# luoao-kddi/SCP

Hardware: AMD Instinct MI355X
Metric: KITTI frames/sec encode (SCP-EHEM, level 16) + bpp match vs ref (higher is better)
Workload: dtype f32 (dense layers and attention as bf16x3 split on bf16 MFMA, feature kNN as f16x3 split on f16 MFMA, fp32 accumulate; position kNN / CDF in fp32); 1 GPU; SCP-EHEM KITTI-like synthetic 120k-pt frames, --spher --mullevel lidar_level=16 (BASELINE.json configs[2]), seeded random weights; nodes_per_frame=577403, windows_per_frame=100, frames_per_gpu=46, frames_in_flight=4, frames_per_launch_sequence=1, transform=host-numpy on a prefetch thread (strict identity: the reference's integers), parallelism=frame-sharded x1, rank_cores=256, rank_cores_pinned=False

## Files before the change

include/scp.h:

```cpp
#ifndef SCP_H
#define SCP_H
#include <stddef.h>
#include <stdint.h>

#ifdef __cplusplus
extern "C" {
#endif

#define SCP_API __attribute__((visibility("default")))

#define SCP_OK 0
#define SCP_EINVAL (-1)
#define SCP_ENOMEM (-2)
#define SCP_ESMALL (-3)
#define SCP_EHIP (-4)
#define SCP_ESTATE (-5)

#define SCP_MAX_DEPTH 21
#define SCP_MAX_SEGMENTS 62

#define SCP_ABI_VERSION 220
SCP_API int scp_version(void);
SCP_API int scp_last_hip_error(void);
SCP_API int scp_device_count(void);
SCP_API int scp_device_name(char *buf, int cap);

typedef struct scp_ctx scp_ctx;
enum { SCP_CTX_KNN_F16X3 = 1, SCP_CTX_ATTENTION_BF16X3 = 2 };
SCP_API int scp_ctx_create(scp_ctx **out);
SCP_API int scp_ctx_destroy(scp_ctx *c);
SCP_API int scp_ctx_set(scp_ctx *c, int32_t key, int32_t value);
SCP_API int scp_ctx_get(const scp_ctx *c, int32_t key);
SCP_API int scp_ctx_make_current(const scp_ctx *c);

enum { SCP_CART = 0, SCP_SPHER = 1, SCP_CYLIN = 2 };

typedef struct scp_quant_info {
    double bin_num;
    double qs[3];
    double offset[3];
    int32_t max_coord;
    int32_t min_coord;
} scp_quant_info;

SCP_API int scp_quantize(const float *xyz, int64_t n, int32_t mode, double qs, double cart_offset,
                 int32_t *q_out, float *tr_out, scp_quant_info *info, void *stream);

typedef struct scp_geom scp_geom;

typedef struct scp_segment {
    int64_t point_begin;
    int64_t point_count;
    int32_t path_len;
    int32_t path_bits;
    int32_t drop_last;
    int32_t reserved;
} scp_segment;

typedef struct scp_segment_info {
    int32_t depth;
    int32_t max_coord;
    int64_t n_leaves;
    int64_t n_nodes;
    int64_t node_base;
    int64_t level_count[SCP_MAX_DEPTH + 1];
} scp_segment_info;

SCP_API int scp_geom_create(scp_geom **out);
SCP_API int scp_geom_destroy(scp_geom *g);

SCP_API int scp_geom_build(scp_geom *g, const int32_t *q, int64_t n, const scp_segment *segs, int32_t nseg,
                   scp_segment_info *info, void *stream);

SCP_API int scp_geom_build_xyz(scp_geom *g, const float *const *frames, const int64_t *n_points, int32_t nframes, int32_t mode,
                               const double *qs, int32_t nshell, double cart_offset, const scp_segment *shells, int32_t *q_out,
                               scp_quant_info *qinfo, scp_segment_info *info, void *stream);

SCP_API int scp_geom_emit_nodes(scp_geom *g, uint8_t *occ, uint8_t *level, uint8_t *octant, int32_t *parent,
                        int32_t *pos, void *stream);

SCP_API int scp_geom_emit_leaves(scp_geom *g, int32_t seg, int32_t *pts, void *stream);

SCP_API int scp_geom_krecords_i64(scp_geom *g, int32_t seg, int64_t *out, void *stream);

enum { SCP_POS_MINMAX = 0,
       SCP_POS_MINMAX_MUL = 1,
       SCP_POS_POW2 = 2 };

SCP_API int scp_geom_context_ehem(scp_geom *g, int32_t seg, int32_t pos_mode, int32_t lidar_level,
                          uint8_t *ctx, float *pos, uint8_t *sym, int64_t *pos_mm, void *stream);

SCP_API int scp_geom_context_ehem_all(scp_geom *g, int32_t pos_mode, int32_t lidar_level, int32_t context_size, uint8_t *ctx, float *pos,
                                      uint8_t *sym_coded, int64_t *pos_mm, void *stream);

SCP_API int scp_geom_context_octattn(scp_geom *g, int32_t seg, uint8_t *ctx, float *pos, uint8_t *sym, void *stream);

SCP_API int scp_knn_topk(const float *x, int32_t B, int32_t n, int32_t C, int32_t k, int32_t *idx, void *stream);

SCP_API int scp_knn_topk_packed(const float *x, const int32_t *ctab, int32_t total_rows, int32_t C, int32_t *idx, void *stream);
SCP_API int scp_knn_topk_packed_bounded(const float *x, const int32_t *ctab, int32_t total_rows, int32_t C, const float *thr0,
                                int32_t *idx, void *stream);

SCP_API int scp_edge_gather_max(const float *u, const float *v, const int32_t *idx, const float *scale, const float *shift,
                        int32_t B, int32_t n, int32_t Cout, int32_t k, float *out, int32_t out_stride, void *stream);
SCP_API int scp_edge_gather_max_ld(const float *u, int64_t ldu, const float *v, int64_t ldv, const int32_t *idx, const float *scale,
                           const float *shift, int32_t B, int32_t n, int32_t Cout, int32_t k, float *out, int32_t out_stride,
                           void *stream);

SCP_API int scp_swin_attention(const float *q, const float *k, const float *v, const float *bias_table,
                       int32_t B, int32_t Lp, int32_t shift, int32_t ldq, int32_t ldkv, float *out, void *stream);

SCP_API int scp_split_weight_bf16(const float *W, int32_t N, int32_t K, int32_t Npad, int32_t Kpad, void *hi, void *lo, void *stream);
SCP_API int scp_linear_bf16x3(const float *A, int64_t lda, const void *Whi, const void *Wlo, int32_t Kpad, const float *bias,
                      const float *residual, int64_t ldr, float *C, int64_t ldc, int32_t M, int32_t N, int32_t K, int32_t act,
                      void *stream);

SCP_API int scp_split_weight_f16(const float *W, int32_t N, int32_t K, int32_t Npad, int32_t Kpad, void *hi, void *lo,
                                 float *inv_scale, void *stream);
SCP_API int scp_linear_f16x3(const float *A, int64_t lda, const void *Whi, const void *Wlo, const float *w_inv_scale, int32_t Kpad,
                             const float *bias, const float *residual, int64_t ldr, float *C, int64_t ldc, int32_t M, int32_t N,
                             int32_t K, int32_t act, float *row_scale_ws, void *stream);
SCP_API int scp_row_scale_f16(const float *A, int64_t lda, int32_t M, int32_t K, float *scale, float *inv_scale, void *stream);
SCP_API int scp_linear_f16x3_scaled(const float *A, int64_t lda, const void *Whi, const void *Wlo, const float *w_inv_scale, int32_t Kpad,
                                    const float *bias, const float *residual, int64_t ldr, float *C, int64_t ldc, int32_t M, int32_t N,
                                    int32_t K, int32_t act, const float *scale, const float *inv_scale, void *stream);

SCP_API int scp_tile_weight_bf16(const void *plane, int32_t Npad, int32_t Kpad, void *tiled, void *stream);
SCP_API int scp_split_rows_f16(const float *A, int64_t lda, int32_t M, int32_t K, void *hi, void *lo, int64_t ldp, float *scale, float *inv_scale,
                               void *stream);
SCP_API int scp_layernorm_add_split_f16(const float *a, const float *b, int64_t rows, int32_t C, const float *gamma, const float *beta, float eps,
                                        float *out, void *hi, void *lo, int64_t ldp, float *scale, float *inv_scale, void *stream);
SCP_API int scp_linear_split_f16(const void *Ahi, const void *Alo, int64_t lda, const float *a_inv_scale, const void *Whi, const void *Wlo,
                                 const float *w_inv_scale, int32_t Npad, int32_t Kpad, const float *bias, const float *residual, int64_t ldr,
                                 float *C, int64_t ldc, int32_t M, int32_t N, int32_t K, int32_t act, int32_t cfg, void *stream);
SCP_API int scp_linear_split_f16_max(const void *Ahi, const void *Alo, int64_t lda, const float *a_inv_scale, const void *Whi, const void *Wlo,
                                     const float *w_inv_scale, int32_t Npad, int32_t Kpad, const float *bias, const float *residual, int64_t ldr,
                                     float *C, int64_t ldc, int32_t M, int32_t N, int32_t K, int32_t act, int32_t cfg, uint32_t *row_max,
                                     uint32_t *col_max, int32_t col_lo, int32_t col_hi, int32_t col_rows, void *stream);
SCP_API int scp_row_scale_from_max(const uint32_t *row_max, int32_t M, float *scale, float *inv_scale, void *stream);
SCP_API int scp_linear_split(const void *Ahi, const void *Alo, int64_t lda, const void *Whi, const void *Wlo, int32_t Npad, int32_t Kpad,
                     const float *bias, const float *residual, int64_t ldr, float *C, int64_t ldc, void *Ohi, void *Olo, int64_t ldo,
                     int32_t M, int32_t N, int32_t K, int32_t act, int32_t cfg, void *stream);

SCP_API int scp_linear_split_gather(const void *Ahi, const void *Alo, int64_t lda, const void *Whi, const void *Wlo, int32_t Npad, int32_t Kpad,
                            const float *bias, const float *residual, int64_t ldr, const int64_t *res_map, float *C, int64_t ldc, void *Ohi,
                            void *Olo, int64_t ldo, int32_t M, int32_t N, int32_t K, int32_t act, int32_t cfg, void *stream);
SCP_API int scp_linear_split_hier2(const void *A0hi, const void *A0lo, int64_t lda0, int32_t K0pad, const void *A1hi, const void *A1lo, int64_t lda1,
                                   int64_t M1, const void *W0hi, const void *W0lo, const void *W1hi, const void *W1lo, int32_t Npad,
                                   const int64_t *parent, const float *bias, const float *res, int64_t ldr, const int64_t *res_map, void *Ohi,
                                   void *Olo, int64_t ldo, int32_t M, int32_t N, int32_t act, void *stream);
SCP_API int scp_linear_split_scatter(const void *Ahi, const void *Alo, int64_t lda, const void *Whi, const void *Wlo, int32_t Npad, int32_t Kpad,
                             const float *bias, const int64_t *out_map, float *C, int64_t ldc, int32_t M, int32_t N, int32_t K, int32_t act,
                             int32_t cfg, void *stream);
SCP_API int scp_split_rows(const float *src, int64_t ld_src, int64_t n_src, const int64_t *idx, int32_t C, void *hi, void *lo, int64_t ldo,
                   int64_t rows, void *stream);
SCP_API int scp_layernorm_rows_split(const float *x, int64_t ldx, int64_t n_src_rows, const int64_t *ia, const int64_t *ib, int32_t C,
                             const float *gamma, const float *beta, const float *valid, float eps, void *ohi, void *olo, int64_t ldo,
                             int64_t rows, void *stream);
SCP_API int scp_layernorm_add(const float *a, const float *b, int64_t rows, int32_t C, const float *gamma, const float *beta, float eps,
                              float *out, void *stream);
SCP_API int scp_swin_attention_packed_split(const float *q, const float *k, const float *v, const float *bias_table, const int32_t *wtab,
                                    int32_t total_windows, int32_t shift, int32_t ldq, int32_t ldkv, void *ohi, void *olo, int64_t ldo,
                                    void *stream);


SCP_API int scp_swin_attention_packed(const float *q, const float *k, const float *v, const float *bias_table, const int32_t *wtab,
                              int32_t total_windows, int32_t shift, int32_t ldq, int32_t ldkv, float *out, void *stream);

SCP_API int scp_layernorm_rows(const float *x, int64_t ldx, int64_t n_src_rows, const int64_t *ia, const int64_t *ib, int32_t C,
                       const float *gamma, const float *beta, const float *valid, float eps, float *out, int64_t ldo, int64_t rows,
                       void *stream);
SCP_API int scp_gather_rows(const float *src, int64_t lds, const int64_t *idx, int32_t C, float *out, int64_t ldo, int64_t rows, void *stream);

SCP_API int scp_linear_f32(const float *A, int64_t lda, const float *W, const float *bias, float *C, int64_t ldc, int32_t M, int32_t N, int32_t K,
                   int32_t act, void *stream);

SCP_API int scp_octattn_attention(const float *q_u, const float *k, const float *k_u, const float *v, const float *v_u,
                          int32_t B, int32_t c, int32_t H, int32_t hd, float *out, float *out_u, void *stream);

SCP_API int64_t scp_octattn_f16x3_ws_bytes(int32_t B, int32_t c, int32_t H);
SCP_API int scp_octattn_attention_f16x3(const float *q_u, const float *k, const float *k_u, const float *v, const float *v_u,
                                        int64_t ldkv, int32_t B, int32_t c, int32_t H, int32_t hd, float *out, float *out_u, void *workspace,
                                        int64_t ws_bytes, void *stream);
SCP_API int scp_octattn_attention_f16x3_vmax(const float *q_u, const float *k, const float *k_u, const float *v, const float *v_u,
                                             int64_t ldkv, int32_t B, int32_t c, int32_t H, int32_t hd, float *out, float *out_u, void *workspace,
                                             int64_t ws_bytes, const uint32_t *vmax_bits, void *stream);
SCP_API int scp_octattn_attention_rowinv(const float *q_u, int64_t qw, int64_t qr, const float *k, const float *v, int64_t kw, int64_t kr,
                                         const float *k_u, const float *v_u, int64_t uw, int64_t ur, float *out, float *out_u, int64_t ow,
                                         int64_t orr, int32_t B, int32_t q0, int32_t q1, int32_t qoff, int32_t H, int32_t hd, void *stream);
SCP_API int scp_decode_expand_octattn(const int64_t *sym, const int64_t *cum, const uint8_t *ctx, const int32_t *apos, int64_t n, int32_t L,
                                      int32_t shift, int32_t depth, uint8_t *cctx, int32_t *capos, float *cpos, uint8_t *occ8, void *stream);
SCP_API int scp_octattn_embed(const uint8_t *ctx, const float *pos, int64_t n, int32_t c, const float *occ_enc, int32_t d_occ,
                              const float *level_enc, int32_t d_lvl, int32_t max_level, const float *octant_enc, int32_t d_oct,
                              const float *pos_w, const float *pos_b, int32_t d_pos, const float *pe, int32_t level_cap, float *E,
                              void *hi, void *lo, int64_t ldp, float *scale, float *inv_scale, void *stream);

SCP_API int scp_softmax_cdf(const float *logits, int64_t ld, int64_t n, int32_t nsym, const uint8_t *sym,
                    float *pmf, uint32_t *lohi, uint16_t *cdf_full, void *stream);
SCP_API int scp_pmf_cdf(const float *pmf, int64_t n, int32_t nsym, const uint8_t *sym, uint32_t *lohi,
                uint16_t *cdf_full, void *stream);

SCP_API int scp_ac_encode_cdf(const uint16_t *cdf, const int16_t *sym, int64_t n, int32_t Lp, uint8_t *out, size_t cap,
                      size_t *out_len);
SCP_API int scp_ac_encode_lohi(const uint32_t *lohi, int64_t n, uint8_t *out, size_t cap, size_t *out_len);
typedef struct scp_ac_dec scp_ac_dec;
SCP_API int scp_ac_dec_new(scp_ac_dec **d, const uint8_t *stream, size_t len, int32_t Lp);
SCP_API int scp_ac_dec_next(scp_ac_dec *d, const uint16_t *cdf_row);
SCP_API int scp_ac_dec_run(scp_ac_dec *d, const uint16_t *cdf, int64_t n, int16_t *out);
SCP_API int scp_ac_dec_free(scp_ac_dec *d);

typedef struct scp_legacy_node { uint32_t nodeid, octant, parent; uint8_t oct; uint32_t pos[3]; } scp_legacy_node;
SCP_API void *new_vector(void);
SCP_API void delete_vector(void *v);
SCP_API int vector_size(void *v);
SCP_API void *vector_get(void *v, int level);
SCP_API void vector_push_back(void *v, int i);
SCP_API void *genOctreeInterface(void *v, const double *xyz, int n);
SCP_API int Nodes_size(void *level);
SCP_API scp_legacy_node *Nodes_get(void *level, int i);
SCP_API int int_size(void *codes);
SCP_API int int_get(void *codes, int i);

SCP_API int scp_nn_sqdist_f64(const double *a, int64_t na, const double *b, int64_t nb, double *d2, void *stream);

SCP_API int scp_embed_gather(const uint8_t *ctx, const float *pos, const int64_t *inmap, int64_t n_tokens, const float *occ_enc,
                     const float *level_enc, const float *octant_enc, float *x, float *pos_out, int64_t *occ_self, int64_t rows,
                     void *stream);

SCP_API int scp_packed_plan_sizes(const int64_t *lengths, int32_t W, int64_t *rows_out);
SCP_API int scp_packed_plan(const int64_t *lengths, int32_t W, int64_t *tables_dev, void *const *outs, int32_t n_outs, void *stream);

SCP_API int scp_decode_expand(const int64_t *sym, const int64_t *cum, const int32_t *pos, const uint8_t *anc, const uint8_t *octant, int64_t n,
                              int32_t L, int32_t shift, int32_t lv_next, int32_t lv_clamp, int32_t polar, double mn, double den, int32_t *cpos,
                              uint8_t *canc, uint8_t *coct, uint8_t *cctx, float *cposn, uint8_t *occ8, void *stream);

SCP_API int scp_swin_ln_linear(const float *x, int64_t ldx, const float *valid, const void *Whi, const void *Wlo, const float *bias,
                               const float *wbeta, float eps, float *out, int64_t ldo, int32_t M, int32_t N, void *stream);
SCP_API int scp_swin_post_attn(const void *Ohi, const void *Olo, int64_t ldo_in, const float *x, int64_t ldx, const void *W, const float *bp,
                               const float *b1, const float *b2, float eps, float *out, int64_t ldc, int32_t M, const int32_t *tile_list,
                               int32_t n_tiles, void *stream);
SCP_API int64_t scp_swin_post_attn_weight_bytes(void);
SCP_API double scp_gelu_prescale(void);

SCP_API int scp_swin_merge(const float *x, int64_t ldx, int64_t n_src, const int64_t *ia, const int64_t *ib, const void *W, const float *wbeta,
                           float eps, float *out, int64_t ldo, int32_t M, void *stream);

SCP_API int scp_geo_edge_mlps(const float *pos1, int64_t ld1, const float *pos2, int64_t ld2, const float *pos3, int64_t ld3, const void *W,
                              const float *bias, float *out, int64_t ldo, int32_t M, void *stream);
SCP_API int scp_mlp3_rows(const float *x, int64_t ldx, int64_t n_src, const int64_t *in_map, const void *W, const float *bias, float *out, int64_t ldo,
                          const int64_t *out_map, int32_t M, int32_t N, void *stream);

SCP_API int scp_swin_kv_planes(const float *k, const float *v, int64_t ldkv, int64_t rows, void *khi, void *klo, void *vthi, void *vtlo, void *stream);
SCP_API int scp_swin_ln_qkv(const float *x, int64_t ldx, const float *valid, const void *Whi, const void *Wlo, const float *bias, const float *wbeta,
                            float eps, float *q, int64_t ldq, void *planes, int64_t Tp, int32_t M, int32_t N, void *stream);
SCP_API int scp_swin_attention_packed_planes(const float *q, const void *khi, const void *klo, const void *vthi, const void *vtlo,
                                             const float *bias_table, const int32_t *wtab, int32_t total_windows, int32_t shift, int32_t ldq,
                                             float *out, void *ohi, void *olo, int64_t ldo, const float *valid, void *stream);

#ifdef __cplusplus
}
#endif
#endif
```

scp_amd/csrc/rowchain.hip:

```cpp
#include <stdlib.h>
#include "scp_internal.h"

typedef __bf16 rbf16x8 __attribute__((ext_vector_type(8)));
typedef float rf32x16 __attribute__((ext_vector_type(16)));
typedef float rf32x4 __attribute__((ext_vector_type(4)));
typedef int ri32x4 __attribute__((ext_vector_type(4)));
typedef __attribute__((address_space(3))) void *rc_lds_ptr_t;
typedef const __attribute__((address_space(1))) void *rc_glb_ptr_t;

#define RC_ROWS 128
#define RC_SLOT 32768
#define RC_RING (4 * RC_SLOT)
#define RC_BOUNCE 4096
#define RC_OFF_BOUNCE RC_RING
#define RC_OFF_BIAS (RC_RING + 4 * RC_BOUNCE)
#define RC_LDS (RC_OFF_BIAS + 16384)

__device__ __forceinline__ void rc_dma16(const void *g, char *l) {
    __builtin_amdgcn_global_load_lds((rc_glb_ptr_t)g, (rc_lds_ptr_t)l, 16, 0, 0);
}

typedef float rf32x2 __attribute__((ext_vector_type(2)));
typedef __bf16 rbf16x2 __attribute__((ext_vector_type(2)));
typedef unsigned ru32x4 __attribute__((ext_vector_type(4)));
typedef unsigned ru32x2 __attribute__((ext_vector_type(2)));
__device__ __forceinline__ unsigned rc_pack2(float a, float b) {
    const rf32x2 v = {a, b};
    return __builtin_bit_cast(unsigned, __builtin_convertvector(v, rbf16x2));
}
__device__ __forceinline__ void rc_split2(float a, float b, unsigned &hi, unsigned &lo) {
    asm volatile("" : "+v"(a), "+v"(b));
    hi = rc_pack2(a, b);
    lo = rc_pack2(a - __builtin_bit_cast(float, hi << 16), b - __builtin_bit_cast(float, hi & 0xffff0000u));
}
__device__ __forceinline__ void rc_split8(const float *f, rbf16x8 &hi, rbf16x8 &lo) {
    ru32x4 h, l;
#pragma unroll
    for (int i = 0; i < 4; ++i) { unsigned a, b; rc_split2(f[2 * i], f[2 * i + 1], a, b); h[i] = a; l[i] = b; }
    hi = __builtin_bit_cast(rbf16x8, h);
    lo = __builtin_bit_cast(rbf16x8, l);
}

struct RcLane {
    int lane, col, h, w;
    int frag;
    int rg;
};

__device__ __forceinline__ RcLane rc_lane() {
    RcLane L;
    const int tid = threadIdx.x;
    L.lane = tid & 63; L.col = L.lane & 31; L.h = L.lane >> 5;
    L.w = __builtin_amdgcn_readfirstlane(tid >> 6);
    L.frag = (L.col & 15) * 64 + ((L.h ^ ((L.col >> 2) & 3)) << 4);
    L.rg = L.col >> 4;
    return L;
}

__device__ __forceinline__ void rc_issue_rowchunk(const RcLane &L, const __bf16 *Whi, const __bf16 *Wlo, int g, char *slot) {
#pragma unroll
    for (int j = 0; j < 4; ++j) {
        const int p = L.w + 4 * j;
        const int64_t off = ((int64_t)g * 16 + p) * 512 + L.lane * 8;
        rc_dma16(Whi + off, slot + p * 1024);
        rc_dma16(Wlo + off, slot + 16384 + p * 1024);
    }
}

__device__ __forceinline__ void rc_issue_kchunk(const RcLane &L, const __bf16 *Whi, const __bf16 *Wlo, int c, int nks, char *slot) {
#pragma unroll
    for (int j = 0; j < 4; ++j) {
        const int p = L.w + 4 * j;
        const int64_t off = ((int64_t)p * nks + c) * 512 + L.lane * 8;
        rc_dma16(Whi + off, slot + p * 1024);
        rc_dma16(Wlo + off, slot + 16384 + p * 1024);
    }
}

__device__ __forceinline__ rbf16x8 rc_frag_rowchunk(const RcLane &L, const char *slot, int plane, int s) {
    return *(const rbf16x8 *)(slot + plane * 16384 + (L.rg * 8 + (s >> 1)) * 1024 + (L.frag ^ ((s & 1) << 5)));
}

__device__ __forceinline__ rbf16x8 rc_frag_kchunk(const RcLane &L, const char *slot, int plane, int b, int t) {
    return *(const rbf16x8 *)(slot + plane * 16384 + (2 * b + L.rg) * 1024 + (L.frag ^ (t << 5)));
}

#define RC_DS_READ4_WAIT(d0, a0, o0, d1, a1, o1, d2, a2, o2, d3, a3, o3)                                                              \
    asm volatile("ds_read_b128 %0, %4 offset:%8\n\tds_read_b128 %1, %5 offset:%9\n\tds_read_b128 %2, %6 offset:%10\n\t"                   \
                 "ds_read_b128 %3, %7 offset:%11\n\ts_waitcnt lgkmcnt(0)"                                                              \
                 : "=&v"(d0), "=&v"(d1), "=&v"(d2), "=&v"(d3) : "v"(a0), "v"(a1), "v"(a2), "v"(a3), "n"(o0), "n"(o1), "n"(o2), "n"(o3) : "memory")
#define RC_DS_READ(dst, addr, off) asm volatile("ds_read_b128 %0, %1 offset:%2" : "=v"(dst) : "v"(addr), "n"(off) : "memory")

__device__ __forceinline__ void rc_mfma3x2(rf32x16 &c0, rf32x16 &c1, const rbf16x8 &a0h, const rbf16x8 &a0l, const rbf16x8 &a1h,
                                           const rbf16x8 &a1l, const rbf16x8 &bh, const rbf16x8 &bl) {
    c0 = __builtin_amdgcn_mfma_f32_32x32x16_bf16(a0l, bh, c0, 0, 0, 0);
    c1 = __builtin_amdgcn_mfma_f32_32x32x16_bf16(a1l, bh, c1, 0, 0, 0);
    c0 = __builtin_amdgcn_mfma_f32_32x32x16_bf16(a0h, bl, c0, 0, 0, 0);
    c1 = __builtin_amdgcn_mfma_f32_32x32x16_bf16(a1h, bl, c1, 0, 0, 0);
    c0 = __builtin_amdgcn_mfma_f32_32x32x16_bf16(a0h, bh, c0, 0, 0, 0);
    c1 = __builtin_amdgcn_mfma_f32_32x32x16_bf16(a1h, bh, c1, 0, 0, 0);
}

__device__ __forceinline__ void rc_store_block(const RcLane &L, char *bounce, const rf32x4 v[4], __amdgpu_buffer_rsrc_t rs, int ldo_bytes, int voff,
                                               int ch0) {
#pragma unroll
    for (int q = 0; q < 4; ++q)
        *(rf32x4 *)(bounce + L.col * 128 + (((2 * q + L.h) ^ (L.col & 7)) << 4)) = v[q];
    asm volatile("s_waitcnt lgkmcnt(0)" ::: "memory");
    rf32x4 y[4];
#pragma unroll
    for (int it = 0; it < 4; ++it) {
        const int rho = 8 * it + (L.lane >> 3), kap = L.lane & 7;
        y[it] = *(const rf32x4 *)(bounce + rho * 128 + ((kap ^ (rho & 7)) << 4));
    }
#pragma unroll
    for (int it = 0; it < 4; ++it) __builtin_amdgcn_raw_buffer_store_b128(__builtin_bit_cast(ri32x4, y[it]), rs, voff, it * 8 * ldo_bytes + ch0 * 4, 0);
    asm volatile("s_waitcnt lgkmcnt(0)" ::: "memory");
}

__device__ __forceinline__ void rc_ln_stats(const float *v , float eps, float &mean, float &rstd) {
    float s = 0.f;
#pragma unroll
    for (int i = 0; i < 128; i += 4) s += (v[i] + v[i + 1]) + (v[i + 2] + v[i + 3]);
    s += __shfl_xor(s, 32);
    mean = s * (1.0f / 256.0f);
    float q = 0.f;
#pragma unroll
    for (int i = 0; i < 128; ++i) { const float d = v[i] - mean; q += d * d; }
    q += __shfl_xor(q, 32);
    rstd = rsqrtf(q * (1.0f / 256.0f) + eps);
}

struct RcLnLinArgs {
    const float *x; int64_t ldx;
    const float *valid;
    const __bf16 *Whi, *Wlo;
    const float *bias, *wbeta;
    float *out; int64_t ldo;
    int M, N;
    float eps;
    int probe;
    unsigned long long *dbg;
    __bf16 *planes; int64_t plane_bytes; int nq;
    int ngroups;
};

#define RC_DS_WRITE(addr, val, off) asm volatile("ds_write_b128 %0, %1 offset:%2" :: "v"(addr), "v"(val), "n"(off) : "memory")

#define RC_SB __builtin_amdgcn_sched_barrier(0)
#ifndef RC_SKEW
#define RC_SKEW 0
#endif
#if RC_SKEW > 0
#define RC_STEP_BARRIER(WAITS, w)                                                                                                          \
    do {                                                                                                                                   \
        int _rc_n;                                                                                                                         \
        asm volatile("s_waitcnt " WAITS "\n\ts_barrier\n\ts_mov_b32 %0, %1\n\ts_cmp_eq_u32 %0, 0\n\ts_cbranch_scc1 .Lrcskew_done%=\n"          \
                     ".Lrcskew_loop%=:\n\ts_nop 7\n\ts_sub_u32 %0, %0, 1\n\ts_cmp_lg_u32 %0, 0\n\ts_cbranch_scc1 .Lrcskew_loop%=\n"              \
                     ".Lrcskew_done%=:"                                                                                                   \
                     : "=&s"(_rc_n) : "s"((w) * RC_SKEW) : "memory", "scc");                                                                \
    } while (0)
#else
#ifdef RC_PROBE_NOBAR
#define RC_STEP_BARRIER(WAITS, w) asm volatile("s_waitcnt " WAITS ::: "memory")
#else
#define RC_STEP_BARRIER(WAITS, w) asm volatile("s_waitcnt " WAITS "\n\ts_barrier" ::: "memory")
#endif
#endif
#ifdef RC_PROBE_NODMA
#define RC_PROBE_DMA_ON 0
#else
#define RC_PROBE_DMA_ON 1
#endif
#ifdef RC_PROBE_NOFRAG
#define RC_PROBE_FRAG_ON 0
#else
#define RC_PROBE_FRAG_ON 1
#endif
#ifdef RC_DMA_SPREAD
#define RC_DMA_P(s, gap) ((s) < 4 ? 2 * (s) + ((gap) == 3) : (s) + 4)
#define RC_DMA_HERE(s, gap) (((s) < 4 && ((gap) == 1 || (gap) == 3)) || ((s) >= 4 && (s) < 12 && (gap) == 1))
#define RC_DMA_SLOT(s, gap) (RC_DMA_P(s, gap) >> 3)
#define RC_DMA_IDX(s, gap) ((RC_DMA_P(s, gap) >> 1) & 3)
#define RC_DMA_PLANE(s, gap) (RC_DMA_P(s, gap) & 1)
#else
#define RC_DMA_HERE(s, gap) ((s) < 8 && ((gap) == 1 || (gap) == 3))
#define RC_DMA_SLOT(s, gap) ((s) >> 2)
#define RC_DMA_IDX(s, gap) ((s) & 3)
#define RC_DMA_PLANE(s, gap) ((gap) >> 1)
#endif
#ifdef RC_WAIT0
#define RC_FRAG_WAIT() asm volatile("s_waitcnt lgkmcnt(0)" ::: "memory")
#else
#define RC_FRAG_WAIT() asm volatile("s_waitcnt lgkmcnt(3)" ::: "memory")
#endif
#ifndef RC_STORE_AUX
#define RC_STORE_AUX 0
#endif
template <bool LOADX, int PROBE, bool SWAP = false, bool NSWAP = false>
__device__ __forceinline__ void rc_ll_step(const RcLane &L, const RcLnLinArgs &a, char *smem, int half, rf32x16 &c0, rf32x16 &c1,
                                           rf32x16 &p0, rf32x16 &p1, const rbf16x8 (&Xh)[16], const rbf16x8 (&Xl)[16], int g_next,
                                           __amdgpu_buffer_rsrc_t rs_prev, int voff, int ldo_bytes, int ch0_prev, const unsigned (&bw)[4],
                                           unsigned br, const float *xsrc, float (&v)[128], rbf16x8 (&A)[2][4], const float *tb_next, unsigned long long *st,
                                           __amdgpu_buffer_rsrc_t wr_hi, __amdgpu_buffer_rsrc_t wr_lo, const float *sbn = nullptr, unsigned maskh = 0) {
    const unsigned ab = (unsigned)(uintptr_t)(rc_lds_ptr_t)(smem + half * (2 * RC_SLOT)) + L.rg * 8192;
    const unsigned ad0 = ab + L.frag, ad1 = ab + (L.frag ^ 32);
    const unsigned an0 = (unsigned)(uintptr_t)(rc_lds_ptr_t)(smem + (half ^ 1) * (2 * RC_SLOT)) + L.rg * 8192 + L.frag;
    char *nxt = smem + (half ^ 1) * (2 * RC_SLOT);
    rf32x4 rd[4];
    unsigned long long ts0 = 0;
    if (st) ts0 = __builtin_amdgcn_s_memtime();
#pragma unroll
    for (int s = 0; s < 16; ++s) {
        if (st && (s == 1 || s == 8 || s == 15)) { const unsigned long long t = __builtin_amdgcn_s_memtime(); st[s == 1 ? 0 : s == 8 ? 1 : 2] += t - ts0; ts0 = t; }
        if (s == 15) {
            asm volatile("s_waitcnt lgkmcnt(0)" ::: "memory");
            if (PROBE) RC_STEP_BARRIER("vmcnt(0)", L.w);
            else if (LOADX) RC_STEP_BARRIER("vmcnt(24)", L.w);
            else RC_STEP_BARRIER("vmcnt(8)", L.w);
            if (st) { const unsigned long long t = __builtin_amdgcn_s_memtime(); st[3] += t - ts0; ts0 = t; }
        }
        RC_SB;
        const int nb = (s + 1) & 1, ns = (s + 1) & 15;
        const unsigned ra = (ns & 1) ? ad1 : ad0;
#pragma unroll
        for (int gap = 0; gap < 6; ++gap) {
            if (gap < 4) { RC_FRAG_WAIT(); RC_SB; }
#define RC_LL_MFMA(c, wf, xf) c = SWAP ? __builtin_amdgcn_mfma_f32_32x32x16_bf16(xf, wf, c, 0, 0, 0) : __builtin_amdgcn_mfma_f32_32x32x16_bf16(wf, xf, c, 0, 0, 0)
            if (gap == 0) RC_LL_MFMA(c0, A[s & 1][1], Xh[s]);
            if (gap == 1) RC_LL_MFMA(c1, A[s & 1][3], Xh[s]);
            if (gap == 2) RC_LL_MFMA(c0, A[s & 1][0], Xl[s]);
            if (gap == 3) RC_LL_MFMA(c1, A[s & 1][2], Xl[s]);
            if (gap == 4) RC_LL_MFMA(c0, A[s & 1][0], Xh[s]);
            if (gap == 5) RC_LL_MFMA(c1, A[s & 1][2], Xh[s]);
#undef RC_LL_MFMA
            RC_SB;
            if (gap < 4 && s < 15) {
                if (gap == 0) RC_DS_READ(A[nb][1], ra, 16384 + (ns >> 1) * 1024);
                if (gap == 1) RC_DS_READ(A[nb][3], ra, RC_SLOT + 16384 + (ns >> 1) * 1024);
                if (gap == 2) RC_DS_READ(A[nb][0], ra, (ns >> 1) * 1024);
                if (gap == 3) RC_DS_READ(A[nb][2], ra, RC_SLOT + (ns >> 1) * 1024);
            }
            if (s < 8 && (gap == 1 || gap == 3) && !(PROBE & 2)) {
                const int slot = s >> 2, pb = L.w + 4 * (s & 3), plane = gap >> 1;
                const int soff = ((g_next + slot) * 16 + pb) * 1024;
                __builtin_amdgcn_raw_ptr_buffer_load_lds(plane ? wr_lo : wr_hi, (rc_lds_ptr_t)(nxt + slot * RC_SLOT + plane * 16384 + pb * 1024), 16,
                                                         L.lane * 16, soff, 0, 0);
            }
            if ((s == 8 || s == 11) && gap < 4 && !(PROBE & 8)) {
                const rf32x16 &pp = (s == 8) ? p0 : p1;
                const rf32x4 t = {pp[4 * gap], pp[4 * gap + 1], pp[4 * gap + 2], pp[4 * gap + 3]};
                RC_DS_WRITE(bw[gap], t, 0);
            }
            if ((s == 9 || s == 12) && gap < 4 && !(PROBE & 8))
                asm volatile("ds_read_b128 %0, %1 offset:%2" : "=v"(rd[gap]) : "v"(br), "n"(gap * 1024) : "memory");
            if ((s == 10 || s == 13) && gap < 4 && !(PROBE & 8))
                __builtin_amdgcn_raw_buffer_store_b128(__builtin_bit_cast(ri32x4, rd[gap]), rs_prev, voff,
                                                       gap * 8 * ldo_bytes + (ch0_prev + 32 * (s == 13 ? 1 : 0)) * 4, RC_STORE_AUX);
            if (LOADX && s >= 14 && gap < 4 && !(PROBE & 4)) {
#pragma unroll
                for (int t = 8 * (s - 14) + 2 * gap; t < 8 * (s - 14) + 2 * gap + 2; ++t) {
                    const rf32x4 q0 = *(const rf32x4 *)(xsrc + 16 * t), q1 = *(const rf32x4 *)(xsrc + 16 * t + 4);
#pragma unroll
                    for (int u = 0; u < 4; ++u) { v[8 * t + u] = q0[u]; v[8 * t + 4 + u] = q1[u]; }
                }
            }
            if (NSWAP && s == 14 && gap >= 4) {
                const float bb = sbn[32 * (gap - 4)], bwv = sbn[32 * (gap - 4) + 1024];
                rf32x16 &pp = (gap == 4) ? p0 : p1;
#pragma unroll
                for (int r = 0; r < 16; ++r) pp[r] = ((maskh >> (8 * (r >> 2) + (r & 3))) & 1u) ? bwv : bb;
            }
            if (!NSWAP && s == 14 && gap >= 4) {
#pragma unroll
                for (int q = 2 * (gap - 4); q < 2 * (gap - 4) + 2; ++q) {
                    const rf32x4 b0 = *(const rf32x4 *)(tb_next + 8 * q), b1 = *(const rf32x4 *)(tb_next + 32 + 8 * q);
#pragma unroll
                    for (int u = 0; u < 4; ++u) { p0[4 * q + u] = b0[u]; p1[4 * q + u] = b1[u]; }
                }
            }
            RC_SB;
        }
    }
    RC_DS_READ4_WAIT(A[0][1], an0, 16384, A[0][3], an0, RC_SLOT + 16384, A[0][0], an0, 0, A[0][2], an0, RC_SLOT);
    if (st) { const unsigned long long t = __builtin_amdgcn_s_memtime(); st[4] += t - ts0; }
}

template <int PROBE, bool KV = false>
__global__ __launch_bounds__(256, 1) void rc_ln_linear_kernel(const RcLnLinArgs a) {
    extern __shared__ __attribute__((aligned(1024))) char smem[];
    const RcLane L = rc_lane();
    const int ntiles = (a.M + RC_ROWS - 1) / RC_ROWS;
    const int nsteps = a.N >> 6;
    float *sb = (float *)(smem + RC_OFF_BIAS), *sbw = sb + 1024;
    for (int i = threadIdx.x; i < a.N; i += 256) {
        const float b = a.bias ? a.bias[i] : 0.f;
        sb[i] = b; sbw[i] = b + (a.wbeta ? a.wbeta[i] : 0.f);
    }
    __syncthreads();
    const int ngr = a.ngroups > 1 ? a.ngroups : 1;
    int tile = blockIdx.x / ngr;
    const int tstride = (int)gridDim.x / ngr;
    const int j0 = (int)(blockIdx.x % ngr) * (nsteps / ngr), j1 = j0 + nsteps / ngr;
    if (tile >= ntiles) return;
    char *bounce = smem + RC_OFF_BOUNCE + L.w * RC_BOUNCE;
    unsigned bw[4];
#pragma unroll
    for (int q = 0; q < 4; ++q) bw[q] = (unsigned)(uintptr_t)(rc_lds_ptr_t)(bounce + L.col * 128 + (((2 * q + L.h) ^ (L.col & 7)) << 4));
    const unsigned br0 = (unsigned)(uintptr_t)(rc_lds_ptr_t)(bounce + (L.lane >> 3) * 128 + (((L.lane & 7) ^ ((L.lane >> 3) & 7)) << 4));
    const int ldo_bytes = (int)(a.ldo * 4);
    const int voff = (32 * L.w + (L.lane >> 3)) * ldo_bytes + (L.lane & 7) * 16;
    const __amdgpu_buffer_rsrc_t rs_none = __builtin_amdgcn_make_buffer_rsrc(a.out, 0, 0, 0x00020000);
    const int pbytes = (int)a.plane_bytes;
    const __amdgpu_buffer_rsrc_t prs = __builtin_amdgcn_make_buffer_rsrc((void *)a.planes, 0, KV ? (int)(4 * a.plane_bytes) : 0, 0x00020000);

    const int wbytes = ((a.N + 255) & ~255) * 512;
    const __amdgpu_buffer_rsrc_t wr_hi = __builtin_amdgcn_make_buffer_rsrc((void *)a.Whi, 0, wbytes, 0x00020000);
    const __amdgpu_buffer_rsrc_t wr_lo = __builtin_amdgcn_make_buffer_rsrc((void *)a.Wlo, 0, wbytes, 0x00020000);
    unsigned long long t_step = 0, t_ln = 0, t_drain = 0, t_prev = 0, n_tiles = 0;
    unsigned long long tsl[5] = {0, 0, 0, 0, 0};
    const bool DBG = a.dbg != nullptr;
    if (DBG) t_prev = __builtin_amdgcn_s_memtime();
    auto stamp = [&](unsigned long long &acc_t) { if (DBG) { const unsigned long long t = __builtin_amdgcn_s_memtime(); acc_t += t - t_prev; t_prev = t; } };

    rc_issue_rowchunk(L, a.Whi, a.Wlo, 2 * j0, smem);
    rc_issue_rowchunk(L, a.Whi, a.Wlo, 2 * j0 + 1, smem + RC_SLOT);
    float v[128];
    auto xrow = [&](int t) {
        const int r = t * RC_ROWS + 32 * L.w + L.col;
        return a.x + (int64_t)(r < a.M ? r : a.M - 1) * a.ldx + 8 * L.h;
    };
    {
        const float *src = xrow(tile);
#pragma unroll
        for (int s = 0; s < 16; ++s) {
            const rf32x4 q0 = *(const rf32x4 *)(src + 16 * s), q1 = *(const rf32x4 *)(src + 16 * s + 4);
#pragma unroll
            for (int u = 0; u < 4; ++u) { v[8 * s + u] = q0[u]; v[8 * s + 4 + u] = q1[u]; }
        }
    }
    rbf16x8 A[2][4];
    {
        SCP_BARRIER_DMA(0);
        const unsigned ad0 = (unsigned)(uintptr_t)(rc_lds_ptr_t)(smem) + L.rg * 8192 + L.frag;
        RC_DS_READ4_WAIT(A[0][1], ad0, 16384, A[0][3], ad0, RC_SLOT + 16384, A[0][0], ad0, 0, A[0][2], ad0, RC_SLOT);
    }
    int gstep = 0;
    for (; tile < ntiles; tile += tstride) {
        const int m0 = tile * RC_ROWS;
        const int row = m0 + 32 * L.w + L.col;
        const int rowc = row < a.M ? row : a.M - 1;
        float keep = (row < a.M) ? 1.0f : 0.0f;
        if (a.valid) keep *= a.valid[rowc];
        float mean, rstd;
        rc_ln_stats(v, a.eps, mean, rstd);
        const float sc = rstd * keep;
        rbf16x8 Xh[16], Xl[16];
#pragma unroll
        for (int s = 0; s < 16; ++s) {
            float f[8];
#pragma unroll
            for (int i = 0; i < 8; ++i) f[i] = (v[8 * s + i] - mean) * sc;
            rc_split8(f, Xh[s], Xl[s]);
        }
        stamp(t_ln);
        const float *tb = (keep != 0.f ? sbw : sb) + 4 * L.h;
        const int64_t rows_left = (int64_t)a.M - m0;
        const int64_t span = (rows_left < RC_ROWS ? rows_left : RC_ROWS) * a.ldo * 4;
        const __amdgpu_buffer_rsrc_t rs = (a.probe & 1) ? rs_none : __builtin_amdgcn_make_buffer_rsrc(a.out + (int64_t)m0 * a.ldo, 0, (int)span, 0x00020000);
        const bool more = tile + tstride < ntiles;
        const float *xnext = xrow(more ? tile + tstride : tile);

        rf32x16 acc[2][2];
#pragma unroll
        for (int q = 0; q < 4; ++q) {
            const rf32x4 b0 = *(const rf32x4 *)(tb + 64 * j0 + 8 * q), b1 = *(const rf32x4 *)(tb + 64 * j0 + 32 + 8 * q);
#pragma unroll
            for (int u = 0; u < 4; ++u) { acc[0][0][4 * q + u] = b0[u]; acc[0][1][4 * q + u] = b1[u]; }
        }
        if (!KV) {
        for (int j = j0; j < j1; j += 2) {
            if (j + 2 == j1)
                rc_ll_step<true, PROBE>(L, a, smem, gstep & 1, acc[0][0], acc[0][1], acc[1][0], acc[1][1], Xh, Xl, 2 * (j + 1), j > j0 ? rs : rs_none, voff,
                                 ldo_bytes, 64 * (j - 1), bw, br0, xnext, v, A, tb + 64 * (j + 1), DBG ? tsl : nullptr, wr_hi, wr_lo);
            else
                rc_ll_step<false, PROBE>(L, a, smem, gstep & 1, acc[0][0], acc[0][1], acc[1][0], acc[1][1], Xh, Xl, 2 * (j + 1), j > j0 ? rs : rs_none, voff,
                                  ldo_bytes, 64 * (j - 1), bw, br0, xnext, v, A, tb + 64 * (j + 1), DBG ? tsl : nullptr, wr_hi, wr_lo);
            ++gstep;
            rc_ll_step<false, PROBE>(L, a, smem, gstep & 1, acc[1][0], acc[1][1], acc[0][0], acc[0][1], Xh, Xl, (j + 2 < j1) ? 2 * (j + 2) : 2 * j0, rs, voff,
                              ldo_bytes, 64 * j, bw, br0, xnext, v, A, tb + 64 * ((j + 2 < j1) ? j + 2 : j0), DBG ? tsl : nullptr, wr_hi, wr_lo);
            ++gstep;
        }
        stamp(t_step);
        asm volatile("s_waitcnt lgkmcnt(0)" ::: "memory");
#pragma unroll
        for (int blk = 0; blk < 2; ++blk) {
            rf32x4 o[4];
#pragma unroll
            for (int q = 0; q < 4; ++q)
#pragma unroll
                for (int u = 0; u < 4; ++u) o[q][u] = acc[1][blk][4 * q + u];
            rc_store_block(L, bounce, o, rs, ldo_bytes, voff, 64 * (j1 - 1) + 32 * blk);
        }
        } else {
        const int nq = a.nq;
        const unsigned kmask = (unsigned)__builtin_amdgcn_ballot_w64(keep != 0.f);
        const unsigned maskh = kmask >> (4 * L.h);
        const float *sbl = sb + L.col;
        const int kvoff = (m0 + 32 * L.w + (L.lane >> 3)) * 512 + (L.lane & 7) * 16;
        const int vblk = ((m0 >> 5) + L.w) * 4;
        auto split_pair = [&](float x0, float x1, int plane) {
            const unsigned hh = rc_pack2(x0, x1);
            return plane ? rc_pack2(x0 - __builtin_bit_cast(float, hh << 16), x1 - __builtin_bit_cast(float, hh & 0xffff0000u)) : hh;
        };
        auto store_k = [&](const rf32x16 &c0, const rf32x16 &c1, int head) {
            ri32x4 y[2][4];
#pragma unroll
            for (int plane = 0; plane < 2; ++plane) {
#pragma unroll
                for (int b = 0; b < 2; ++b)
#pragma unroll
                    for (int q = 0; q < 4; ++q) {
                        const rf32x16 &c = b ? c1 : c0;
                        *(ru32x2 *)(bounce + L.col * 128 + (((4 * b + q) ^ (L.col & 7)) << 4) + 8 * L.h) =
                            (ru32x2){split_pair(c[4 * q], c[4 * q + 1], plane), split_pair(c[4 * q + 2], c[4 * q + 3], plane)};
                    }
#pragma unroll
                for (int it = 0; it < 4; ++it) y[plane][it] = *(const ri32x4 *)(bounce + it * 1024 + L.lane * 16);
            }
#pragma unroll
            for (int plane = 0; plane < 2; ++plane)
#pragma unroll
                for (int it = 0; it < 4; ++it)
                    __builtin_amdgcn_raw_buffer_store_b128(y[plane][it], prs, kvoff, it * 8 * 512 + head * 128 + plane * pbytes, 0);
            asm volatile("s_waitcnt lgkmcnt(0)" ::: "memory");
        };
        auto store_v = [&](const rf32x16 &c0, const rf32x16 &c1, int head) {
            ri32x4 y[2][4];
#pragma unroll
            for (int plane = 0; plane < 2; ++plane) {
#pragma unroll
                for (int b = 0; b < 2; ++b)
#pragma unroll
                    for (int cc = 0; cc < 2; ++cc) {
                        const rf32x16 &c = b ? c1 : c0;
                        const int d = L.col + 32 * b, R = d >> 1, sl = (d & 1) * 4 + 2 * cc + L.h;
                        *(ru32x4 *)(bounce + R * 128 + ((sl ^ (R & 7)) << 4)) =
                            (ru32x4){split_pair(c[8 * cc], c[8 * cc + 1], plane), split_pair(c[8 * cc + 2], c[8 * cc + 3], plane),
                                     split_pair(c[8 * cc + 4], c[8 * cc + 5], plane), split_pair(c[8 * cc + 6], c[8 * cc + 7], plane)};
                    }
#pragma unroll
                for (int it = 0; it < 4; ++it) y[plane][it] = *(const ri32x4 *)(bounce + it * 1024 + L.lane * 16);
            }
#pragma unroll
            for (int plane = 0; plane < 2; ++plane)
#pragma unroll
                for (int it = 0; it < 4; ++it)
                    __builtin_amdgcn_raw_buffer_store_b128(y[plane][it], prs, L.lane * 16, it * 1024 + (vblk + head) * 4096 + (2 + plane) * pbytes, 0);
            asm volatile("s_waitcnt lgkmcnt(0)" ::: "memory");
        };
        auto role = [&](int j) { return j < nq ? 0 : (j < nq + 4 ? 1 : 2); };
        if (role(j0) == 2) {
#pragma unroll
            for (int blk = 0; blk < 2; ++blk) {
                const float bb = sbl[64 * j0 + 32 * blk], bwv = sbl[64 * j0 + 32 * blk + 1024];
#pragma unroll
                for (int r = 0; r < 16; ++r) acc[0][blk][r] = ((maskh >> (8 * (r >> 2) + (r & 3))) & 1u) ? bwv : bb;
            }
        }
        auto post = [&](int j, const rf32x16 &c0, const rf32x16 &c1) {
            const int r = role(j);
            if (r == 1) store_k(c0, c1, j - nq);
            else if (r == 2) store_v(c0, c1, j - nq - 4);
        };
        for (int j = j0; j < j1; j += 2) {
            const int jn = j + 2 < j1 ? j + 2 : j0;
            const bool val = role(j) == 2, nval = role(jn) == 2;
            const __amdgpu_buffer_rsrc_t rsa = (j > j0 && role(j - 1) == 0) ? rs : rs_none, rsb = role(j) == 0 ? rs : rs_none;
            const int gn = 2 * jn;
            const float *tbn = tb + 64 * jn, *sbn1 = sbl + 64 * (j + 1), *sbn2 = sbl + 64 * jn;
#define RC_STEP_A(LX, SW) rc_ll_step<LX, PROBE, SW, SW>(L, a, smem, gstep & 1, acc[0][0], acc[0][1], acc[1][0], acc[1][1], Xh, Xl, 2 * (j + 1), rsa, voff, ldo_bytes, \
                                                64 * (j - 1), bw, br0, xnext, v, A, tb + 64 * (j + 1), DBG ? tsl : nullptr, wr_hi, wr_lo, sbn1, maskh)
#define RC_STEP_B(SW, NSW) rc_ll_step<false, PROBE, SW, NSW>(L, a, smem, gstep & 1, acc[1][0], acc[1][1], acc[0][0], acc[0][1], Xh, Xl, gn, rsb, voff, ldo_bytes, 64 * j, bw, \
                                                     br0, xnext, v, A, tbn, DBG ? tsl : nullptr, wr_hi, wr_lo, sbn2, maskh)
            if (!val) RC_STEP_A(false, false);
            else if (j + 2 == j1) RC_STEP_A(true, true);
            else RC_STEP_A(false, true);
            ++gstep;
            post(j, acc[0][0], acc[0][1]);
            if (!val) { if (nval) RC_STEP_B(false, true); else RC_STEP_B(false, false); }
            else { if (nval) RC_STEP_B(true, true); else RC_STEP_B(true, false); }
            ++gstep;
            post(j + 1, acc[1][0], acc[1][1]);
#undef RC_STEP_A
#undef RC_STEP_B
        }
        stamp(t_step);
        if (role(j1 - 1) == 0) {
            asm volatile("s_waitcnt lgkmcnt(0)" ::: "memory");
#pragma unroll
            for (int blk = 0; blk < 2; ++blk) {
                rf32x4 o[4];
#pragma unroll
                for (int q = 0; q < 4; ++q)
#pragma unroll
                    for (int u = 0; u < 4; ++u) o[q][u] = acc[1][blk][4 * q + u];
                rc_store_block(L, bounce, o, rs, ldo_bytes, voff, 64 * (j1 - 1) + 32 * blk);
            }
        }
        }
        stamp(t_drain);
        ++n_tiles;
    }
    if (DBG && L.lane == 0) {
        unsigned long long *o = a.dbg + ((size_t)blockIdx.x * 4 + L.w) * 8;
        o[0] = tsl[3]; o[1] = t_step; o[2] = t_ln; o[3] = t_drain; o[4] = n_tiles; o[5] = tsl[0]; o[6] = tsl[1]; o[7] = tsl[2] + tsl[4];
    }
    SCP_WAIT_DMA(0);
}

struct RcPostArgs {
    const __bf16 *Ohi, *Olo; int64_t ldo_in;
    const float *x; int64_t ldx;
    const void *W;
    const float *bp, *b1, *b2;
    float *out; int64_t ldc;
    int M;
    float eps;
    unsigned long long *dbg;
    int dbg_mode;
    const int32_t *tile_list; int n_list;
};

#define RC_W_PROJ 0
#define RC_W_FC1 (256 * 512)
#define RC_W_FC2 (RC_W_FC1 + 1024 * 512)
#define RC_W_PLANE (RC_W_FC2 + 256 * 2048)
struct RcSlotSrc { int base, stride; };

__device__ __forceinline__ void rc_dma_piece(const RcLane &L, __amdgpu_buffer_rsrc_t wr, const RcSlotSrc &src, char *slot_lds, int s, int plane) {
    const int pb = L.w + 4 * (s & 3);
    const int soff = src.base + pb * src.stride + plane * RC_W_PLANE;
    __builtin_amdgcn_raw_ptr_buffer_load_lds(wr, (rc_lds_ptr_t)(slot_lds + plane * 16384 + pb * 1024), 16, L.lane * 16, soff, 0, 0);
}

struct RcFragAddr { unsigned r0, r1, k0, k1; };
__device__ __forceinline__ RcFragAddr rc_frag_addr(const RcLane &L, char *half_base) {
    RcFragAddr f;
    const unsigned b = (unsigned)(uintptr_t)(rc_lds_ptr_t)half_base;
    f.r0 = b + L.rg * 8192 + L.frag; f.r1 = b + L.rg * 8192 + (L.frag ^ 32);
    f.k0 = b + L.rg * 1024 + L.frag; f.k1 = b + L.rg * 1024 + (L.frag ^ 32);
    return f;
}

#ifdef RC_PROBE_SHAPE16
__device__ __forceinline__ void rc_mfma_shape16(rf32x16 &acc, const rbf16x8 &a, const rbf16x8 &b) {
    rf32x4 q0 = {acc[0], acc[1], acc[2], acc[3]}, q1 = {acc[4], acc[5], acc[6], acc[7]};
    q0 = __builtin_amdgcn_mfma_f32_16x16x32_bf16(a, b, q0, 0, 0, 0);
    q1 = __builtin_amdgcn_mfma_f32_16x16x32_bf16(a, b, q1, 0, 0, 0);
    acc[0] = q0[0]; acc[1] = q0[1]; acc[2] = q0[2]; acc[3] = q0[3];
    acc[4] = q1[0]; acc[5] = q1[1]; acc[6] = q1[2]; acc[7] = q1[3];
}
#define RC_MFMA_AVA(acc, a, b) rc_mfma_shape16(acc, a, b)
#define RC_MFMA_AVV(acc, a, b) rc_mfma_shape16(acc, a, __builtin_bit_cast(rbf16x8, b))
#else
#define RC_MFMA_AVA(acc, a, b) acc = __builtin_amdgcn_mfma_f32_32x32x16_bf16(a, b, acc, 0, 0, 0)
#define RC_MFMA_AVV(acc, a, b) acc = __builtin_amdgcn_mfma_f32_32x32x16_bf16(a, __builtin_bit_cast(rbf16x8, b), acc, 0, 0, 0)
#endif
#define RC_MFMA_DRAIN() do { } while (0)

template <bool NEXT_BODY>
__device__ __forceinline__ void rc_gemm_step(const RcLane &L, char *smem, int half, rf32x16 &c0, rf32x16 &c1, const rbf16x8 (&Bh)[16],
                                             const rbf16x8 (&Bl)[16], rbf16x8 (&A)[2][4], __amdgpu_buffer_rsrc_t wr, const RcSlotSrc &n0,
                                             const RcSlotSrc &n1) {
    const RcFragAddr f = rc_frag_addr(L, smem + half * (2 * RC_SLOT)), fn = rc_frag_addr(L, smem + (half ^ 1) * (2 * RC_SLOT));
    char *nxt = smem + (half ^ 1) * (2 * RC_SLOT);
#pragma unroll
    for (int s = 0; s < 16; ++s) {
        if (s == 15) RC_STEP_BARRIER("vmcnt(0) lgkmcnt(0)", L.w);
        RC_SB;
        const int nb = (s + 1) & 1, ns = (s + 1) & 15;
#pragma unroll
        for (int gap = 0; gap < 6; ++gap) {
            if (gap < 4 && RC_PROBE_FRAG_ON) { RC_FRAG_WAIT(); RC_SB; }
            if (gap == 0) RC_MFMA_AVA(c0, A[s & 1][1], Bh[s]);
            if (gap == 1) RC_MFMA_AVA(c1, A[s & 1][3], Bh[s]);
            if (gap == 2) RC_MFMA_AVV(c0, A[s & 1][0], Bl[s]);
            if (gap == 3) RC_MFMA_AVV(c1, A[s & 1][2], Bl[s]);
            if (gap == 4) RC_MFMA_AVA(c0, A[s & 1][0], Bh[s]);
            if (gap == 5) RC_MFMA_AVA(c1, A[s & 1][2], Bh[s]);
            RC_SB;
            if (s < 15 && RC_PROBE_FRAG_ON) {
                const unsigned ra = (ns & 1) ? f.r1 : f.r0;
                if (gap == 0) RC_DS_READ(A[nb][1], ra, 16384 + (ns >> 1) * 1024);
                if (gap == 1) RC_DS_READ(A[nb][3], ra, RC_SLOT + 16384 + (ns >> 1) * 1024);
                if (gap == 2) RC_DS_READ(A[nb][0], ra, (ns >> 1) * 1024);
                if (gap == 3) RC_DS_READ(A[nb][2], ra, RC_SLOT + (ns >> 1) * 1024);
            }
            if (RC_DMA_HERE(s, gap) && RC_PROBE_DMA_ON) rc_dma_piece(L, wr, RC_DMA_SLOT(s, gap) ? n1 : n0, nxt + RC_DMA_SLOT(s, gap) * RC_SLOT, RC_DMA_IDX(s, gap), RC_DMA_PLANE(s, gap));
            RC_SB;
        }
    }
    if (NEXT_BODY) RC_DS_READ4_WAIT(A[0][1], fn.r0, 16384, A[0][3], fn.k0, RC_SLOT + 16384, A[0][0], fn.r0, 0, A[0][2], fn.k0, RC_SLOT);
    else RC_DS_READ4_WAIT(A[0][1], fn.r0, 16384, A[0][3], fn.r0, RC_SLOT + 16384, A[0][0], fn.r0, 0, A[0][2], fn.r0, RC_SLOT);
}

struct RcGelu { float ea, eb, pa, pb, wa, wb, xa, xb, ga, gb; unsigned hw; };
__device__ __forceinline__ void rc_gelu_stage(int st, RcGelu &g, float ya, float yb, unsigned &wh, unsigned &wl) {
#ifdef RC_NOGELU
    if (st == 0) { g.ga = ya; g.gb = yb; asm volatile("" : "+v"(g.ga), "+v"(g.gb)); }
    if (st == 10) { g.hw = rc_pack2(g.ga, g.gb); wh = g.hw; asm volatile("" : "+v"(g.hw)); }
    if (st == 11) wl = rc_pack2(g.ga - __builtin_bit_cast(float, g.hw << 16), g.gb - __builtin_bit_cast(float, g.hw & 0xffff0000u));
    return;
#endif
    switch (st) {
    case 0: g.ea = -ya * ya; g.eb = -yb * yb; break;
    case 1: g.ea = __builtin_amdgcn_exp2f(g.ea); g.eb = __builtin_amdgcn_exp2f(g.eb); break;
    case 2: g.pa = fmaf(SCP_GELU_C4, __builtin_fabsf(ya), SCP_GELU_C3); g.pb = fmaf(SCP_GELU_C4, __builtin_fabsf(yb), SCP_GELU_C3); break;
    case 3: g.pa = fmaf(g.pa, __builtin_fabsf(ya), SCP_GELU_C2); g.pb = fmaf(g.pb, __builtin_fabsf(yb), SCP_GELU_C2); break;
    case 4: g.pa = fmaf(g.pa, __builtin_fabsf(ya), SCP_GELU_C1); g.pb = fmaf(g.pb, __builtin_fabsf(yb), SCP_GELU_C1); break;
    case 5: g.pa = fmaf(g.pa, __builtin_fabsf(ya), SCP_GELU_C0); g.pb = fmaf(g.pb, __builtin_fabsf(yb), SCP_GELU_C0); break;
    case 6: g.pa = __builtin_amdgcn_rcpf(g.pa); g.pb = __builtin_amdgcn_rcpf(g.pb); break;
    case 7: g.wa = __builtin_fabsf(ya) * g.ea; g.wb = __builtin_fabsf(yb) * g.eb; break;
    case 8: asm("v_max_f32_e32 %0, 0, %1" : "=v"(g.xa) : "v"(ya)); asm("v_max_f32_e32 %0, 0, %1" : "=v"(g.xb) : "v"(yb)); break;
    case 9: g.ga = fmaf(-g.wa, g.pa, g.xa); g.gb = fmaf(-g.wb, g.pb, g.xb); break;
    case 10: g.hw = rc_pack2(g.ga, g.gb); wh = g.hw; break;
    default: wl = rc_pack2(g.ga - __builtin_bit_cast(float, g.hw << 16), g.gb - __builtin_bit_cast(float, g.hw & 0xffff0000u)); break;
    }
    switch (st) {
    case 0: case 1: asm volatile("" : "+v"(g.ea), "+v"(g.eb)); break;
    case 2: case 3: case 4: case 5: case 6: asm volatile("" : "+v"(g.pa), "+v"(g.pb)); break;
    case 7: asm volatile("" : "+v"(g.wa), "+v"(g.wb)); break;
    case 8: asm volatile("" : "+v"(g.xa), "+v"(g.xb)); break;
    case 9: asm volatile("" : "+v"(g.ga), "+v"(g.gb)); break;
    case 10: asm volatile("" : "+v"(g.ga), "+v"(g.gb), "+v"(g.hw)); break;
    default: break;
    }
}

template <bool HAS_P1, bool HAS_GELU, int NEXT>
__device__ __forceinline__ void rc_body_step(const RcLane &L, char *smem, int half, rf32x16 (&Y)[8], rf32x16 &a1n, const rf32x16 &a1g,
                                             const ru32x4 (&Hch)[2], const ru32x4 (&Hcl)[2], ru32x4 (&Hnh)[2],
                                             ru32x4 (&Hnl)[2], const rbf16x8 (&Xh)[16], const rbf16x8 (&Xl)[16], rbf16x8 (&A)[2][4],
                                             __amdgpu_buffer_rsrc_t wr, const RcSlotSrc &n0, const RcSlotSrc &n1) {
    const RcFragAddr f = rc_frag_addr(L, smem + half * (2 * RC_SLOT)), fn = rc_frag_addr(L, smem + (half ^ 1) * (2 * RC_SLOT));
    char *nxt = smem + (half ^ 1) * (2 * RC_SLOT);
    RcGelu g;
#pragma unroll
    for (int s = 0; s < 16; ++s) {
        if (s == 15) RC_STEP_BARRIER("vmcnt(0) lgkmcnt(0)", L.w);
        RC_SB;
        const int nb = (s + 1) & 1, ns = (s + 1) & 15;
        const int blk = s >> 1, t = s & 1;
#pragma unroll
        for (int gap = 0; gap < 6; ++gap) {
            if (HAS_P1 && gap < 4 && RC_PROBE_FRAG_ON) { RC_FRAG_WAIT(); RC_SB; }
            if (!HAS_P1 && (gap == 1 || gap == 3) && RC_PROBE_FRAG_ON) { asm volatile("s_waitcnt lgkmcnt(1)" ::: "memory"); RC_SB; }
            if (gap == 0 && HAS_P1) RC_MFMA_AVA(a1n, A[s & 1][1], Xh[s]);
            if (gap == 1) RC_MFMA_AVV(Y[blk], A[s & 1][3], Hch[t]);
            if (gap == 2 && HAS_P1) RC_MFMA_AVV(a1n, A[s & 1][0], Xl[s]);
            if (gap == 3) RC_MFMA_AVV(Y[blk], A[s & 1][2], Hcl[t]);
            if (gap == 4 && HAS_P1) RC_MFMA_AVA(a1n, A[s & 1][0], Xh[s]);
            if (gap == 5) RC_MFMA_AVV(Y[blk], A[s & 1][2], Hch[t]);
            RC_SB;
            if (s < 15 && RC_PROBE_FRAG_ON) {
                if (gap == 0 && HAS_P1) RC_DS_READ(A[nb][1], (ns & 1) ? f.r1 : f.r0, 16384 + (ns >> 1) * 1024);
                if (gap == 1) RC_DS_READ(A[nb][3], (ns & 1) ? f.k1 : f.k0, RC_SLOT + 16384 + (ns >> 1) * 2048);
                if (gap == 2 && HAS_P1) RC_DS_READ(A[nb][0], (ns & 1) ? f.r1 : f.r0, (ns >> 1) * 1024);
                if (gap == 3) RC_DS_READ(A[nb][2], (ns & 1) ? f.k1 : f.k0, RC_SLOT + (ns >> 1) * 2048);
            }
            if (RC_DMA_HERE(s, gap) && RC_PROBE_DMA_ON) rc_dma_piece(L, wr, RC_DMA_SLOT(s, gap) ? n1 : n0, nxt + RC_DMA_SLOT(s, gap) * RC_SLOT, RC_DMA_IDX(s, gap), RC_DMA_PLANE(s, gap));
            if (HAS_GELU) {
                const int k = s >> 1, st = (s & 1) * 6 + gap;
                unsigned wh = 0, wl = 0;
// ... 595 lines not shown
#pragma unroll
                for (int s = 0; s < 16; ++s) {
                    float f[8];
#pragma unroll
                    for (int i = 0; i < 8; ++i) f[i] = (vb[8 * s + i] - mean) * rstd;
                    rc_split8(f, Xh[s], Xl[s]);
                }
            }
        }
        asm volatile("s_waitcnt lgkmcnt(0)" ::: "memory");
        const int64_t rows_left = (int64_t)a.M - m0;
        const int64_t span = (rows_left < RC_ROWS ? rows_left : RC_ROWS) * a.ldo * 4;
        const __amdgpu_buffer_rsrc_t rs = __builtin_amdgcn_make_buffer_rsrc(a.out + (int64_t)m0 * a.ldo, 0, (int)span, 0x00020000);
#pragma unroll
        for (int b = 0; b < 8; ++b) {
            rf32x4 o[4];
#pragma unroll
            for (int q = 0; q < 4; ++q)
#pragma unroll
                for (int u = 0; u < 4; ++u) o[q][u] = Y[b][4 * q + u];
            rc_store_block(L, bounce, o, rs, ldo_bytes, voff, 32 * b);
        }
    }
    SCP_WAIT_DMA(0);
}

extern "C" SCP_API int scp_swin_merge(const float *x, int64_t ldx, int64_t n_src, const int64_t *ia, const int64_t *ib, const void *W, const float *wbeta,
                                      float eps, float *out, int64_t ldo, int32_t M, void *stream);

struct RcEdgeArgs {
    const float *p1, *p2, *p3; int64_t ld1, ld2, ld3;
    const void *W; const float *bias;
    float *out; int64_t ldo; int M;
};

__device__ __forceinline__ float rc_leaky(float y) { return y > 0.f ? y : 0.01f * y; }

__global__ __launch_bounds__(256, 1) void rc_edge_mlp_kernel(const RcEdgeArgs a) {
    extern __shared__ __attribute__((aligned(1024))) char smem[];
    const RcLane L = rc_lane();
    const int ntiles = (a.M + RC_ROWS - 1) / RC_ROWS;
    float *sb = (float *)(smem + RC_OFF_BIAS);
    for (int i = threadIdx.x; i < 5 * 256 + 128; i += 256) sb[i] = a.bias[i];
    __syncthreads();
    int tile = blockIdx.x;
    if (tile >= ntiles) return;
    char *bounce = smem + RC_OFF_BOUNCE + L.w * RC_BOUNCE;
    const int ldo_bytes = (int)(a.ldo * 4);
    const int voff = (32 * L.w + (L.lane >> 3)) * ldo_bytes + (L.lane & 7) * 16;
    const __amdgpu_buffer_rsrc_t wr = __builtin_amdgcn_make_buffer_rsrc((void *)a.W, 0, 2 * RC_W_PLANE, 0x00020000);
    auto src = [&](int t, int k) {
        int m, g;
        if (t < 8) { m = t & 1; g = t >> 1; }
        else if (t < 16) { m = t >> 2; g = t & 3; }
        else if (t < 24) { m = 4 + (t & 1); g = (t - 16) >> 1; }
        else if (t < 28) { m = 6; g = t & 3; }
        else { m = 7; g = t - 28; }
        RcSlotSrc r = {m * 131072 + (2 * g + k) * 16384, 1024};
        return r;
    };
    {
        const RcSlotSrc s0 = src(0, 0), s1 = src(0, 1);
#pragma unroll
        for (int q = 0; q < 4; ++q)
#pragma unroll
            for (int plane = 0; plane < 2; ++plane) { rc_dma_piece(L, wr, s0, smem, q, plane); rc_dma_piece(L, wr, s1, smem + RC_SLOT, q, plane); }
    }
    rbf16x8 A[2][4];
    {
        SCP_BARRIER_DMA(0);
        const RcFragAddr f = rc_frag_addr(L, smem);
        RC_DS_READ4_WAIT(A[0][1], f.r0, 16384, A[0][3], f.r0, RC_SLOT + 16384, A[0][0], f.r0, 0, A[0][2], f.r0, RC_SLOT);
    }
    int gstep = 0, t = 0;
    for (; tile < ntiles; tile += gridDim.x) {
        const int m0 = tile * RC_ROWS;
        const int row = m0 + 32 * L.w + L.col;
        const int64_t rowc = row < a.M ? row : a.M - 1;
        const float *q1 = a.p1 + rowc * a.ld1 + 8 * L.h, *q2 = a.p2 + rowc * a.ld2 + 8 * L.h, *q3 = a.p3 + rowc * a.ld3 + 8 * L.h;
        rbf16x8 Xh[16], Xl[16], Zh[16], Zl[16];
        rf32x16 Y[8];
        auto frag_of = [&](const float *p, rbf16x8 &hi, rbf16x8 &lo) {
            const rf32x4 v0 = *(const rf32x4 *)p, v1 = *(const rf32x4 *)(p + 4);
            const float f[8] = {v0[0], v0[1], v0[2], v0[3], v1[0], v1[1], v1[2], v1[3]};
            rc_split8(f, hi, lo);
        };
        auto to_frags = [&](rbf16x8 (&Fh)[16], rbf16x8 (&Fl)[16], bool act) {
#pragma unroll
            for (int b = 0; b < 8; ++b)
#pragma unroll
                for (int tt = 0; tt < 2; ++tt) {
                    float fr[8];
#pragma unroll
                    for (int i = 0; i < 8; ++i) fr[i] = act ? rc_leaky(Y[b][8 * tt + i]) : Y[b][8 * tt + i];
                    rc_split8(fr, Fh[2 * b + tt], Fl[2 * b + tt]);
                }
        };
#define RC_STEP(Fh, Fl) { const int tn = t + 1 < 30 ? t + 1 : 0; rc_gemm_step<false>(L, smem, gstep & 1, c0, c1, Fh, Fl, A, wr, src(tn, 0), src(tn, 1)); ++gstep; t = tn; }
#define RC_LAYER(LAYER, NG, STEPS)                                                                                                             \
        for (int g = 0; g < (NG); ++g) {                                                                                                       \
            rf32x16 c0, c1;                                                                                                                    \
            _Pragma("unroll") for (int q = 0; q < 4; ++q) {                                                                                    \
                const rf32x4 b0 = *(const rf32x4 *)(sb + 256 * (LAYER) + 64 * g + 8 * q + 4 * L.h), b1 = *(const rf32x4 *)(sb + 256 * (LAYER) + 64 * g + 32 + 8 * q + 4 * L.h); \
                _Pragma("unroll") for (int u = 0; u < 4; ++u) { c0[4 * q + u] = b0[u]; c1[4 * q + u] = b1[u]; }                                 \
            }                                                                                                                                  \
            asm volatile("s_waitcnt lgkmcnt(0)" ::: "memory");                                                                                 \
            STEPS                                                                                                                              \
            switch (g) { case 0: Y[0] = c0; Y[1] = c1; break; case 1: Y[2] = c0; Y[3] = c1; break; case 2: Y[4] = c0; Y[5] = c1; break; default: Y[6] = c0; Y[7] = c1; break; } \
        }
#pragma unroll
        for (int s = 0; s < 16; ++s) frag_of(s < 4 ? q1 + 16 * s : (s < 12 ? q2 + 16 * (s - 4) : q3 + 16 * (s - 12)), Xh[s], Xl[s]);
#pragma unroll
        for (int s = 0; s < 16; ++s) {
            if (s < 12) frag_of(q3 + 64 + 16 * s, Zh[s], Zl[s]);
            else { Zh[s] = __builtin_bit_cast(rbf16x8, (ru32x4){0u, 0u, 0u, 0u}); Zl[s] = Zh[s]; }
        }
        RC_LAYER(0, 4, RC_STEP(Xh, Xl) RC_STEP(Zh, Zl))
        to_frags(Xh, Xl, true);
        RC_LAYER(1, 4, RC_STEP(Xh, Xl))
        to_frags(Xh, Xl, true);
        RC_LAYER(2, 4, RC_STEP(Xh, Xl))
        to_frags(Xh, Xl, false);
#pragma unroll
        for (int s = 0; s < 16; ++s) frag_of(q3 + 16 * s, Zh[s], Zl[s]);
        RC_LAYER(3, 4, RC_STEP(Xh, Xl) RC_STEP(Zh, Zl))
        to_frags(Xh, Xl, true);
        RC_LAYER(4, 4, RC_STEP(Xh, Xl))
        to_frags(Xh, Xl, true);
        RC_LAYER(5, 2, RC_STEP(Xh, Xl))
#undef RC_LAYER
#undef RC_STEP
        asm volatile("s_waitcnt lgkmcnt(0)" ::: "memory");
        const int64_t rows_left = (int64_t)a.M - m0;
        const int64_t span = (rows_left < RC_ROWS ? rows_left : RC_ROWS) * a.ldo * 4;
        const __amdgpu_buffer_rsrc_t rs = __builtin_amdgcn_make_buffer_rsrc(a.out + (int64_t)m0 * a.ldo, 0, (int)span, 0x00020000);
#pragma unroll
        for (int b = 0; b < 4; ++b) {
            rf32x4 o[4];
#pragma unroll
            for (int q = 0; q < 4; ++q)
#pragma unroll
                for (int u = 0; u < 4; ++u) o[q][u] = Y[b][4 * q + u];
            rc_store_block(L, bounce, o, rs, ldo_bytes, voff, 32 * b);
        }
    }
    SCP_WAIT_DMA(0);
}

struct RcMlp3Args {
    const float *x; int64_t ldx; const int64_t *in_map; int64_t n_src;
    const void *W; const float *bias;
    float *out; int64_t ldo; const int64_t *out_map;
    int M, N;
};

__global__ __launch_bounds__(256, 1) void rc_mlp3_kernel(const RcMlp3Args a) {
    extern __shared__ __attribute__((aligned(1024))) char smem[];
    const RcLane L = rc_lane();
    const int ntiles = (a.M + RC_ROWS - 1) / RC_ROWS;
    float *sb = (float *)(smem + RC_OFF_BIAS);
    for (int i = threadIdx.x; i < 3 * 256; i += 256) sb[i] = a.bias[i];
    __syncthreads();
    int tile = blockIdx.x;
    if (tile >= ntiles) return;
    char *bounce = smem + RC_OFF_BOUNCE + L.w * RC_BOUNCE;
    const __amdgpu_buffer_rsrc_t wr = __builtin_amdgcn_make_buffer_rsrc((void *)a.W, 0, 2 * RC_W_PLANE, 0x00020000);
    auto src = [&](int t, int k) {
        RcSlotSrc r = {(t >> 2) * 131072 + (2 * (t & 3) + k) * 16384, 1024};
        return r;
    };
    {
        const RcSlotSrc s0 = src(0, 0), s1 = src(0, 1);
#pragma unroll
        for (int q = 0; q < 4; ++q)
#pragma unroll
            for (int plane = 0; plane < 2; ++plane) { rc_dma_piece(L, wr, s0, smem, q, plane); rc_dma_piece(L, wr, s1, smem + RC_SLOT, q, plane); }
    }
    rbf16x8 A[2][4];
    {
        SCP_BARRIER_DMA(0);
        const RcFragAddr f = rc_frag_addr(L, smem);
        RC_DS_READ4_WAIT(A[0][1], f.r0, 16384, A[0][3], f.r0, RC_SLOT + 16384, A[0][0], f.r0, 0, A[0][2], f.r0, RC_SLOT);
    }
    int gstep = 0, t = 0;
    for (; tile < ntiles; tile += gridDim.x) {
        const int m0 = tile * RC_ROWS;
        const int row = m0 + 32 * L.w + L.col;
        int64_t srow = row < a.M ? row : a.M - 1;
        if (a.in_map) srow = a.in_map[srow];
        srow = srow < a.n_src ? (srow < 0 ? 0 : srow) : a.n_src - 1;
        const float *q0 = a.x + srow * a.ldx + 8 * L.h;
        rbf16x8 Xh[16], Xl[16];
        rf32x16 Y[8];
        auto to_frags = [&]() {
#pragma unroll
            for (int b = 0; b < 8; ++b)
#pragma unroll
                for (int tt = 0; tt < 2; ++tt) {
                    float fr[8];
#pragma unroll
                    for (int i = 0; i < 8; ++i) fr[i] = rc_leaky(Y[b][8 * tt + i]);
                    rc_split8(fr, Xh[2 * b + tt], Xl[2 * b + tt]);
                }
        };
#define RC_STEP3() { const int tn = t + 1 < 12 ? t + 1 : 0; rc_gemm_step<false>(L, smem, gstep & 1, c0, c1, Xh, Xl, A, wr, src(tn, 0), src(tn, 1)); ++gstep; t = tn; }
#define RC_BIAS3(LAYER)                                                                                                                        \
            rf32x16 c0, c1;                                                                                                                    \
            _Pragma("unroll") for (int q = 0; q < 4; ++q) {                                                                                    \
                const rf32x4 b0 = *(const rf32x4 *)(sb + 256 * (LAYER) + 64 * g + 8 * q + 4 * L.h), b1 = *(const rf32x4 *)(sb + 256 * (LAYER) + 64 * g + 32 + 8 * q + 4 * L.h); \
                _Pragma("unroll") for (int u = 0; u < 4; ++u) { c0[4 * q + u] = b0[u]; c1[4 * q + u] = b1[u]; }                                 \
            }                                                                                                                                  \
            asm volatile("s_waitcnt lgkmcnt(0)" ::: "memory");
#define RC_LAYER3(LAYER)                                                                                                                       \
        for (int g = 0; g < 4; ++g) {                                                                                                          \
            RC_BIAS3(LAYER)                                                                                                                    \
            RC_STEP3()                                                                                                                         \
            switch (g) { case 0: Y[0] = c0; Y[1] = c1; break; case 1: Y[2] = c0; Y[3] = c1; break; case 2: Y[4] = c0; Y[5] = c1; break; default: Y[6] = c0; Y[7] = c1; break; } \
        }
#pragma unroll
        for (int s = 0; s < 16; ++s) {
            const rf32x4 v0 = *(const rf32x4 *)(q0 + 16 * s), v1 = *(const rf32x4 *)(q0 + 16 * s + 4);
            const float f[8] = {v0[0], v0[1], v0[2], v0[3], v1[0], v1[1], v1[2], v1[3]};
            rc_split8(f, Xh[s], Xl[s]);
        }
        RC_LAYER3(0)
        to_frags();
        RC_LAYER3(1)
        to_frags();
        const int kap = L.lane & 7;
        float *orow[4];
#pragma unroll
        for (int it = 0; it < 4; ++it) {
            const int r = m0 + 32 * L.w + 8 * it + (L.lane >> 3);
            const int64_t o = r < a.M ? (a.out_map ? a.out_map[r] : (int64_t)r) : -1;
            orow[it] = o >= 0 ? a.out + o * a.ldo + 4 * kap : nullptr;
        }
        auto store_block = [&](const rf32x16 &c, int ch0) {
#pragma unroll
            for (int q = 0; q < 4; ++q) {
                rf32x4 v;
#pragma unroll
                for (int u = 0; u < 4; ++u) v[u] = c[4 * q + u];
                *(rf32x4 *)(bounce + L.col * 128 + (((2 * q + L.h) ^ (L.col & 7)) << 4)) = v;
            }
            asm volatile("s_waitcnt lgkmcnt(0)" ::: "memory");
            rf32x4 y[4];
#pragma unroll
            for (int it = 0; it < 4; ++it) {
                const int rho = 8 * it + (L.lane >> 3);
                y[it] = *(const rf32x4 *)(bounce + rho * 128 + ((kap ^ (rho & 7)) << 4));
            }
            asm volatile("s_waitcnt lgkmcnt(0)" ::: "memory");
#pragma unroll
            for (int it = 0; it < 4; ++it)
                if (orow[it] && ch0 + 4 * kap < a.N) *(rf32x4 *)(orow[it] + ch0) = y[it];
        };
        for (int g = 0; g < 4; ++g) {
            RC_BIAS3(2)
            RC_STEP3()
            store_block(c0, 64 * g);
            store_block(c1, 64 * g + 32);
        }
#undef RC_LAYER3
#undef RC_BIAS3
#undef RC_STEP3
    }
    SCP_WAIT_DMA(0);
}

extern "C" SCP_API double scp_gelu_prescale(void) { return (double)SCP_GELU_S; }

static int rc_ll_groups(int ntiles, int nsteps, int ncu) {
    static int on = -1;
    if (on < 0) { const char *e = getenv("SCP_RC_GROUPS"); on = (e && e[0] == '0') ? 0 : 1; }
    int best = 1;
    if (on)
        for (int g = 2; g <= nsteps / 2; ++g)
            if ((nsteps / 2) % g == 0 && (int64_t)ntiles * g <= ncu) best = g;
    return best;
}

static unsigned long long *g_rc_dbg = nullptr;
extern "C" SCP_API int scp_rc_debug_buffer(unsigned long long *dev_buf) { g_rc_dbg = dev_buf; return SCP_OK; }

static int g_rc_num_cu = 0, g_rc_grid = 0;
static int g_rc_wide = -2;
static int rc_wide_mode() {
    if (g_rc_wide == -2) { const char *e = getenv("SCP_RC_WIDE"); g_rc_wide = e ? atoi(e) : -1; if (g_rc_wide < -1 || g_rc_wide > 1) g_rc_wide = -1; }
    return g_rc_wide;
}
extern "C" SCP_API int scp_rc_set_wide(int32_t mode) { g_rc_wide = (mode < -1 || mode > 1) ? -1 : mode; return SCP_OK; }
extern "C" SCP_API int scp_rc_set_grid(int32_t workgroups) { g_rc_grid = workgroups > 0 ? workgroups : 0; return SCP_OK; }
static int rc_num_cu() {
    if (g_rc_grid) return g_rc_grid;
    if (!g_rc_num_cu) {
        int dev = 0;
        hipDeviceProp_t p;
        if (hipGetDevice(&dev) != hipSuccess || hipGetDeviceProperties(&p, dev) != hipSuccess) return 256;
        g_rc_num_cu = p.multiProcessorCount > 0 ? p.multiProcessorCount : 256;
    }
    return g_rc_num_cu;
}

extern "C" SCP_API int scp_swin_ln_linear(const float *x, int64_t ldx, const float *valid, const void *Whi, const void *Wlo, const float *bias,
                                          const float *wbeta, float eps, float *out, int64_t ldo, int32_t M, int32_t N, void *stream) {
    if (!x || !Whi || !Wlo || !out || M <= 0 || N <= 0 || (N & 127) || N > 1024 || ldx < 256 || (ldx & 3) || ldo < N || (ldo & 3) ||
        (((uintptr_t)x | (uintptr_t)out | (uintptr_t)Whi | (uintptr_t)Wlo) & 15) || (int64_t)RC_ROWS * ldo * 4 > 0x7fffffffLL)
        return SCP_EINVAL;
    static bool configured = false;
    if (!configured) {
        HIP_TRY(hipFuncSetAttribute((const void *)rc_ln_linear_kernel<0>, hipFuncAttributeMaxDynamicSharedMemorySize, RC_LDS));
        configured = true;
    }
    RcLnLinArgs a;
    a.x = x; a.ldx = ldx; a.valid = valid; a.Whi = (const __bf16 *)Whi; a.Wlo = (const __bf16 *)Wlo; a.bias = bias; a.wbeta = wbeta;
    a.out = out; a.ldo = ldo; a.M = M; a.N = N; a.eps = eps;
    a.planes = nullptr; a.plane_bytes = 0; a.nq = 0;
    { static int pr = -1; if (pr < 0) { const char *e = getenv("SCP_RC_PROBE"); pr = e ? atoi(e) : 0; } a.probe = pr; }
    if (a.probe) { const char *e = getenv("SCP_RC_PROBE"); a.probe = e ? atoi(e) : 0; }
    a.dbg = g_rc_dbg;
    const int ntiles = (M + RC_ROWS - 1) / RC_ROWS;
    const int ncu = rc_num_cu();
    SCP_PROF(SCP_PROF_LN_LINEAR, stream, 2.0 * M * 256.0 * N);
    a.ngroups = rc_ll_groups(ntiles, N / 64, ncu);
    hipLaunchKernelGGL(rc_ln_linear_kernel<0>, dim3((unsigned)(a.ngroups > 1 ? ntiles * a.ngroups : (ntiles < ncu ? ntiles : ncu))), dim3(256), RC_LDS, (hipStream_t)stream, a);
    LAUNCH_CHECK();
    return SCP_OK;
}

extern "C" SCP_API int scp_swin_ln_qkv(const float *x, int64_t ldx, const float *valid, const void *Whi, const void *Wlo, const float *bias,
                                       const float *wbeta, float eps, float *q, int64_t ldq, void *planes, int64_t Tp, int32_t M, int32_t N, void *stream) {
    if (!x || !Whi || !Wlo || !planes || M <= 0 || (M & 127) || (N != 768 && N != 512) || (N == 768 && (!q || ldq < 256 || (ldq & 3))) || ldx < 256 ||
        (ldx & 3) || Tp < M || (Tp & 31) || (((uintptr_t)x | (uintptr_t)q | (uintptr_t)Whi | (uintptr_t)Wlo | (uintptr_t)planes) & 15) ||
        (q && (int64_t)RC_ROWS * ldq * 4 > 0x7fffffffLL) || 4 * Tp * 512 > 0x7fffffffLL)
        return SCP_EINVAL;
    static bool configured = false;
    if (!configured) {
        HIP_TRY(hipFuncSetAttribute((const void *)rc_ln_linear_kernel<0, true>, hipFuncAttributeMaxDynamicSharedMemorySize, RC_LDS));
        configured = true;
    }
    RcLnLinArgs a;
    a.x = x; a.ldx = ldx; a.valid = valid; a.Whi = (const __bf16 *)Whi; a.Wlo = (const __bf16 *)Wlo; a.bias = bias; a.wbeta = wbeta;
    a.out = q; a.ldo = q ? ldq : 256; a.M = M; a.N = N; a.eps = eps; a.probe = 0; a.dbg = nullptr;
    a.planes = (__bf16 *)planes; a.plane_bytes = Tp * 512; a.nq = N / 64 - 8;
    const int ntiles = M / RC_ROWS, ncu = rc_num_cu();
    SCP_PROF(SCP_PROF_LN_LINEAR, stream, 2.0 * M * 256.0 * N);
    a.ngroups = rc_ll_groups(ntiles, N / 64, ncu);
    hipLaunchKernelGGL((rc_ln_linear_kernel<0, true>), dim3((unsigned)(a.ngroups > 1 ? ntiles * a.ngroups : (ntiles < ncu ? ntiles : ncu))), dim3(256), RC_LDS, (hipStream_t)stream, a);
    LAUNCH_CHECK();
    return SCP_OK;
}

extern "C" SCP_API int scp_swin_post_attn(const void *Ohi, const void *Olo, int64_t ldo_in, const float *x, int64_t ldx, const void *W, const float *bp,
                                          const float *b1, const float *b2, float eps, float *out, int64_t ldc, int32_t M, const int32_t *tile_list,
                                          int32_t n_tiles, void *stream) {
    if (!Ohi || !Olo || !x || !W || !bp || !b1 || !b2 || !out || M <= 0 || (tile_list && (n_tiles <= 0 || n_tiles > (M + RC_ROWS - 1) / RC_ROWS)) || ldo_in < 256 || (ldo_in & 7) || ldx < 256 || (ldx & 3) || ldc < 256 ||
        (ldc & 3) || (((uintptr_t)Ohi | (uintptr_t)Olo | (uintptr_t)x | (uintptr_t)out | (uintptr_t)W) & 15) ||
        (int64_t)RC_ROWS * ldc * 4 > 0x7fffffffLL)
        return SCP_EINVAL;
    static bool configured = false;
    if (!configured) {
        HIP_TRY(hipFuncSetAttribute((const void *)rc_post_attn_kernel, hipFuncAttributeMaxDynamicSharedMemorySize, RC_LDS));
        HIP_TRY(hipFuncSetAttribute((const void *)rc_post_attn_wide_kernel, hipFuncAttributeMaxDynamicSharedMemorySize, RC_LDS));
        configured = true;
    }
    RcPostArgs a;
    a.Ohi = (const __bf16 *)Ohi; a.Olo = (const __bf16 *)Olo; a.ldo_in = ldo_in; a.x = x; a.ldx = ldx; a.W = W;
    a.bp = bp; a.b1 = b1; a.b2 = b2; a.out = out; a.ldc = ldc; a.M = M; a.eps = eps;
    a.dbg = g_rc_dbg;
    { const char *e = getenv("SCP_RC_DUMP"); a.dbg_mode = e ? atoi(e) : 0; }
    a.tile_list = tile_list; a.n_list = tile_list ? n_tiles : 0;
    const int ntiles = tile_list ? n_tiles : (M + RC_ROWS - 1) / RC_ROWS;
    const int ncu = rc_num_cu();
    SCP_PROF(SCP_PROF_POST_ATTN, stream, 2.0 * (tile_list ? (double)n_tiles * RC_ROWS : (double)M) * (256.0 * 256.0 + 2.0 * 256.0 * 1024.0));
    if (rc_wide_mode() == 1 || (rc_wide_mode() < 0 && !g_rc_dbg && !a.dbg_mode && 4 * (int64_t)ntiles <= (int64_t)ncu)) {
        const int items = 4 * ntiles;
        hipLaunchKernelGGL(rc_post_attn_wide_kernel, dim3((unsigned)(items < 2 * ncu ? items : 2 * ncu)), dim3(256), RC_LDS, (hipStream_t)stream, a);
        LAUNCH_CHECK();
        return SCP_OK;
    }
    hipLaunchKernelGGL(rc_post_attn_kernel, dim3((unsigned)(ntiles < ncu ? ntiles : ncu)), dim3(256), RC_LDS, (hipStream_t)stream, a);
    LAUNCH_CHECK();
    return SCP_OK;
}

extern "C" SCP_API int64_t scp_swin_post_attn_weight_bytes(void) { return 2 * (int64_t)RC_W_PLANE; }

extern "C" SCP_API int scp_geo_edge_mlps(const float *pos1, int64_t ld1, const float *pos2, int64_t ld2, const float *pos3, int64_t ld3, const void *W,
                                         const float *bias, float *out, int64_t ldo, int32_t M, void *stream) {
    if (!pos1 || !pos2 || !pos3 || !W || !bias || !out || M <= 0 || ld1 < 64 || ld2 < 128 || ld3 < 256 || ((ld1 | ld2 | ld3) & 3) || ldo < 128 || (ldo & 3) ||
        (((uintptr_t)pos1 | (uintptr_t)pos2 | (uintptr_t)pos3 | (uintptr_t)out | (uintptr_t)W) & 15) || (int64_t)RC_ROWS * ldo * 4 > 0x7fffffffLL)
        return SCP_EINVAL;
    static bool configured = false;
    if (!configured) {
        HIP_TRY(hipFuncSetAttribute((const void *)rc_edge_mlp_kernel, hipFuncAttributeMaxDynamicSharedMemorySize, RC_LDS));
        configured = true;
    }
    RcEdgeArgs a;
    a.p1 = pos1; a.p2 = pos2; a.p3 = pos3; a.ld1 = ld1; a.ld2 = ld2; a.ld3 = ld3; a.W = W; a.bias = bias; a.out = out; a.ldo = ldo; a.M = M;
    const int ntiles = (M + RC_ROWS - 1) / RC_ROWS, ncu = rc_num_cu();
    SCP_PROF(SCP_PROF_EDGE_MLP, stream, 2.0 * M * (448.0 * 256 + 2.0 * 256 * 256 + 512.0 * 256 + 256.0 * 256 + 256.0 * 128));
    hipLaunchKernelGGL(rc_edge_mlp_kernel, dim3((unsigned)(ntiles < ncu ? ntiles : ncu)), dim3(256), RC_LDS, (hipStream_t)stream, a);
    LAUNCH_CHECK();
    return SCP_OK;
}

extern "C" SCP_API int scp_mlp3_rows(const float *x, int64_t ldx, int64_t n_src, const int64_t *in_map, const void *W, const float *bias, float *out, int64_t ldo,
                                     const int64_t *out_map, int32_t M, int32_t N, void *stream) {
    if (!x || !W || !bias || !out || M <= 0 || n_src <= 0 || N <= 0 || N > 256 || (N & 3) || ldx < 256 || (ldx & 3) || ldo < N || (ldo & 3) ||
        (((uintptr_t)x | (uintptr_t)out | (uintptr_t)W) & 15))
        return SCP_EINVAL;
    static bool configured = false;
    if (!configured) {
        HIP_TRY(hipFuncSetAttribute((const void *)rc_mlp3_kernel, hipFuncAttributeMaxDynamicSharedMemorySize, RC_LDS));
        configured = true;
    }
    RcMlp3Args a;
    a.x = x; a.ldx = ldx; a.in_map = in_map; a.n_src = n_src; a.W = W; a.bias = bias; a.out = out; a.ldo = ldo; a.out_map = out_map; a.M = M; a.N = N;
    const int ntiles = (M + RC_ROWS - 1) / RC_ROWS, ncu = rc_num_cu();
    SCP_PROF(SCP_PROF_MLP3, stream, 2.0 * M * 3.0 * 256.0 * 256.0);
    hipLaunchKernelGGL(rc_mlp3_kernel, dim3((unsigned)(ntiles < ncu ? ntiles : ncu)), dim3(256), RC_LDS, (hipStream_t)stream, a);
    LAUNCH_CHECK();
    return SCP_OK;
}

extern "C" SCP_API int scp_swin_merge(const float *x, int64_t ldx, int64_t n_src, const int64_t *ia, const int64_t *ib, const void *W, const float *wbeta,
                                      float eps, float *out, int64_t ldo, int32_t M, void *stream) {
    if (!x || !ia || !ib || !W || !out || M <= 0 || n_src <= 0 || ldx < 256 || (ldx & 3) || ldo < 256 || (ldo & 3) ||
        (((uintptr_t)x | (uintptr_t)out | (uintptr_t)W) & 15) || (int64_t)RC_ROWS * ldo * 4 > 0x7fffffffLL)
        return SCP_EINVAL;
    static bool configured = false;
    if (!configured) {
        HIP_TRY(hipFuncSetAttribute((const void *)rc_merge_kernel, hipFuncAttributeMaxDynamicSharedMemorySize, RC_LDS));
        configured = true;
    }
    RcMergeArgs a;
    a.x = x; a.ldx = ldx; a.n_src = n_src; a.ia = ia; a.ib = ib; a.W = W; a.wbeta = wbeta; a.out = out; a.ldo = ldo; a.M = M; a.eps = eps;
    const int ntiles = (M + RC_ROWS - 1) / RC_ROWS, ncu = rc_num_cu();
    SCP_PROF(SCP_PROF_MERGE, stream, 2.0 * M * 512.0 * 256.0);
    hipLaunchKernelGGL(rc_merge_kernel, dim3((unsigned)(ntiles < ncu ? ntiles : ncu)), dim3(256), RC_LDS, (hipStream_t)stream, a);
    LAUNCH_CHECK();
    return SCP_OK;
}
```

scp_amd/models/packed.py:

```python
import numpy as np
import torch
import torch.nn.functional as F

from .. import native
from ..ops import linear_s, leaky_mlp3_s, split_cat, linear, layer_norm, leaky_mlp3, _split, derived, frozen_epoch
from .ehem import SHIFT, WINDOW, _edge_conv_packed, qkv_fused


def _ceil512(a):
    return (a + WINDOW - 1) // WINDOW * WINDOW


def _tokens(L):
    wid = torch.repeat_interleave(torch.arange(L.numel(), device=L.device), L)
    first = torch.cumsum(L, 0) - L
    return wid, torch.arange(int(L.sum()), device=L.device) - first[wid]


class StageLayout:

    def __init__(self, L):
        self.L = L
        self.Lp = _ceil512(L)
        self.base = torch.cumsum(self.Lp, 0) - self.Lp
        self.rows = int(self.Lp.sum())
        self.wid, self.t = _tokens(L)
        self.real_rows = self.base[self.wid] + self.t

    def table(self, real=False):
        reps = self.Lp // WINDOW
        return torch.stack([torch.repeat_interleave(self.base, reps), torch.repeat_interleave(self.L if real else self.Lp, reps)],
                           1).to(torch.int32).contiguous()

    def valid(self):
        v = torch.zeros(self.rows, dtype=torch.float32, device=self.L.device)
        v[self.real_rows] = 1.0
        return v[:, None]

    def row_index(self, counts):
        wid, t = _tokens(counts)
        return self.base[wid] + t


def _merge_maps(cur, nxt):
    dev = cur.L.device
    even = torch.full((nxt.rows,), cur.rows, dtype=torch.int64, device=dev)
    odd = torch.full((nxt.rows,), cur.rows, dtype=torch.int64, device=dev)
    even[nxt.real_rows] = cur.base[nxt.wid] + 2 * nxt.t
    o = 2 * nxt.t + 1
    odd[nxt.real_rows] = torch.where(o < cur.L[nxt.wid], cur.base[nxt.wid] + o, torch.full_like(o, cur.rows))
    return even, odd


def _out_map(q0, counts, first):
    m = torch.full((q0.rows,), -1, dtype=torch.int64, device=q0.L.device)
    wid, t = _tokens(counts)
    m[q0.base[wid] + t] = first[wid] + t
    return m


def _concat_map(l0, ls, s):
    m = torch.zeros(l0.rows, dtype=torch.int64, device=l0.L.device)
    m[l0.real_rows] = ls.base[l0.wid] + (l0.t >> s)
    return m


class PackedPlan:

    def __init__(self, lengths, n_self=5, n_cross=4, device=None, use_native=True):
        dev = device if device is not None else torch.device("cuda", torch.cuda.current_device())
        dev = torch.device(dev)
        if use_native and dev.type == "cuda" and n_self == 5 and n_cross == 4:
            self.c = torch.as_tensor(np.asarray(lengths, np.int64))
            self.n_tokens = int(np.asarray(lengths, np.int64).sum())
            self.rows, self.d = native.packed_plan(lengths, dev)
            return
        c = torch.as_tensor(np.asarray(lengths, np.int64), device=dev)
        self.c = c
        e = c + (c & 1)
        self.self_layouts = [StageLayout(e)]
        for _ in range(n_self - 1):
            self.self_layouts.append(StageLayout((self.self_layouts[-1].L + 1) // 2))
        self.cross_layouts = [StageLayout(e // 2)]
        for _ in range(n_cross - 1):
            self.cross_layouts.append(StageLayout((self.cross_layouts[-1].L + 1) // 2))
        P0, Q0 = self.self_layouts[0], self.cross_layouts[0]
        self.n_tokens = int(c.sum())
        inmap = torch.full((P0.rows,), self.n_tokens, dtype=torch.int64, device=dev)
        inmap[P0.row_index(c)] = torch.arange(self.n_tokens, device=dev)
        a1 = torch.zeros(Q0.rows, dtype=torch.int64, device=dev)
        a2 = torch.zeros(Q0.rows, dtype=torch.int64, device=dev)
        a1[Q0.real_rows] = P0.base[Q0.wid] + 2 * Q0.t
        a2[Q0.real_rows] = P0.base[Q0.wid] + 2 * Q0.t + 1
        ne, no = (c + 1) // 2, c // 2
        coded = torch.cumsum(c, 0) - c
        we, te = _tokens(ne)
        wo, to = _tokens(no)
        self.d = dict(
            inmap=inmap, a1map=a1, a2map=a2, even_rows=Q0.row_index(ne), odd_rows=Q0.row_index(no),
            even_dst=coded[we] + te, odd_dst=coded[wo] + ne[wo] + to,
            self_merge=[_merge_maps(self.self_layouts[s], self.self_layouts[s + 1]) for s in range(n_self - 1)],
            cross_merge=[_merge_maps(self.cross_layouts[s], self.cross_layouts[s + 1]) for s in range(n_cross - 1)],
            self_concat=[_concat_map(P0, self.self_layouts[s], s) for s in range(1, n_self)],
            cross_concat=[_concat_map(Q0, self.cross_layouts[s], s) for s in range(1, n_cross)],
            self_tab=[l.table() for l in self.self_layouts], cross_tab=[l.table() for l in self.cross_layouts],
            knn_tab=P0.table(real=True),
            self_valid=[l.valid().contiguous() for l in self.self_layouts], cross_valid=[l.valid().contiguous() for l in self.cross_layouts],
            self_parent=[_concat_map(self.self_layouts[s], self.self_layouts[s + 1], 1) for s in range(n_self - 1)],
            cross_parent=[_concat_map(self.cross_layouts[s], self.cross_layouts[s + 1], 1) for s in range(n_cross - 1)],
            even_out=_out_map(Q0, ne, coded), odd_out=_out_map(Q0, no, coded + ne))


def _rowchain_weights(layer, cross):
    att = layer.attention.self
    lnb, lna = layer.layernorm_before, layer.layernorm_after
    W, b = qkv_fused(layer, cross)
    fc1, fc2, proj = layer.intermediate.dense, layer.output.dense, layer.attention.output.dense
    srcs = [W, b, lnb.weight, lnb.bias, lna.weight, lna.bias, fc1.weight, fc1.bias, fc2.weight, fc2.bias, proj.weight, proj.bias]
    if cross:
        srcs += [att.query.weight, att.query.bias]

    def build():
        out = dict(kv=native.LnFoldedWeight(W, lnb.weight, lnb.bias), b=b,
                   post=native.PostAttnWeights(proj.weight, proj.bias, lna.weight, lna.bias, fc1.weight, fc1.bias, fc2.weight, fc2.bias))
        if cross:
            out["q"] = native.LnFoldedWeight(att.query.weight, lnb.weight, lnb.bias)
        return out
    return derived(layer, "rowchain+" if cross else "rowchain", srcs, build)


def _block_consts(layer, cross):
    ep = frozen_epoch()
    key = "_scp_fast_x" if cross else "_scp_fast"
    fast = layer.__dict__.get(key) if ep else None
    if fast is not None and fast[0] == ep:
        return fast[1:]
    att = layer.attention.self
    out = (_rowchain_weights(layer, cross), att.relative_position_bias_table, (att.query.bias if cross else None), layer.layernorm_before.eps, layer.layernorm_after.eps)
    if ep:
        layer.__dict__[key] = (ep,) + out
    return out


def _swin_layer_rowchain(layer, x, valid, wtab, shift, query=None, tiles=None, q_pre=None):
    cross = query is not None
    w, table, qbias, eps_b, eps_a = _block_consts(layer, cross)
    v1 = None if valid is None else valid.reshape(-1)
    if native.attention_bf16x3():
        if not cross:
            q, kvp = native.swin_ln_qkv(x, w["kv"], w["b"], eps_b, v1)
        else:
            q = q_pre if q_pre is not None else native.swin_ln_linear(query, w["q"], qbias, eps_b, v1)
            _, kvp = native.swin_ln_qkv(x, w["kv"], w["b"], eps_b, v1)
        o = native.swin_attention_packed_planes(q, kvp, table, wtab, shift, split=True, valid=v1 if tiles is not None else None)
        if tiles is not None and tiles.shape[0] > 0:
            return native.swin_post_attn(o, x, w["post"], eps_a, out=x, tiles=tiles)
        return native.swin_post_attn(o, x, w["post"], eps_a)
    att, lnb = layer.attention.self, layer.layernorm_before
    if not cross:
        qkv = native.swin_ln_linear(x, w["kv"], w["b"], lnb.eps, v1)
        q, k, v = qkv[:, :256], qkv[:, 256:512], qkv[:, 512:]
    else:
        q = q_pre if q_pre is not None else native.swin_ln_linear(query, w["q"], att.query.bias, lnb.eps, v1)
        kv = native.swin_ln_linear(x, w["kv"], w["b"], lnb.eps, v1)
        k, v = kv[:, :256], kv[:, 256:]
    o = native.swin_attention_packed(q, k, v, att.relative_position_bias_table, wtab, shift, split=True)
    return native.swin_post_attn(o, x, w["post"], layer.layernorm_after.eps)


def _swin_layer(layer, x, valid, wtab, shift, query=None, tiles=None, q_pre=None):
    fc1, fc2 = layer.intermediate.dense, layer.output.dense
    if x.shape[1] != 256 or fc1.weight.shape != (1024, 256) or fc2.weight.shape != (256, 1024):
        raise native.ScpError("EHEM's Swin blocks are 256 wide with a 1024-wide MLP (configs/model/ehem.yaml); other widths are not built")
    return _swin_layer_rowchain(layer, x, valid, wtab, shift, query, tiles, q_pre)


def _merge(m, x, maps):
    ev, od = maps
    if x.shape[1] != 256 or m.reduction.weight.shape != (256, 512) or m.reduction.bias is not None:
        raise native.ScpError("SwinPatchMerging: 2 x 256 -> 256 without bias expected")
    mw = derived(m, "rowchain_merge", [m.reduction.weight, m.norm.weight, m.norm.bias],
                 lambda: native.MergeWeights(m.reduction.weight, m.norm.weight, m.norm.bias))
    return native.swin_merge(x, ev, od, mw, m.norm.eps)


def _encoder(enc, x, valids, tabs, merges, query=None, tiles=None, q_pre=None):
    hs = [x]
    for s, stage in enumerate(enc.layers):
        for b, blk in enumerate(stage.blocks):
            x = _swin_layer(blk, x, valids[s], tabs[s], SHIFT if b % 2 else 0, query, None if tiles is None else tiles[s],
                            None if q_pre is None else q_pre[s][b])
        hs.append(x)
        if s < len(enc.layers) - 1:
            x = _merge(stage.downsample, x, merges[s])
            if query is not None and q_pre is None:
                query = _merge(stage.downsample, query, merges[s])
    return hs


def _concat(hs, cmaps, extra=None):
    n = len(hs) - 1 + (1 if extra is not None else 0)
    out = native.SplitAct.empty(hs[1].shape[0], 256 * n, hs[1].device)
    native.split_rows(hs[1], out=out.cols(0, 256))
    for s in range(1, len(hs) - 1):
        native.split_rows(hs[s + 1], idx=cmaps[s - 1], out=out.cols(256 * s, 256 * (s + 1)))
    if extra is not None:
        k = len(hs) - 1
        native.split_rows(extra[0], idx=extra[1], out=out.cols(256 * k, 256 * (k + 1)))
    return out


HIER = True


FUSE2 = __import__("os").environ.get("SCP_CONCAT_FUSE2", "1")[:1] != "0"


def _concat_layer(lin, hs, parents, extra=None, grand=None, a0_pre=None):
    n = len(hs) - 1
    def build():
        W = lin.weight.detach()
        slabs = [W[:, 256 * s:256 * (s + 1)].contiguous() for s in range(n)]
        if extra is not None:
            slabs[0] = torch.cat((slabs[0], W[:, 256 * n:256 * (n + 1)]), 1).contiguous()
        return slabs
    cache = derived(lin, "slabs+" if extra is not None else "slabs", (lin.weight,), build)
    fused = FUSE2 and n >= 3 and grand is not None and native.WTILE and hs[1].shape[0] % 256 == 0
    z = None
    for s in range(n - 1, 1 if fused else 0, -1):
        z = linear_s(native.split_rows(hs[s + 1]), cache[s], None, residual=z, res_map=None if z is None else parents[s], res_first=z is not None)
    if a0_pre is not None:
        native.split_rows(hs[1], out=a0_pre.cols(0, 256))
        a0 = a0_pre
    else:
        a0 = native.split_rows(hs[1]) if extra is None else split_cat((hs[1], extra))
    if fused:
        return native.linear_split_hier2(a0, _split(cache[0]), native.split_rows(hs[2]), _split(cache[1]), parents[0], lin.bias, native.ACT_LEAKY,
                                         residual=z, res_map=grand)
    return linear_s(a0, cache[0], lin.bias, act="leaky", residual=z, res_map=None if z is None else parents[0], res_first=z is not None,
                    want="split")


def _mlp_over_concat(seq, hs, parents, extra=None, grand=None, a0_pre=None):
    a = _concat_layer(seq[0], hs, parents, extra, grand, a0_pre)
    a = linear_s(a, seq[2].weight, seq[2].bias, act="leaky", want="split")
    return linear_s(a, seq[4].weight, seq[4].bias)


CHAIN_HEADS = __import__("os").environ.get("SCP_HEADS", "chain") != "split"


def _mlp3_weights(owner, name, seq):
    return derived(owner, "mlp3_" + name, [seq[i].weight for i in (0, 2, 4)] + [seq[i].bias for i in (0, 2, 4)], lambda: native.Mlp3Weights(seq))


def _head3(model, name, a, out=None, out_map=None, ncols=None):
    seq = getattr(model, name)
    N = seq[4].weight.shape[0]
    if CHAIN_HEADS:
        if out is None:
            out = torch.empty((a.shape[0], -(-N // 4) * 4), dtype=torch.float32, device=a.device)
        native.mlp3_rows(a, _mlp3_weights(model, name, seq), out, out_map=out_map, ncols=ncols)
        return out[:, :N] if out_map is None else None
    sa = native.split_rows(a)
    if out_map is not None:
        sa = linear_s(sa, seq[0].weight, seq[0].bias, act="leaky", want="split")
        sa = linear_s(sa, seq[2].weight, seq[2].bias, act="leaky", want="split")
        native.linear_split_scatter(sa, _split(seq[4].weight), seq[4].bias, out_map, out)
        return None
    return leaky_mlp3_s(seq, sa, out=out)


def _head_to_table(model, a, out_map, table):
    if CHAIN_HEADS and table.stride(0) < 256:
        raise native.ScpError("the coding-order table must have rows of at least 256 floats")
    _head3(model, "prob_pred_mlp1", a, out=table, out_map=out_map)


@torch.no_grad()
def ehem_phase1_packed(model, ctx, pos, plan, table=None):
    d = plan.d
    g = model.geo_feat_generator
    dev = ctx.device
    fused_in = (ctx.dtype == torch.uint8 and g.occ_enc.weight.shape[1] == 16 and g.level_enc.weight.shape[1] == 4
                and g.octant_enc.weight.shape[1] == 4)
    if fused_in:
        x, pos0, occ_self = native.embed_gather(ctx, pos, d["inmap"], g.occ_enc.weight, g.level_enc.weight, g.octant_enc.weight)
        P0 = x.shape[0]
    else:
        pad_ctx = torch.tensor([[0, 0, 255] * 4], dtype=ctx.dtype, device=dev)
        ctx0 = torch.cat((ctx, pad_ctx))[d["inmap"]].long()
        pos0 = torch.cat((pos, torch.zeros((1, 3), dtype=pos.dtype, device=dev)))[d["inmap"]].contiguous()
        P0 = ctx0.shape[0]
        x = torch.cat((F.embedding(ctx0[:, 2:11:3], g.occ_enc.weight).reshape(P0, -1),
                       F.embedding(ctx0[:, 0::3], g.level_enc.weight).reshape(P0, -1),
                       F.embedding(ctx0[:, 1::3], g.octant_enc.weight).reshape(P0, -1)), 1)
        occ_self = ctx0[:, 11]
    ktab = d["knn_tab"]
    c1, c2 = g.conv1[0].weight.shape[0], g.conv2[0].weight.shape[0]
    f2 = torch.empty((P0, c1 + x.shape[1]), dtype=torch.float32, device=dev)
    f2[:, c1:] = x
    pos1 = _edge_conv_packed(g.conv1, pos0, ktab, out=f2[:, :c1])
    x = leaky_mlp3(g.mlp2, x, exact=True)
    f3 = torch.empty((P0, c2 + x.shape[1]), dtype=torch.float32, device=dev)
    f3[:, c2:] = x
    pos2 = _edge_conv_packed(g.conv2, f2, ktab, out=f3[:, :c2])
    pos3 = _edge_conv_packed(g.conv3, f3, ktab, feeds_knn=False)
    nx = g.mlp3[4].weight.shape[0]
    feat = torch.empty((P0, nx + g.edge_mlp2[4].weight.shape[0]), dtype=torch.float32, device=dev)
    leaky_mlp3_s(g.mlp3, native.split_rows(x), out=feat[:, :nx])
    if (pos1.shape[1], pos2.shape[1], pos3.shape[1]) != (64, 128, 256) or feat.shape[1] - nx != 128:
        raise native.ScpError("GeoFeatGenerator: edge features of 64 / 128 / 256 channels expected (models/dgcnn.py:74-119)")
    ew = derived(g, "rowchain_edge", [l.weight for l in (g.edge_mlp1[0], g.edge_mlp1[2], g.edge_mlp1[4], g.edge_mlp2[0], g.edge_mlp2[2], g.edge_mlp2[4])] +
                 [l.bias for l in (g.edge_mlp1[0], g.edge_mlp1[2], g.edge_mlp1[4], g.edge_mlp2[0], g.edge_mlp2[2], g.edge_mlp2[4])],
                 lambda: native.EdgeMlpWeights(g.edge_mlp1, g.edge_mlp2))
    native.geo_edge_mlps(pos1, pos2, pos3, ew, feat[:, nx:])
    hs = _encoder(model.swin_self_transformer, feat, d["self_valid"], d["self_tab"], d["self_merge"], tiles=d.get("self_tiles"))
    feat_a = _mlp_over_concat(model.ancient_mlp, hs, d["self_parent"], grand=d["self_concat"][1]) if HIER else leaky_mlp3_s(model.ancient_mlp, _concat(hs, d["self_concat"]))
    Q0 = d["a1map"].shape[0]
    a1 = native.gather_rows(feat_a, d["a1map"], torch.empty((Q0, 256), dtype=torch.float32, device=dev))
    a2 = native.gather_rows(feat_a, d["a2map"], torch.empty((Q0, 256), dtype=torch.float32, device=dev))
    st = dict(a1=a1, a2=a2, pre_occ=occ_self[d["a1map"]])
    if table is not None:
        _head_to_table(model, a1, d["even_out"], table)
        return None, st
    prob1 = _head3(model, "prob_pred_mlp1", a1)
    return prob1[d["even_rows"]], st


@torch.no_grad()
def ehem_phase2_prepare(model, st, plan):
    d = plan.d
    a1, a2 = st["a1"], st["a2"]
    no = model.pre_occ_mlp[4].weight.shape[0]
    pre = torch.empty((a2.shape[0], no + model.pre_attn_mlp[4].weight.shape[0]), dtype=torch.float32, device=a2.device)
    _head3(model, "pre_attn_mlp", a1, out=pre[:, no:])
    enc = model.swin_cross_transformer
    qs, query = [], a2
    for s, stage in enumerate(enc.layers):
        v1 = d["cross_valid"][s].reshape(-1)
        row = []
        for blk in stage.blocks:
            w, _, qbias, eps_b, _ = _block_consts(blk, True)
            row.append(native.swin_ln_linear(query, w["q"], qbias, eps_b, v1))
        qs.append(row)
        if s < len(enc.layers) - 1:
            query = _merge(stage.downsample, query, d["cross_merge"][s])
    a0 = native.SplitAct.empty(a2.shape[0], 512, a2.device)
    native.split_rows(a2, out=a0.cols(256, 512))
    return dict(pre=pre, q=qs, a0=a0)


def phase2_prep_window(prep, bases, rows):
    return dict(pre=prep["pre"][bases[0]:bases[0] + rows[0]], q=[[q[bases[s]:bases[s] + rows[s]] for q in qs] for s, qs in enumerate(prep["q"])],
                a0=native.SplitAct(prep["a0"].t[:, bases[0]:bases[0] + rows[0]], prep["a0"].K))


@torch.no_grad()
def ehem_phase2_packed(model, st, plan, pre_occ=None, table=None, prep=None):
    d = plan.d
    g = model.geo_feat_generator
    a1, a2 = st["a1"], st["a2"]
    po = st["pre_occ"] if pre_occ is None else pre_occ
    lut = derived(model, "pre_occ_lut", [g.occ_enc.weight] + [model.pre_occ_mlp[i].weight for i in (0, 2, 4)] + [model.pre_occ_mlp[i].bias for i in (0, 2, 4)],
                  lambda: leaky_mlp3(model.pre_occ_mlp, g.occ_enc.weight.detach()).contiguous())
    no = lut.shape[1]
    if prep is not None:
        pre = prep["pre"]
    else:
        pre = torch.empty((a2.shape[0], no + model.pre_attn_mlp[4].weight.shape[0]), dtype=torch.float32, device=a2.device)
        _head3(model, "pre_attn_mlp", a1, out=pre[:, no:])
    native.gather_rows(lut, po, pre[:, :no])
    hc = _encoder(model.swin_cross_transformer, pre, d["cross_valid"], d["cross_tab"], d["cross_merge"], query=a2, tiles=d.get("cross_tiles"),
                  q_pre=None if prep is None else prep["q"])
    if table is not None:
        a = _concat_layer(model.prob_pred_mlp2[0], hc, d["cross_parent"], a2, d["cross_concat"][1], None if prep is None else prep.get("a0")) if HIER else linear_s(_concat(hc, d["cross_concat"], extra=(a2, None)), model.prob_pred_mlp2[0].weight, model.prob_pred_mlp2[0].bias, act="leaky", want="split")
        from ..ops import _split
        a = linear_s(a, model.prob_pred_mlp2[2].weight, model.prob_pred_mlp2[2].bias, act="leaky", want="split")
        native.linear_split_scatter(a, _split(model.prob_pred_mlp2[4].weight), model.prob_pred_mlp2[4].bias, d["odd_out"], table)
        return None
    prob2 = (_mlp_over_concat(model.prob_pred_mlp2, hc, d["cross_parent"], extra=a2, grand=d["cross_concat"][1], a0_pre=None if prep is None else prep.get("a0")) if HIER
             else leaky_mlp3_s(model.prob_pred_mlp2, _concat(hc, d["cross_concat"], extra=(a2, None))))
    return prob2[d["odd_rows"]]


@torch.no_grad()
def ehem_forward_packed(model, ctx, pos, plan, table=None):
    ev, st = ehem_phase1_packed(model, ctx, pos, plan, table=table)
    return ev, ehem_phase2_packed(model, st, plan, table=table)
```

scp_amd/native.py:

```python
import ctypes as C
import os

import numpy as np
import torch

HERE = os.path.dirname(os.path.abspath(__file__))
LIB_PATH = os.path.join(HERE, "libscp_hip.so")
MAX_DEPTH = 21

CART, SPHER, CYLIN = 0, 1, 2
POS_MINMAX, POS_MINMAX_MUL, POS_POW2 = 0, 1, 2
_ERR = {-1: "SCP_EINVAL", -2: "SCP_ENOMEM", -3: "SCP_ESMALL", -4: "SCP_EHIP", -5: "SCP_ESTATE"}


class ScpError(RuntimeError):
    pass


class QuantInfo(C.Structure):
    _fields_ = [("bin_num", C.c_double), ("qs", C.c_double * 3), ("offset", C.c_double * 3),
                ("max_coord", C.c_int32), ("min_coord", C.c_int32)]


class Segment(C.Structure):
    _fields_ = [("point_begin", C.c_int64), ("point_count", C.c_int64), ("path_len", C.c_int32),
                ("path_bits", C.c_int32), ("drop_last", C.c_int32), ("reserved", C.c_int32)]


class SegmentInfo(C.Structure):
    _fields_ = [("depth", C.c_int32), ("max_coord", C.c_int32), ("n_leaves", C.c_int64), ("n_nodes", C.c_int64),
                ("node_base", C.c_int64), ("level_count", C.c_int64 * (MAX_DEPTH + 1))]


_lib = None
_vp = C.c_void_p


ABI_VERSION = 220


def lib():
    global _lib
    if _lib is not None:
        return _lib
    if not os.path.exists(LIB_PATH):
        raise ScpError(f"{LIB_PATH} is missing: run `python scp_amd/build.py` (hipcc, gfx950). "
                       "The SCP hot path has no CPU fallback.")
    L = C.CDLL(LIB_PATH)
    i32, i64 = C.c_int32, C.c_int64
    sig = {
        "scp_version": (C.c_int, []),
        "scp_geo_edge_mlps": (C.c_int, [_vp, i64, _vp, i64, _vp, i64, _vp, _vp, _vp, i64, i32, _vp]),
        "scp_mlp3_rows": (C.c_int, [_vp, i64, i64, _vp, _vp, _vp, _vp, i64, _vp, i32, i32, _vp]),
        "scp_swin_merge": (C.c_int, [_vp, i64, i64, _vp, _vp, _vp, _vp, C.c_float, _vp, i64, i32, _vp]),
        "scp_swin_ln_qkv": (C.c_int, [_vp, i64, _vp, _vp, _vp, _vp, _vp, C.c_float, _vp, i64, _vp, i64, i32, i32, _vp]),
        "scp_swin_kv_planes": (C.c_int, [_vp, _vp, i64, i64, _vp, _vp, _vp, _vp, _vp]),
        "scp_swin_attention_packed_planes": (C.c_int, [_vp, _vp, _vp, _vp, _vp, _vp, _vp, i32, i32, i32, _vp, _vp, _vp, i64, _vp, _vp]),
        "scp_split_rows_f16": (C.c_int, [_vp, i64, i32, i32, _vp, _vp, i64, _vp, _vp, _vp]),
        "scp_linear_split_f16": (C.c_int, [_vp, _vp, i64, _vp, _vp, _vp, _vp, i32, i32, _vp, _vp, i64, _vp, i64, i32, i32, i32, i32, i32, _vp]),
        "scp_last_hip_error": (C.c_int, []),
        "scp_device_count": (C.c_int, []),
        "scp_device_name": (C.c_int, [C.c_char_p, C.c_int]),
        "scp_quantize": (C.c_int, [_vp, i64, i32, C.c_double, C.c_double, _vp, _vp, C.POINTER(QuantInfo), _vp]),
        "scp_geom_create": (C.c_int, [C.POINTER(_vp)]),
        "scp_geom_destroy": (C.c_int, [_vp]),
        "scp_geom_build": (C.c_int, [_vp, _vp, i64, C.POINTER(Segment), i32, C.POINTER(SegmentInfo), _vp]),
        "scp_geom_build_xyz": (C.c_int, [_vp, _vp, _vp, i32, i32, _vp, i32, C.c_double, C.POINTER(Segment), _vp, C.POINTER(QuantInfo),
                                         C.POINTER(SegmentInfo), _vp]),
        "scp_geom_context_ehem_all": (C.c_int, [_vp, i32, i32, i32, _vp, _vp, _vp, _vp, _vp]),
        "scp_geom_emit_nodes": (C.c_int, [_vp, _vp, _vp, _vp, _vp, _vp, _vp]),
        "scp_geom_emit_leaves": (C.c_int, [_vp, i32, _vp, _vp]),
        "scp_geom_krecords_i64": (C.c_int, [_vp, i32, _vp, _vp]),
        "scp_geom_context_ehem": (C.c_int, [_vp, i32, i32, i32, _vp, _vp, _vp, _vp, _vp]),
        "scp_geom_context_octattn": (C.c_int, [_vp, i32, _vp, _vp, _vp, _vp]),
        "scp_knn_topk": (C.c_int, [_vp, i32, i32, i32, i32, _vp, _vp]),
        "scp_knn_topk_packed": (C.c_int, [_vp, _vp, i32, i32, _vp, _vp]),
        "scp_knn_topk_packed_bounded": (C.c_int, [_vp, _vp, i32, i32, _vp, _vp, _vp]),
        "scp_swin_attention_packed": (C.c_int, [_vp, _vp, _vp, _vp, _vp, i32, i32, i32, i32, _vp, _vp]),
        "scp_swin_attention_packed_split": (C.c_int, [_vp, _vp, _vp, _vp, _vp, i32, i32, i32, i32, _vp, _vp, i64, _vp]),
        "scp_set_attention_mode": (C.c_int, [i32]),
        "scp_set_attention_variant": (C.c_int, [i32]),
        "scp_get_attention_variant": (C.c_int, []),
        "scp_ctx_create": (C.c_int, [C.POINTER(_vp)]),
        "scp_ctx_destroy": (C.c_int, [_vp]),
        "scp_ctx_set": (C.c_int, [_vp, i32, i32]),
        "scp_ctx_get": (C.c_int, [_vp, i32]),
        "scp_ctx_make_current": (C.c_int, [_vp]),
        "scp_rc_debug_buffer": (C.c_int, [_vp]),
        "scp_rc_set_wide": (C.c_int, [i32]),
        "scp_prof_enable": (C.c_int, [i32]),
        "scp_prof_count": (C.c_int, []),
        "scp_prof_read": (C.c_int, [i32, _vp, _vp, _vp]),
        "scp_set_knn_mode": (C.c_int, [i32]),
        "scp_row_scale_f16": (C.c_int, [_vp, i64, i32, i32, _vp, _vp, _vp]),
        "scp_row_scale_from_max": (C.c_int, [_vp, i32, _vp, _vp, _vp]),
        "scp_linear_split_f16_max": (C.c_int, [_vp, _vp, i64, _vp, _vp, _vp, _vp, i32, i32, _vp, _vp, i64, _vp, i64, i32, i32, i32, i32, i32, _vp, _vp, i32, i32, i32, _vp]),
        "scp_octattn_attention_f16x3_vmax": (C.c_int, [_vp, _vp, _vp, _vp, _vp, i64, i32, i32, i32, i32, _vp, _vp, _vp, i64, _vp, _vp]),
        "scp_linear_f16x3_scaled": (C.c_int, [_vp, i64, _vp, _vp, _vp, i32, _vp, _vp, i64, _vp, i64, i32, i32, i32, i32, _vp, _vp, _vp]),
        "scp_layernorm_add": (C.c_int, [_vp, _vp, i64, i32, _vp, _vp, C.c_float, _vp, _vp]),
        "scp_layernorm_add_split_f16": (C.c_int, [_vp, _vp, i64, i32, _vp, _vp, C.c_float, _vp, _vp, _vp, i64, _vp, _vp, _vp]),
        "scp_set_knn_workgroup": (C.c_int, [i32]),
        "scp_knn_debug_buffer": (C.c_int, [_vp]),
        "scp_nn_sqdist_f64": (C.c_int, [_vp, i64, _vp, i64, _vp, _vp]),
        "scp_edge_gather_max_ld": (C.c_int, [_vp, i64, _vp, i64, _vp, _vp, _vp, i32, i32, i32, i32, _vp, i32, _vp]),
        "scp_embed_gather": (C.c_int, [_vp, _vp, _vp, i64, _vp, _vp, _vp, _vp, _vp, _vp, i64, _vp]),
        "scp_packed_plan_sizes": (C.c_int, [_vp, i32, _vp]),
        "scp_packed_plan": (C.c_int, [_vp, i32, _vp, _vp, i32, _vp]),
        "scp_decode_expand": (C.c_int, [_vp, _vp, _vp, _vp, _vp, i64, i32, i32, i32, i32, i32, C.c_double, C.c_double, _vp, _vp, _vp, _vp, _vp, _vp, _vp]),
        "scp_edge_gather_max": (C.c_int, [_vp, _vp, _vp, _vp, _vp, i32, i32, i32, i32, _vp, i32, _vp]),
        "scp_swin_attention": (C.c_int, [_vp, _vp, _vp, _vp, i32, i32, i32, i32, i32, _vp, _vp]),
        "scp_octattn_attention": (C.c_int, [_vp, _vp, _vp, _vp, _vp, i32, i32, i32, i32, _vp, _vp, _vp]),
        "scp_octattn_f16x3_ws_bytes": (C.c_int64, [i32, i32, i32]),
        "scp_octattn_embed": (C.c_int, [_vp, _vp, i64, i32, _vp, i32, _vp, i32, i32, _vp, i32, _vp, _vp, i32, _vp, i32, _vp, _vp, _vp, i64, _vp, _vp, _vp]),
        "scp_octattn_attention_f16x3": (C.c_int, [_vp, _vp, _vp, _vp, _vp, i64, i32, i32, i32, i32, _vp, _vp, _vp, i64, _vp]),
        "scp_octattn_attention_rowinv": (C.c_int, [_vp, i64, i64, _vp, _vp, i64, i64, _vp, _vp, i64, i64, _vp, _vp, i64, i64, i32, i32, i32, i32, i32,
                                                   i32, _vp]),
        "scp_decode_expand_octattn": (C.c_int, [_vp, _vp, _vp, _vp, i64, i32, i32, i32, _vp, _vp, _vp, _vp, _vp]),
        "scp_split_weight_bf16": (C.c_int, [_vp, i32, i32, i32, i32, _vp, _vp, _vp]),
        "scp_linear_bf16x3": (C.c_int, [_vp, i64, _vp, _vp, i32, _vp, _vp, i64, _vp, i64, i32, i32, i32, i32, _vp]),
        "scp_split_weight_f16": (C.c_int, [_vp, i32, i32, i32, i32, _vp, _vp, _vp, _vp]),
        "scp_linear_f16x3": (C.c_int, [_vp, i64, _vp, _vp, _vp, i32, _vp, _vp, i64, _vp, i64, i32, i32, i32, i32, _vp, _vp]),
        "scp_linear_split": (C.c_int, [_vp, _vp, i64, _vp, _vp, i32, i32, _vp, _vp, i64, _vp, i64, _vp, _vp, i64, i32, i32, i32, i32, i32, _vp]),
        "scp_tile_weight_bf16": (C.c_int, [_vp, i32, i32, _vp, _vp]),
        "scp_swin_ln_linear": (C.c_int, [_vp, i64, _vp, _vp, _vp, _vp, _vp, C.c_float, _vp, i64, i32, i32, _vp]),
        "scp_swin_post_attn": (C.c_int, [_vp, _vp, i64, _vp, i64, _vp, _vp, _vp, _vp, C.c_float, _vp, i64, i32, _vp, i32, _vp]),
        "scp_swin_post_attn_weight_bytes": (C.c_int64, []),
        "scp_gelu_prescale": (C.c_double, []),
        "scp_split_rows": (C.c_int, [_vp, i64, i64, _vp, i32, _vp, _vp, i64, i64, _vp]),
        "scp_linear_split_scatter": (C.c_int, [_vp, _vp, i64, _vp, _vp, i32, i32, _vp, _vp, _vp, i64, i32, i32, i32, i32, i32, _vp]),
        "scp_linear_split_gather": (C.c_int, [_vp, _vp, i64, _vp, _vp, i32, i32, _vp, _vp, i64, _vp, _vp, i64, _vp, _vp, i64, i32, i32, i32, i32, i32, _vp]),
        "scp_linear_split_hier2": (C.c_int, [_vp, _vp, i64, i32, _vp, _vp, i64, i64, _vp, _vp, _vp, _vp, i32, _vp, _vp, _vp, i64, _vp, _vp, _vp, i64, i32, i32, i32, _vp]),
        "scp_layernorm_rows": (C.c_int, [_vp, i64, i64, _vp, _vp, i32, _vp, _vp, _vp, C.c_float, _vp, i64, i64, _vp]),
        "scp_layernorm_rows_split": (C.c_int, [_vp, i64, i64, _vp, _vp, i32, _vp, _vp, _vp, C.c_float, _vp, _vp, i64, i64, _vp]),
        "scp_gather_rows": (C.c_int, [_vp, i64, _vp, i32, _vp, i64, i64, _vp]),
        "scp_linear_f32": (C.c_int, [_vp, i64, _vp, _vp, _vp, i64, i32, i32, i32, i32, _vp]),
        "scp_softmax_cdf": (C.c_int, [_vp, i64, i64, i32, _vp, _vp, _vp, _vp, _vp]),
        "scp_pmf_cdf": (C.c_int, [_vp, i64, i32, _vp, _vp, _vp, _vp]),
        "scp_ac_encode_cdf": (C.c_int, [_vp, _vp, i64, i32, _vp, C.c_size_t, C.POINTER(C.c_size_t)]),
        "scp_ac_encode_lohi": (C.c_int, [_vp, i64, _vp, C.c_size_t, C.POINTER(C.c_size_t)]),
        "scp_ac_dec_new": (C.c_int, [C.POINTER(_vp), _vp, C.c_size_t, i32]),
        "scp_ac_dec_next": (C.c_int, [_vp, _vp]),
        "scp_ac_dec_run": (C.c_int, [_vp, _vp, i64, _vp]),
        "scp_ac_dec_free": (C.c_int, [_vp]),
    }
    for name, (res, args) in sig.items():
        if hasattr(L, name):
            f = getattr(L, name)
            f.restype = res
            f.argtypes = args
    if L.scp_version() != ABI_VERSION:
        raise ScpError(f"{LIB_PATH} implements ABI {L.scp_version()}, this binding is written for {ABI_VERSION} (include/scp.h: "
                       "SCP_ABI_VERSION; the weight-plane layout differs between versions): rebuild with `python scp_amd/build.py`")
    _lib = L
    return L


def _check(rc, what):
    if rc < 0:
        extra = f" (hipError {lib().scp_last_hip_error()})" if rc == -4 else ""
        raise ScpError(f"{what} failed: {_ERR.get(rc, rc)}{extra}")
    return rc


_RAW_STREAM = getattr(torch._C, "_cuda_getCurrentRawStream", None)
_RAW_DEVICE = getattr(torch._C, "_cuda_getDevice", None)


def _stream():
    if _RAW_STREAM is not None and _RAW_DEVICE is not None:
        return _RAW_STREAM(_RAW_DEVICE())
    return torch.cuda.current_stream().cuda_stream


def _dev(t, dtype=None):
    if not t.is_cuda:
        raise ScpError("device tensor expected (the SCP hot path has no CPU fallback)")
    if dtype is not None and t.dtype != dtype:
        raise ScpError(f"expected {dtype}, got {t.dtype}")
    if not t.is_contiguous():
        raise ScpError("contiguous tensor expected")
    return t.data_ptr()


def _opt(t):
    return None if t is None else _dev(t)


PROF_TAGS = {1: "post_attn", 2: "ln_linear", 3: "attention", 4: "knn_feat", 5: "knn_pos", 6: "gemm_split", 7: "edge_mlp", 8: "merge",
             9: "edge_gather", 10: "cdf", 11: "gemm_f32", 12: "gemm_rows", 13: "split_rows", 14: "layernorm", 15: "oa_attention", 16: "geom",
             17: "other", 18: "mlp3"}


class launch_profile:

    def __enter__(self):
        _check(lib().scp_prof_enable(1), "scp_prof_enable")
        return self

    def __exit__(self, *exc):
        lib().scp_prof_enable(0)
        return False

    def records(self):
        n = _check(lib().scp_prof_count(), "scp_prof_count")
        tags, ms, work = np.zeros(n, np.int32), np.zeros(n, np.float32), np.zeros(n, np.float64)
        if n:
            n = _check(lib().scp_prof_read(n, tags.ctypes.data, ms.ctypes.data, work.ctypes.data), "scp_prof_read")
        return [(PROF_TAGS.get(int(t), str(int(t))), float(m), float(w)) for t, m, w in zip(tags[:n], ms[:n], work[:n])]


def quantize(xyz, mode, qs, cart_offset=-200.0, want_transformed=False):
    n = xyz.shape[0]
    q = torch.empty((n, 3), dtype=torch.int32, device=xyz.device)
    tr = torch.empty((n, 3), dtype=torch.float32, device=xyz.device) if want_transformed else None
    info = QuantInfo()
    rc = lib().scp_quantize(_dev(xyz, torch.float32), n, mode, float(qs), float(cart_offset), _dev(q), _opt(tr),
                            C.byref(info), _stream())
    _check(rc, "scp_quantize")
    return q, info, tr


class Geom:

    def __init__(self):
        self._h = _vp()
        _check(lib().scp_geom_create(C.byref(self._h)), "scp_geom_create")
        self.info = []
        self.device = None

    def close(self):
        if self._h:
            lib().scp_geom_destroy(self._h)
            self._h = _vp()

    def __del__(self):
        try:
            self.close()
        except Exception:
            pass

    def build(self, q, segments):
        nseg = len(segments)
        segs = (Segment * nseg)()
        for i, (b, c, path, drop) in enumerate(segments):
            path = list(path or [])
            bits = 0
            for p in path:
                bits = (bits << 1) | int(p)
            segs[i] = Segment(int(b), int(c), len(path), bits, int(bool(drop)), 0)
        infos = (SegmentInfo * nseg)()
        rc = lib().scp_geom_build(self._h, _dev(q, torch.int32), q.shape[0], segs, nseg, infos, _stream())
        _check(rc, "scp_geom_build")
        self.info = list(infos)
        self.segments = segments
        self.device = q.device
        self.total_nodes = sum(i.n_nodes for i in self.info)
        return self.info

    def build_xyz(self, frames, mode, qs_list, cart_offset, shells, want_q=False):
        nf, ns = len(frames), len(shells)
        if len(qs_list) != ns or nf == 0:
            raise ScpError("build_xyz: one step per shell expected")
        ptrs = (C.c_void_p * nf)(*[_dev(f, torch.float32) for f in frames])
        cnt = (C.c_int64 * nf)(*[int(f.shape[0]) for f in frames])
        qs = (C.c_double * ns)(*[float(q) for q in qs_list])
        segs = (Segment * ns)()
        for i, (path, drop) in enumerate(shells):
            path = list(path or [])
            bits = 0
            for p in path:
                bits = (bits << 1) | int(p)
            segs[i] = Segment(0, 0, len(path), bits, int(bool(drop)), 0)
        nseg = nf * ns
        qinfo, infos = (QuantInfo * nseg)(), (SegmentInfo * nseg)()
        q = torch.empty((sum(int(f.shape[0]) for f in frames) * ns, 3), dtype=torch.int32, device=frames[0].device) if want_q else None
        rc = lib().scp_geom_build_xyz(self._h, ptrs, cnt, nf, mode, qs, ns, float(cart_offset), segs, _opt(q), qinfo, infos, _stream())
        _check(rc, "scp_geom_build_xyz")
        self.info = list(infos)
        self.segments = [(0, int(f.shape[0]), path, drop) for f in frames for (path, drop) in shells]
        self.device = frames[0].device
        self.total_nodes = sum(i.n_nodes for i in self.info)
        return (list(qinfo), q) if want_q else list(qinfo)

    def context_ehem_all(self, pos_mode, lidar_level, context_size):
        R = sum(self.rows(s) for s in range(len(self.info)))
        dev = self.device
        ctx = torch.empty((R, 12), dtype=torch.uint8, device=dev)
        pos = torch.empty((R, 3), dtype=torch.float32, device=dev)
        sym = torch.empty(R, dtype=torch.uint8, device=dev)
        mm = torch.empty((sum(i.depth for i in self.info), 2), dtype=torch.int64, device=dev)
        _check(lib().scp_geom_context_ehem_all(self._h, pos_mode, lidar_level, context_size, _dev(ctx), _dev(pos), _dev(sym), _dev(mm), _stream()),
               "scp_geom_context_ehem_all")
        return ctx, pos, sym, mm

    def level_counts(self, seg):
        i = self.info[seg]
        return [int(i.level_count[l]) for l in range(i.depth)]

    def nodes(self, want=("occ", "level", "octant", "parent", "pos")):
        N, dev = self.total_nodes, self.device
        out = {}
        if "occ" in want:
            out["occ"] = torch.empty(N, dtype=torch.uint8, device=dev)
        if "level" in want:
            out["level"] = torch.empty(N, dtype=torch.uint8, device=dev)
        if "octant" in want:
            out["octant"] = torch.empty(N, dtype=torch.uint8, device=dev)
        if "parent" in want:
            out["parent"] = torch.empty(N, dtype=torch.int32, device=dev)
        if "pos" in want:
            out["pos"] = torch.empty((N, 3), dtype=torch.int32, device=dev)
        rc = lib().scp_geom_emit_nodes(self._h, _opt(out.get("occ")), _opt(out.get("level")), _opt(out.get("octant")),
                                       _opt(out.get("parent")), _opt(out.get("pos")), _stream())
        _check(rc, "scp_geom_emit_nodes")
        return out

    def leaves(self, seg):
        pts = torch.empty((self.info[seg].n_leaves, 3), dtype=torch.int32, device=self.device)
        _check(lib().scp_geom_emit_leaves(self._h, seg, _dev(pts), _stream()), "scp_geom_emit_leaves")
        return pts

    def rows(self, seg):
        return int(self.info[seg].n_nodes) - int(bool(self.segments[seg][3]))

    def krecords(self, seg):
        out = torch.empty((self.rows(seg), 4, 6), dtype=torch.int64, device=self.device)
        _check(lib().scp_geom_krecords_i64(self._h, seg, _dev(out), _stream()), "scp_geom_krecords_i64")
        return out

    def context_ehem(self, seg, pos_mode, lidar_level):
        r, dev = self.rows(seg), self.device
        ctx = torch.empty((r, 12), dtype=torch.uint8, device=dev)
        pos = torch.empty((r, 3), dtype=torch.float32, device=dev)
        sym = torch.empty(r, dtype=torch.uint8, device=dev)
        mm = torch.empty((self.info[seg].depth, 2), dtype=torch.int64, device=dev)
        rc = lib().scp_geom_context_ehem(self._h, seg, pos_mode, lidar_level, _dev(ctx), _dev(pos), _dev(sym), _dev(mm),
                                         _stream())
        _check(rc, "scp_geom_context_ehem")
        return ctx, pos, sym, mm

    def context_octattn(self, seg):
        r, dev = self.rows(seg), self.device
        ctx = torch.empty((r, 12), dtype=torch.uint8, device=dev)
        pos = torch.empty((r, 4, 3), dtype=torch.float32, device=dev)
        sym = torch.empty(r, dtype=torch.uint8, device=dev)
        _check(lib().scp_geom_context_octattn(self._h, seg, _dev(ctx), _dev(pos), _dev(sym), _stream()),
               "scp_geom_context_octattn")
        return ctx, pos, sym


def knn_topk(x, k):
    B, n, Cc = x.shape
    idx = torch.empty((B, n, k), dtype=torch.int32, device=x.device)
    _check(lib().scp_knn_topk(_dev(x, torch.float32), B, n, Cc, k, _dev(idx), _stream()), "scp_knn_topk")
    return idx


def knn_topk_packed(x, ctab, thr0=None):
    T, Cc = x.shape
    idx = torch.zeros((T, 20), dtype=torch.int32, device=x.device)
    if thr0 is None:
        _check(lib().scp_knn_topk_packed(_dev(x, torch.float32), _dev(ctab, torch.int32), T, Cc, _dev(idx), _stream()), "scp_knn_topk_packed")
    else:
        _check(lib().scp_knn_topk_packed_bounded(_dev(x, torch.float32), _dev(ctab, torch.int32), T, Cc, _dev(thr0, torch.float32), _dev(idx),
                                                 _stream()), "scp_knn_topk_packed_bounded")
    return idx


def swin_attention_packed(q, k, v, bias_table, wtab, shift, split=False):
    T = q.shape[0]
    if split:
        o = SplitAct.empty(T, 256, q.device)
        rc = lib().scp_swin_attention_packed_split(q.data_ptr(), k.data_ptr(), v.data_ptr(), _dev(bias_table, torch.float32),
                                                   _dev(wtab, torch.int32), T // 512, shift, q.stride(0), k.stride(0), o.t[0].data_ptr(),
                                                   o.t[1].data_ptr(), o.t.stride(1), _stream())
        _check(rc, "scp_swin_attention_packed_split")
        return o
    out = torch.empty((T, 256), dtype=torch.float32, device=q.device)
    rc = lib().scp_swin_attention_packed(q.data_ptr(), k.data_ptr(), v.data_ptr(), _dev(bias_table, torch.float32),
                                         _dev(wtab, torch.int32), T // 512, shift, q.stride(0), k.stride(0), _dev(out), _stream())
    _check(rc, "scp_swin_attention_packed")
    return out


class KvPlanes:

    __slots__ = ("t",)

    def __init__(self, k=None, v=None, t=None):
        if t is None:
            T = k.shape[0]
            t = torch.empty((4, T, 256), dtype=torch.bfloat16, device=k.device)
            _check(lib().scp_swin_kv_planes(k.data_ptr(), v.data_ptr(), k.stride(0), T, t[0].data_ptr(), t[1].data_ptr(), t[2].data_ptr(),
                                            t[3].data_ptr(), _stream()), "scp_swin_kv_planes")
        self.t = t


def swin_attention_packed_planes(q, kv, bias_table, wtab, shift, split=False, valid=None):
    T = q.shape[0]
    p = kv.t
    vp = None if valid is None else _dev(valid, torch.float32)
    if split:
        o = SplitAct.empty(T, 256, q.device)
        rc = lib().scp_swin_attention_packed_planes(q.data_ptr(), p[0].data_ptr(), p[1].data_ptr(), p[2].data_ptr(), p[3].data_ptr(),
                                                    _dev(bias_table, torch.float32), _dev(wtab, torch.int32), T // 512, shift, q.stride(0), None,
                                                    o.t[0].data_ptr(), o.t[1].data_ptr(), o.t.stride(1), vp, _stream())
        _check(rc, "scp_swin_attention_packed_planes")
        return o
    out = torch.empty((T, 256), dtype=torch.float32, device=q.device)
    rc = lib().scp_swin_attention_packed_planes(q.data_ptr(), p[0].data_ptr(), p[1].data_ptr(), p[2].data_ptr(), p[3].data_ptr(),
                                                _dev(bias_table, torch.float32), _dev(wtab, torch.int32), T // 512, shift, q.stride(0), _dev(out), None,
                                                None, 0, vp, _stream())
    _check(rc, "scp_swin_attention_packed_planes")
    return out


def nn_sqdist(a, b):
    a = _dev_f64(a)
    b = _dev_f64(b)
    out = torch.empty((a.shape[0],), dtype=torch.float64, device=a.device)
    _check(lib().scp_nn_sqdist_f64(a.data_ptr(), a.shape[0], b.data_ptr(), b.shape[0], out.data_ptr(), _stream()), "scp_nn_sqdist_f64")
    return out


def _dev_f64(t):
    if not t.is_cuda:
        raise ScpError("device tensor required (there is no CPU path in the product)")
    return t.to(torch.float64).contiguous()


def embed_gather(ctx, pos, inmap, occ_enc, level_enc, octant_enc):
    rows = inmap.shape[0]
    dev = ctx.device
    x = torch.empty((rows, 80), dtype=torch.float32, device=dev)
    p = torch.empty((rows, 3), dtype=torch.float32, device=dev)
    o = torch.empty((rows,), dtype=torch.int64, device=dev)
    _check(lib().scp_embed_gather(_dev(ctx, torch.uint8), _dev(pos, torch.float32), _dev(inmap, torch.int64), ctx.shape[0], _dev(occ_enc),
                                  _dev(level_enc), _dev(octant_enc), x.data_ptr(), p.data_ptr(), o.data_ptr(), rows, _stream()),
           "scp_embed_gather")
    return x, p, o


_POPC = {}


def decode_expand(sym, pos, anc, octant, L, shift, lv_next, lv_clamp, polar, mn, den):
    dev, n = sym.device, sym.shape[0]
    tab = _POPC.get(dev)
    if tab is None:
        tab = _POPC[dev] = torch.tensor([bin(v).count("1") for v in range(256)], dtype=torch.int64, device=dev)
    cum = torch.cumsum(tab[sym + 1], 0)
    m = int(cum[-1])
    occ8 = torch.empty(n, dtype=torch.uint8, device=dev)
    cpos = torch.empty((m, 3), dtype=torch.int32, device=dev)
    canc = torch.empty((m, 9), dtype=torch.uint8, device=dev)
    coct = torch.empty(m, dtype=torch.uint8, device=dev)
    cctx = torch.empty((m, 12), dtype=torch.uint8, device=dev)
    cposn = torch.empty((m, 3), dtype=torch.float32, device=dev)
    if m == 0:
        return (sym + 1).clamp_(min=0).to(torch.uint8), cpos, canc, coct, cctx, cposn
    _check(lib().scp_decode_expand(_dev(sym, torch.int64), cum.data_ptr(), _dev(pos, torch.int32), _dev(anc, torch.uint8), _dev(octant, torch.uint8), n,
                                   int(L), int(shift), int(lv_next), int(lv_clamp), 1 if polar else 0, float(mn), float(den), cpos.data_ptr(), canc.data_ptr(),
                                   coct.data_ptr(), cctx.data_ptr(), cposn.data_ptr(), occ8.data_ptr(), _stream()), "scp_decode_expand")
    return occ8, cpos, canc, coct, cctx, cposn


def packed_plan(lengths, device):
    import numpy as np
    c = np.ascontiguousarray(np.asarray(lengths, np.int64))
    W = int(c.shape[0])
    rows = np.zeros(11, np.int64)
    _check(lib().scp_packed_plan_sizes(c.ctypes.data, W, rows.ctypes.data), "scp_packed_plan_sizes")
    r = [int(x) for x in rows]
    i64, i32, f32 = torch.int64, torch.int32, torch.float32
    spec = [("inmap", i64, (r[0],)), ("a1map", i64, (r[5],)), ("a2map", i64, (r[5],)), ("even_rows", i64, (r[9],)), ("odd_rows", i64, (r[10],)),
            ("even_dst", i64, (r[9],)), ("odd_dst", i64, (r[10],))]
    for s_ in range(4):
        spec += [(f"sme{s_}", i64, (r[s_ + 1],)), (f"smo{s_}", i64, (r[s_ + 1],))]
    for s_ in range(3):
        spec += [(f"cme{s_}", i64, (r[6 + s_],)), (f"cmo{s_}", i64, (r[6 + s_],))]
    spec += [(f"sc{s_}", i64, (r[0],)) for s_ in range(1, 5)] + [(f"cc{s_}", i64, (r[5],)) for s_ in range(1, 4)]
    spec += [(f"tab{l}", i32, (r[l] // 512, 2)) for l in range(9)] + [("knn_tab", i32, (r[0] // 512, 2))]
    spec += [(f"valid{l}", f32, (r[l], 1)) for l in range(9)]
    spec += [(f"sp{s_}", i64, (r[s_],)) for s_ in range(4)] + [(f"cp{s_}", i64, (r[5 + s_],)) for s_ in range(3)]
    spec += [("even_out", i64, (r[5],)), ("odd_out", i64, (r[5],))]
    t = {name: torch.empty(shape, dtype=dt, device=device) for name, dt, shape in spec}
    ptrs = (C.c_void_p * len(spec))(*[t[name].data_ptr() for name, _, _ in spec])
    scratch = torch.empty((36 * W,), dtype=torch.int64, device=device)
    _check(lib().scp_packed_plan(c.ctypes.data, W, scratch.data_ptr(), ptrs, len(spec), _stream()), "scp_packed_plan")
    d = dict(inmap=t["inmap"], a1map=t["a1map"], a2map=t["a2map"], even_rows=t["even_rows"], odd_rows=t["odd_rows"],
             even_dst=t["even_dst"], odd_dst=t["odd_dst"],
             self_merge=[(t[f"sme{s_}"], t[f"smo{s_}"]) for s_ in range(4)], cross_merge=[(t[f"cme{s_}"], t[f"cmo{s_}"]) for s_ in range(3)],
             self_concat=[t[f"sc{s_}"] for s_ in range(1, 5)], cross_concat=[t[f"cc{s_}"] for s_ in range(1, 4)],
             self_tab=[t[f"tab{l}"] for l in range(5)], cross_tab=[t[f"tab{l}"] for l in range(5, 9)], knn_tab=t["knn_tab"],
             self_valid=[t[f"valid{l}"] for l in range(5)], cross_valid=[t[f"valid{l}"] for l in range(5, 9)],
             self_parent=[t[f"sp{s_}"] for s_ in range(4)], cross_parent=[t[f"cp{s_}"] for s_ in range(3)],
             even_out=t["even_out"], odd_out=t["odd_out"])
    d["self_tiles"], d["cross_tiles"] = real_tiles(c, device)
    return r, d


def real_tiles(lengths, device, n_self=5, n_cross=4):
    import numpy as np
    c = np.asarray(lengths, np.int64)
    e = c + (c & 1)

    def lists(L, n):
        out = []
        for _ in range(n):
            Lp = -(-L // 512) * 512
            base = np.cumsum(Lp) - Lp
            nt = -(-L // 128)
            first = np.repeat(base // 128, nt)
            within = np.arange(int(nt.sum())) - np.repeat(np.cumsum(nt) - nt, nt)
            out.append((first + within).astype(np.int32))
            L = (L + 1) // 2
        return out
    parts = lists(e, n_self) + lists(e // 2, n_cross)
    flat = torch.from_numpy(np.concatenate(parts)).to(device, non_blocking=True)
    cuts = np.cumsum([0] + [len(p) for p in parts])
    views = [flat[cuts[i]:cuts[i + 1]] for i in range(len(parts))]
    return views[:n_self], views[n_self:]


def edge_gather_max_rows(u, v, idx, scale, shift, out=None):
    n, Co = u.shape
    if out is None:
        out = torch.empty((n, Co), dtype=torch.float32, device=u.device)
    elif out.shape != (n, Co) or out.stride(1) != 1 or out.dtype != torch.float32 or out.stride(0) % 4 or out.data_ptr() % 16:
        raise ScpError("edge_gather_max_rows: out must be a float32 [n, C'] view with unit channel stride and 16-byte aligned rows")
    _check(lib().scp_edge_gather_max_ld(u.data_ptr(), u.stride(0), v.data_ptr(), v.stride(0), _dev(idx, torch.int32), _dev(scale), _dev(shift),
                                        1, n, Co, idx.shape[1], out.data_ptr(), out.stride(0), _stream()), "scp_edge_gather_max_ld")
    return out


_MODES = {"knn": "f32" if os.environ.get("SCP_KNN", "")[:1] == "f" else "f16x3",
          "attn": "f32" if os.environ.get("SCP_ATTN", "")[:1] == "f" else "bf16x3"}


def set_knn_mode(f16x3):
    _check(lib().scp_set_knn_mode(1 if f16x3 else 0), "scp_set_knn_mode")
    _MODES["knn"] = "f16x3" if f16x3 else "f32"


def set_knn_workgroup(shape):
    _check(lib().scp_set_knn_workgroup(int(shape)), "scp_set_knn_workgroup")


class NumericProfile:

    def __init__(self, knn_f16x3=True, attention_bf16x3=True):
        self._h = _vp()
        _check(lib().scp_ctx_create(C.byref(self._h)), "scp_ctx_create")
        self.knn_f16x3, self.attention_bf16x3 = bool(knn_f16x3), bool(attention_bf16x3)
        _check(lib().scp_ctx_set(self._h, 1, int(self.knn_f16x3)), "scp_ctx_set")
        _check(lib().scp_ctx_set(self._h, 2, int(self.attention_bf16x3)), "scp_ctx_set")

    def describe(self, model_name):
        return numeric_profile(model_name, self)

    def __del__(self):
        try:
            if self._h:
                lib().scp_ctx_destroy(self._h)
        except Exception:
            pass


_TLS = __import__("threading").local()


def current_profile():
    return getattr(_TLS, "profile", None)


class use_profile:

    def __init__(self, profile):
        self.profile = profile

    def __enter__(self):
        self.prev = current_profile()
        _check(lib().scp_ctx_make_current(self.profile._h if self.profile is not None else None), "scp_ctx_make_current")
        _TLS.profile = self.profile
        return self.profile

    def __exit__(self, *exc):
        lib().scp_ctx_make_current(self.prev._h if self.prev is not None else None)
        _TLS.profile = self.prev
        return False


def attention_bf16x3():
    p = current_profile()
    return (_MODES["attn"] == "bf16x3") if p is None else p.attention_bf16x3


def numeric_profile(model_name, profile="current", decodable=False):
    from . import ops
    from .models import packed
    if model_name == "OctAttention":
        if decodable:
            return f"octattn/1d:gemm={ops.MODE},attn=rowinv32"
        return f"octattn/1:gemm={ops.MODE},attn={OCTATTN_MODE}"
    if profile == "current":
        profile = current_profile()
    knn = _MODES["knn"] if profile is None else ("f16x3" if profile.knn_f16x3 else "f32")
    attn = _MODES["attn"] if profile is None else ("bf16x3" if profile.attention_bf16x3 else "f32")
    L = lib()
    attnv = "" if L.scp_get_attention_variant() == 1 else f",attnv={L.scp_get_attention_variant()}"
    concat = ("hier2" if packed.FUSE2 else "hier") if packed.HIER else "direct"
    heads = "" if packed.CHAIN_HEADS else ",heads=split"
    return f"ehem/6:gemm={ops.MODE},knn={knn},attn={attn},concat={concat},swin=rowchain{heads}{attnv}"


def edge_gather_max(u, v, idx, scale, shift, out=None):
    B, n, Co = u.shape
    k = idx.shape[2]
    if out is None:
        out = torch.empty((B, n, Co), dtype=torch.float32, device=u.device)
    stride = out.stride(1)
    if out.stride(2) != 1 or out.stride(0) != n * stride:
        raise ScpError("edge_gather_max: out must be row-major with unit channel stride")
    rc = lib().scp_edge_gather_max(_dev(u, torch.float32), _dev(v, torch.float32), _dev(idx, torch.int32), _dev(scale),
                                   _dev(shift), B, n, Co, k, out.data_ptr(), stride, _stream())
    _check(rc, "scp_edge_gather_max")
    return out


def set_attention_mode(bf16x3=True):
    _check(lib().scp_set_attention_mode(1 if bf16x3 else 0), "scp_set_attention_mode")
    _MODES["attn"] = "bf16x3" if bf16x3 else "f32"


def swin_attention(q, k, v, bias_table, shift):
    B, Lp, _ = q.shape
    for t in (q, k, v):
        if t.stride(2) != 1 or t.stride(0) != Lp * t.stride(1) or not t.is_cuda or t.dtype != torch.float32:
            raise ScpError("swin_attention: operands must be [B,Lp,256] views with unit channel stride")
    if k.stride(1) != v.stride(1):
        raise ScpError("swin_attention: k and v must share a row stride")
    out = torch.empty((B, Lp, 256), dtype=torch.float32, device=q.device)
    rc = lib().scp_swin_attention(q.data_ptr(), k.data_ptr(), v.data_ptr(), _dev(bias_table, torch.float32), B, Lp, shift,
                                  q.stride(1), k.stride(1), _dev(out), _stream())
    _check(rc, "scp_swin_attention")
    return out


ACT_NONE, ACT_LEAKY, ACT_GELU, ACT_RELU = 0, 1, 2, 3

CACHE_FILLS = 0


def note_cache_fill():
    global CACHE_FILLS
    CACHE_FILLS += 1



WTILE = os.environ.get("SCP_WTILE", "1")[:1] != "0"


def _tile_in_place_of(hi, lo, Npad, Kpad):
    th, tl = torch.empty_like(hi), torch.empty_like(lo)
    for src, dst in ((hi, th), (lo, tl)):
        _check(lib().scp_tile_weight_bf16(src.data_ptr(), Npad, Kpad, dst.data_ptr(), _stream()), "scp_tile_weight_bf16")
    return th, tl


class SplitWeight:

    def __init__(self, w, tiled=None):
        N, K = w.shape
        self.N, self.K = N, K
        self.Npad, self.Kpad = -(-N // 256) * 256, -(-K // 32) * 32
        self.hi = torch.empty((self.Npad, self.Kpad), dtype=torch.bfloat16, device=w.device)
        self.lo = torch.empty_like(self.hi)
        wc = w.detach().contiguous().float()
        _check(lib().scp_split_weight_bf16(_dev(wc), N, K, self.Npad, self.Kpad, _dev(self.hi), _dev(self.lo), _stream()),
               "scp_split_weight_bf16")
        self.tiled_layout = WTILE if tiled is None else bool(tiled)
        if self.tiled_layout:
            self.hi, self.lo = _tile_in_place_of(self.hi, self.lo, self.Npad, self.Kpad)
        note_cache_fill()

    def tiled(self):
        if self.tiled_layout != WTILE:
            raise ScpError("SplitWeight: planes are %s but the library reads %s planes (SCP_WTILE)" % (
                "tiled" if self.tiled_layout else "row-major", "tiled" if WTILE else "row-major"))
        return (self.hi, self.lo)


def linear_bf16x3(x, sw, bias=None, act=ACT_NONE, residual=None, out=None):
    K, N = sw.K, sw.N
    lead = x.shape[:-1]
    x2 = x.reshape(-1, K) if x.is_contiguous() else x
    if x2.dim() != 2:
        x2 = x.contiguous().reshape(-1, K)
    if x2.stride(1) != 1:
        x2 = x2.contiguous()
    M = x2.shape[0]
    if out is None:
        out = torch.empty((M, N), dtype=torch.float32, device=x.device)
        o2 = out
    else:
        o2 = out.reshape(-1, N) if out.is_contiguous() else out
    r2 = None
    if residual is not None:
        r2 = residual.reshape(-1, N) if residual.is_contiguous() else residual.contiguous().reshape(-1, N)
    wt = _tiled_pair(sw)
    rc = lib().scp_linear_bf16x3(x2.data_ptr(), x2.stride(0), wt[0].data_ptr(), wt[1].data_ptr(), sw.Kpad, _opt(bias),
                                 None if r2 is None else r2.data_ptr(), 0 if r2 is None else r2.stride(0), o2.data_ptr(),
                                 o2.stride(0), M, N, K, act, _stream())
    _check(rc, "scp_linear_bf16x3")
    return out.reshape(*lead, N) if out.dim() == 2 and len(lead) != 1 else out


def _tiled_pair(sw):
    if sw.tiled_layout != WTILE:
        raise ScpError("weight planes are not in the layout the library reads (SCP_WTILE)")
    return (sw.hi, sw.lo)


def _tiled_planes_always(sw):
    if sw.tiled_layout:
        return sw.hi, sw.lo
    return _tile_in_place_of(sw.hi, sw.lo, sw.Npad, sw.Kpad)


def _tile_planes(t):
    N, K = t.shape
    v = t.view(N // 16, 16, K // 32, 4, 8).permute(0, 2, 1, 3, 4)
    r = torch.arange(16, device=t.device)
    q = (torch.arange(4, device=t.device)[None, :] ^ ((r[:, None] >> 2) & 3))
    idx = q[None, None, :, :, None].expand(N // 16, K // 32, 16, 4, 8)
    return torch.gather(v, 3, idx).contiguous()


class SplitWeightF16:

    def __init__(self, w):
        N, K = w.shape
        self.N, self.K = N, K
        self.Npad, self.Kpad = -(-N // 256) * 256, -(-K // 32) * 32
        self.hi = torch.empty((self.Npad, self.Kpad), dtype=torch.float16, device=w.device)
        self.lo = torch.empty_like(self.hi)
        self.inv_scale = torch.empty((self.Npad,), dtype=torch.float32, device=w.device)
        wc = w.detach().contiguous().float()
        _check(lib().scp_split_weight_f16(_dev(wc), N, K, self.Npad, self.Kpad, _dev(self.hi), _dev(self.lo), _dev(self.inv_scale),
                                          _stream()), "scp_split_weight_f16")
        self.tiled_layout = WTILE
        if self.tiled_layout:
            self.hi, self.lo = _tile_in_place_of(self.hi, self.lo, self.Npad, self.Kpad)
        note_cache_fill()


class RowScales:

    __slots__ = ("sc", "isc", "x")

    def __init__(self, x2=None, sc=None, isc=None):
        if x2 is not None:
            M, K = x2.shape
            ws = torch.empty((2, M), dtype=torch.float32, device=x2.device)
            _check(lib().scp_row_scale_f16(x2.data_ptr(), x2.stride(0), M, K, ws[0].data_ptr(), ws[1].data_ptr(), _stream()), "scp_row_scale_f16")
            sc, isc = ws[0], ws[1]
        self.sc, self.isc, self.x = sc, isc, x2

    def rows(self, a, b):
        return RowScales(None, self.sc[a:b], self.isc[a:b])

    @staticmethod
    def from_max(row_max):
        M = row_max.shape[0]
        ws = torch.empty((2, M), dtype=torch.float32, device=row_max.device)
        _check(lib().scp_row_scale_from_max(_dev(row_max, torch.int32), M, ws[0].data_ptr(), ws[1].data_ptr(), _stream()), "scp_row_scale_from_max")
        return RowScales(None, ws[0], ws[1])


class SplitActF16:

    __slots__ = ("hi", "lo", "sc", "isc", "K")

    def __init__(self, x2=None, parts=None):
        if x2 is not None:
            M, K = x2.shape
            ld = -(-K // 32) * 32
            pl = torch.empty((2, M, ld), dtype=torch.float16, device=x2.device)
            ws = torch.empty((2, M), dtype=torch.float32, device=x2.device)
            _check(lib().scp_split_rows_f16(x2.data_ptr(), x2.stride(0), M, K, pl[0].data_ptr(), pl[1].data_ptr(), ld, ws[0].data_ptr(), ws[1].data_ptr(),
                                            _stream()), "scp_split_rows_f16")
            parts = (pl[0], pl[1], ws[0], ws[1], K)
        self.hi, self.lo, self.sc, self.isc, self.K = parts

    @property
    def M(self):
        return self.hi.shape[0]

    def rows(self, a, b):
        return SplitActF16(parts=(self.hi[a:b], self.lo[a:b], self.sc[a:b], self.isc[a:b], self.K))


def linear_split_f16(a, sw, bias=None, act=ACT_NONE, residual=None, cfg=0, out=None, row_max=None, col_max=None):
    if not sw.tiled_layout and WTILE:
        raise ScpError("linear_split_f16: weight planes are not tiled")
    M, N = a.M, sw.N
    if a.K != sw.K:
        raise ScpError("linear_split_f16: K mismatch")
    if out is None:
        out = torch.empty((M, N), dtype=torch.float32, device=a.hi.device)
    r2 = None
    if residual is not None:
        r2 = residual.reshape(-1, N)
        if r2.stride(1) != 1:
            r2 = r2.contiguous()
    if row_max is not None or col_max is not None:
        if row_max is not None and (row_max.dtype != torch.int32 or row_max.shape[0] != M or not row_max.is_contiguous()):
            raise ScpError("linear_split_f16: row_max must be a contiguous int32 [M]")
        cm, lo, hi, rows = col_max if col_max is not None else (None, 0, 0, 0)
        rc = lib().scp_linear_split_f16_max(a.hi.data_ptr(), a.lo.data_ptr(), a.hi.stride(0), a.isc.data_ptr(), sw.hi.data_ptr(), sw.lo.data_ptr(),
                                            sw.inv_scale.data_ptr(), sw.Npad, sw.Kpad, _opt(bias), None if r2 is None else r2.data_ptr(),
                                            0 if r2 is None else r2.stride(0), out.data_ptr(), out.stride(0), M, N, sw.K, act, cfg,
                                            None if row_max is None else row_max.data_ptr(), None if cm is None else _dev(cm, torch.int32), int(lo), int(hi), int(rows),
                                            _stream())
        _check(rc, "scp_linear_split_f16_max")
        return out
    rc = lib().scp_linear_split_f16(a.hi.data_ptr(), a.lo.data_ptr(), a.hi.stride(0), a.isc.data_ptr(), sw.hi.data_ptr(), sw.lo.data_ptr(),
                                    sw.inv_scale.data_ptr(), sw.Npad, sw.Kpad, _opt(bias), None if r2 is None else r2.data_ptr(),
                                    0 if r2 is None else r2.stride(0), out.data_ptr(), out.stride(0), M, N, sw.K, act, cfg, _stream())
    _check(rc, "scp_linear_split_f16")
    return out


def _rows_f16x3(x, K):
    x2 = x.reshape(-1, K)
    if x2.stride(1) != 1 or (x2.stride(0) & 3) or (x2.data_ptr() & 15):
        x2 = x2.contiguous()
    return x2


def linear_f16x3(x, sw, bias=None, act=ACT_NONE, residual=None, scales=None):
    K, N = sw.K, sw.N
    lead = x.shape[:-1]
    x2 = _rows_f16x3(x, K)
    M = x2.shape[0]
    out = torch.empty((M, N), dtype=torch.float32, device=x.device)
    r2 = None
    if residual is not None:
        r2 = residual.reshape(-1, N)
        if r2.stride(1) != 1:
            r2 = r2.contiguous()
    if scales is not None:
        if scales.sc.shape[0] != M:
            raise ScpError("linear_f16x3: row scales of another row count")
        rc = lib().scp_linear_f16x3_scaled(x2.data_ptr(), x2.stride(0), _tiled_pair(sw)[0].data_ptr(), _tiled_pair(sw)[1].data_ptr(), sw.inv_scale.data_ptr(), sw.Kpad,
                                           _opt(bias), None if r2 is None else r2.data_ptr(), 0 if r2 is None else r2.stride(0), out.data_ptr(),
                                           out.stride(0), M, N, K, act, scales.sc.data_ptr(), scales.isc.data_ptr(), _stream())
        _check(rc, "scp_linear_f16x3_scaled")
        return out.reshape(*lead, N)
    ws = torch.empty((2 * M,), dtype=torch.float32, device=x.device)
    rc = lib().scp_linear_f16x3(x2.data_ptr(), x2.stride(0), _tiled_pair(sw)[0].data_ptr(), _tiled_pair(sw)[1].data_ptr(), sw.inv_scale.data_ptr(), sw.Kpad,
                                _opt(bias), None if r2 is None else r2.data_ptr(), 0 if r2 is None else r2.stride(0), out.data_ptr(),
                                out.stride(0), M, N, K, act, ws.data_ptr(), _stream())
    _check(rc, "scp_linear_f16x3")
    return out.reshape(*lead, N)


class SplitAct:

    __slots__ = ("t", "K")

    def __init__(self, t, K):
        self.t, self.K = t, K

    @staticmethod
    def empty(M, K, device):
        return SplitAct(torch.empty((2, M, -(-K // 32) * 32), dtype=torch.bfloat16, device=device), K)

    @property
    def M(self):
        return self.t.shape[1]

    def cols(self, c0, c1):
        return SplitAct(self.t[:, :, c0:c1], c1 - c0)

    def float(self):
        return self.t[0, :, :self.K].float() + self.t[1, :, :self.K].float()


def linear_split_scatter(a, sw, bias, out_map, table, act=ACT_NONE, cfg=0):
    t = a.t
    N = sw.N
    if N % 4 and table.stride(0) >= -(-N // 4) * 4 and act == ACT_NONE:
        Np = -(-N // 4) * 4
        if bias is not None:
            pb = getattr(sw, "_bias_pad", None)
            ver = (bias._version, bias.data_ptr())
            if pb is None or pb[0] is not bias or pb[2] != ver:
                pb = (bias, torch.cat((bias.detach().float(), torch.zeros(Np - N, dtype=torch.float32, device=bias.device))).contiguous(), ver)
                sw._bias_pad = pb
                note_cache_fill()
            bias = pb[1]
        N = Np
    _check(lib().scp_linear_split_scatter(t[0].data_ptr(), t[1].data_ptr(), t.stride(1), sw.tiled()[0].data_ptr(), sw.tiled()[1].data_ptr(), sw.Npad, sw.Kpad,
                                          _opt(bias), _dev(out_map, torch.int64), table.data_ptr(), table.stride(0), a.M, N, sw.K, act, cfg,
                                          _stream()), "scp_linear_split_scatter")


def split_rows(x, idx=None, out=None):
    Cc = x.shape[1]
    rows = x.shape[0] if idx is None else idx.shape[0]
    if out is None:
        out = SplitAct.empty(rows, Cc, x.device)
    if x.stride(1) != 1:
        x = x.contiguous()
    t = out.t
    _check(lib().scp_split_rows(x.data_ptr(), x.stride(0), x.shape[0], _opt(idx), Cc, t[0].data_ptr(), t[1].data_ptr(), t.stride(1), rows,
                                _stream()), "scp_split_rows")
    return out


def linear_split(a, sw, bias=None, act=ACT_NONE, residual=None, out=None, out_split=None, want="f32", cfg=0, res_map=None, res_first=False):
    M, N, K = a.M, sw.N, sw.K
    if a.K != K:
        raise ScpError("linear_split: K mismatch %d vs %d" % (a.K, K))
    t = a.t
    c = o = None
    if want in ("f32", "both"):
        c = out if out is not None else torch.empty((M, N), dtype=torch.float32, device=t.device)
    if want in ("split", "both"):
        o = out_split if out_split is not None else SplitAct.empty(M, N, t.device)
    r2 = residual
    if res_map is not None or res_first:
        rc = lib().scp_linear_split_gather(t[0].data_ptr(), t[1].data_ptr(), t.stride(1), sw.tiled()[0].data_ptr(), sw.tiled()[1].data_ptr(), sw.Npad, sw.Kpad,
                                           _opt(bias), None if r2 is None else r2.data_ptr(), 0 if r2 is None else r2.stride(0),
                                           None if res_map is None else _dev(res_map, torch.int64),
                                           None if c is None else c.data_ptr(), 0 if c is None else c.stride(0),
                                           None if o is None else o.t[0].data_ptr(), None if o is None else o.t[1].data_ptr(),
                                           0 if o is None else o.t.stride(1), M, N, K, act, cfg, _stream())
        _check(rc, "scp_linear_split_gather")
        return c if want == "f32" else (o if want == "split" else (c, o))
    rc = lib().scp_linear_split(t[0].data_ptr(), t[1].data_ptr(), t.stride(1), sw.tiled()[0].data_ptr(), sw.tiled()[1].data_ptr(), sw.Npad, sw.Kpad, _opt(bias),
                                None if r2 is None else r2.data_ptr(), 0 if r2 is None else r2.stride(0),
                                None if c is None else c.data_ptr(), 0 if c is None else c.stride(0),
                                None if o is None else o.t[0].data_ptr(), None if o is None else o.t[1].data_ptr(),
                                0 if o is None else o.t.stride(1), M, N, K, act, cfg, _stream())
    _check(rc, "scp_linear_split")
    return c if want == "f32" else (o if want == "split" else (c, o))


def linear_split_hier2(a0, sw0, a1, sw1, parent, bias=None, act=ACT_NONE, residual=None, res_map=None, out_split=None):
    if not WTILE:
        raise ScpError("linear_split_hier2 reads tiled weight planes (SCP_WTILE=0 is not supported by it)")
    M, N = a0.M, sw0.N
    if a0.K != sw0.K or a1.K != sw1.K or sw1.K != 256 or sw1.N != N or sw1.Npad != sw0.Npad or parent.shape[0] != M:
        raise ScpError("linear_split_hier2: operand shapes do not match")
    o = out_split if out_split is not None else SplitAct.empty(M, N, a0.t.device)
    t0, t1 = a0.t, a1.t
    rc = lib().scp_linear_split_hier2(t0[0].data_ptr(), t0[1].data_ptr(), t0.stride(1), sw0.Kpad, t1[0].data_ptr(), t1[1].data_ptr(), t1.stride(1), a1.M,
                                      sw0.tiled()[0].data_ptr(), sw0.tiled()[1].data_ptr(), sw1.tiled()[0].data_ptr(), sw1.tiled()[1].data_ptr(), sw0.Npad,
                                      _dev(parent, torch.int64), _opt(bias), None if residual is None else residual.data_ptr(),
                                      0 if residual is None else residual.stride(0), None if (residual is None or res_map is None) else _dev(res_map, torch.int64),
                                      o.t[0].data_ptr(), o.t[1].data_ptr(), o.t.stride(1), M, N, act, _stream())
    _check(rc, "scp_linear_split_hier2")
    return o


class LnFoldedWeight:

    def __init__(self, w, gamma, beta):
        w64 = w.detach().double()
        self.sw = SplitWeight((w64 * gamma.detach().double()[None, :]).float())
        self.planes = _tiled_planes_always(self.sw)
        self.wbeta = (w64 @ beta.detach().double()).float().contiguous()
        self.N, self.K = self.sw.N, self.sw.K
        note_cache_fill()


def swin_ln_linear(x, fw, bias, eps=1e-5, valid=None, out=None):
    M = x.shape[0]
    if x.shape[1] != 256 or fw.K != 256 or x.stride(1) != 1:
        raise ScpError("swin_ln_linear: 256-channel rows expected")
    if out is None:
        out = torch.empty((M, fw.N), dtype=torch.float32, device=x.device)
    t = fw.planes
    rc = lib().scp_swin_ln_linear(x.data_ptr(), x.stride(0), None if valid is None else _dev(valid, torch.float32), t[0].data_ptr(), t[1].data_ptr(),
                                  _opt(bias), _dev(fw.wbeta), float(eps), out.data_ptr(), out.stride(0), M, fw.N, _stream())
    _check(rc, "scp_swin_ln_linear")
    return out


def swin_ln_qkv(x, fw, bias, eps=1e-5, valid=None):
    M = x.shape[0]
    if x.shape[1] != 256 or fw.K != 256 or x.stride(1) != 1 or fw.N not in (512, 768) or (M & 127):
        raise ScpError("swin_ln_qkv: 256-channel rows in multiples of 128, N = 768 or 512 expected")
    q = torch.empty((M, 256), dtype=torch.float32, device=x.device) if fw.N == 768 else None
    pl = torch.empty((4, M, 256), dtype=torch.bfloat16, device=x.device)
    t = fw.planes
    rc = lib().scp_swin_ln_qkv(x.data_ptr(), x.stride(0), None if valid is None else _dev(valid, torch.float32), t[0].data_ptr(), t[1].data_ptr(),
                               _opt(bias), _dev(fw.wbeta), float(eps), None if q is None else q.data_ptr(), 256, pl.data_ptr(), M, M, fw.N, _stream())
    _check(rc, "scp_swin_ln_qkv")
    return q, KvPlanes(t=pl)


class EdgeMlpWeights:

    def __init__(self, mlp1, mlp2):
        w11, w12, w13 = (mlp1[i].weight.detach().float() for i in (0, 2, 4))
        w21, w22, w23 = (mlp2[i].weight.detach().float() for i in (0, 2, 4))
        if tuple(w11.shape) != (256, 448) or tuple(w12.shape) != (256, 256) or tuple(w13.shape) != (256, 256) or tuple(w21.shape) != (256, 512) or \
                tuple(w22.shape) != (256, 256) or tuple(w23.shape) != (128, 256):
            raise ScpError("EdgeMlpWeights: unexpected layer shapes")
        dev = w11.device
        P = rc_perm16(256, dev)
        z = torch.zeros((256, 64), dtype=torch.float32, device=dev)
        mats = [w11[:, :256], torch.cat((w11[:, 256:], z), 1), w12[:, P], w13[:, P], w21[:, 256:][:, P], w21[:, :256], w22[:, P],
                torch.cat((w23[:, P], torch.zeros((128, 256), dtype=torch.float32, device=dev)), 0)]
        nbytes = lib().scp_swin_post_attn_weight_bytes()
        buf = torch.zeros((nbytes // 2,), dtype=torch.bfloat16, device=dev)
        half = nbytes // 4
        for m, w in enumerate(mats):
            hi, lo = _tiled_planes_always(SplitWeight(w.contiguous()))
            buf[m * 65536:(m + 1) * 65536] = hi.reshape(-1)[:65536]
            buf[half + m * 65536:half + (m + 1) * 65536] = lo.reshape(-1)[:65536]
        self.packed = buf
        self.bias = torch.cat([mlp1[i].bias.detach().float() for i in (0, 2, 4)] + [mlp2[i].bias.detach().float() for i in (0, 2, 4)]).contiguous()
        note_cache_fill()


def geo_edge_mlps(pos1, pos2, pos3, ew, out):
    M = pos1.shape[0]
    if pos1.shape[1] != 64 or pos2.shape[1] != 128 or pos3.shape[1] != 256 or pos1.stride(1) != 1 or pos2.stride(1) != 1 or pos3.stride(1) != 1 or out.stride(1) != 1:
        raise ScpError("geo_edge_mlps: [M, 64], [M, 128], [M, 256] rows expected")
    rc = lib().scp_geo_edge_mlps(pos1.data_ptr(), pos1.stride(0), pos2.data_ptr(), pos2.stride(0), pos3.data_ptr(), pos3.stride(0), ew.packed.data_ptr(),
                                 ew.bias.data_ptr(), out.data_ptr(), out.stride(0), M, _stream())
    _check(rc, "scp_geo_edge_mlps")
    return out


class Mlp3Weights:

    def __init__(self, seq):
        ws = [seq[i].weight.detach().float() for i in (0, 2, 4)]
        bs = [seq[i].bias.detach().float() for i in (0, 2, 4)]
        if ws[0].shape[1] != 256 or any(w.shape[0] > 256 or w.shape[1] > 256 for w in ws) or ws[1].shape[1] != ws[0].shape[0] or ws[2].shape[1] != ws[1].shape[0]:
            raise ScpError("Mlp3Weights: a 256 -> (<= 256) -> (<= 256) -> (<= 256) head expected")
        dev = ws[0].device
        P = rc_perm16(256, dev)
        nbytes = lib().scp_swin_post_attn_weight_bytes()
        buf = torch.zeros((nbytes // 2,), dtype=torch.bfloat16, device=dev)
        half = nbytes // 4
        bias = torch.zeros((3, 256), dtype=torch.float32, device=dev)
        for m, (w, b) in enumerate(zip(ws, bs)):
            full = torch.zeros((256, 256), dtype=torch.float32, device=dev)
            full[:w.shape[0], :w.shape[1]] = w
            if m:
                full = full[:, P]
            hi, lo = _tiled_planes_always(SplitWeight(full.contiguous()))
            buf[m * 65536:(m + 1) * 65536] = hi.reshape(-1)[:65536]
            buf[half + m * 65536:half + (m + 1) * 65536] = lo.reshape(-1)[:65536]
            bias[m, :b.shape[0]] = b
        self.packed, self.bias, self.N = buf, bias.reshape(-1).contiguous(), int(ws[2].shape[0])
        note_cache_fill()


def mlp3_rows(x, mw, out, in_map=None, out_map=None, ncols=None):
    M = x.shape[0] if in_map is None else in_map.shape[0]
    if out_map is not None and out_map.shape[0] != M:
        raise ScpError("mlp3_rows: out_map must have one entry per row")
    if x.shape[1] != 256 or x.stride(1) != 1 or out.stride(1) != 1:
        raise ScpError("mlp3_rows: [n, 256] rows with unit channel stride expected")
    N = -(-mw.N // 4) * 4 if ncols is None else int(ncols)
    if out_map is None and out.shape[0] < M:
        raise ScpError("mlp3_rows: output has too few rows")
    _check(lib().scp_mlp3_rows(x.data_ptr(), x.stride(0), x.shape[0], None if in_map is None else _dev(in_map, torch.int64), mw.packed.data_ptr(), mw.bias.data_ptr(),
                               out.data_ptr(), out.stride(0), None if out_map is None else _dev(out_map, torch.int64), M, N, _stream()), "scp_mlp3_rows")
    return out


class MergeWeights:

    def __init__(self, w, gamma, beta):
        w64 = w.detach().double()
        wf = (w64 * gamma.detach().double()[None, :]).float()
        self.wbeta = (w64 @ beta.detach().double()).float().contiguous()
        nbytes = lib().scp_swin_post_attn_weight_bytes()
        buf = torch.zeros((nbytes // 2,), dtype=torch.bfloat16, device=w.device)
        half = nbytes // 4
        for kh in range(2):
            hi, lo = _tiled_planes_always(SplitWeight(wf[:, 256 * kh:256 * (kh + 1)].contiguous()))
            buf[kh * 65536:(kh + 1) * 65536] = hi.reshape(-1)[:65536]
            buf[half + kh * 65536:half + (kh + 1) * 65536] = lo.reshape(-1)[:65536]
        self.packed = buf
        note_cache_fill()


def swin_merge(x, ia, ib, mw, eps=1e-5):
    M = ia.shape[0]
    if x.shape[1] != 256 or x.stride(1) != 1:
        raise ScpError("swin_merge: 256-channel rows expected")
    out = torch.empty((M, 256), dtype=torch.float32, device=x.device)
    rc = lib().scp_swin_merge(x.data_ptr(), x.stride(0), x.shape[0], _dev(ia, torch.int64), _dev(ib, torch.int64), mw.packed.data_ptr(), _dev(mw.wbeta),
                              float(eps), out.data_ptr(), out.stride(0), M, _stream())
    _check(rc, "scp_swin_merge")
    return out


def rc_perm16(n, device):
    p = torch.arange(n, device=device)
    q = p & 15
    return (p & ~15) | (q & 3) | ((q & 4) << 1) | ((q & 8) >> 1)


class PostAttnWeights:

    def __init__(self, wp, bp, gamma, beta, w1, b1, w2, b2):
        dev = wp.device
        perm_k, perm_h = rc_perm16(256, dev), rc_perm16(w1.shape[0], dev)
        w1d = w1.detach().double()
        s = float(lib().scp_gelu_prescale())
        swp = SplitWeight(wp.detach().float().contiguous())
        sw1 = SplitWeight((w1d * gamma.detach().double()[None, :] * s).float()[:, perm_k].contiguous())
        sw2 = SplitWeight((w2.detach().double() / s).float()[:, perm_h].contiguous())
        tiles = [_tiled_planes_always(w) for w in (swp, sw1, sw2)]
        self.packed = torch.cat([t[0].reshape(-1) for t in tiles] + [t[1].reshape(-1) for t in tiles]).contiguous()
        if self.packed.numel() * 2 != lib().scp_swin_post_attn_weight_bytes():
            raise ScpError("swin_post_attn: 256 -> 1024 -> 256 blocks only")
        self.bp = bp.detach().float().contiguous()
        self.b1 = ((b1.detach().double() + w1d @ beta.detach().double()) * s).float().contiguous()
        self.b2 = b2.detach().float().contiguous()
        note_cache_fill()


def swin_post_attn(o, x, pw, eps=1e-5, out=None, tiles=None):
    M = x.shape[0]
    if o.K != 256 or o.M != M or x.shape[1] != 256 or x.stride(1) != 1:
        raise ScpError("swin_post_attn: [M, 256] operands expected")
    if out is None:
        out = torch.empty((M, 256), dtype=torch.float32, device=x.device)
    t = o.t
    rc = lib().scp_swin_post_attn(t[0].data_ptr(), t[1].data_ptr(), t.stride(1), x.data_ptr(), x.stride(0), pw.packed.data_ptr(), _dev(pw.bp),
                                  _dev(pw.b1), _dev(pw.b2), float(eps), out.data_ptr(), out.stride(0), M,
                                  None if tiles is None else _dev(tiles, torch.int32), 0 if tiles is None else int(tiles.shape[0]), _stream())
    _check(rc, "scp_swin_post_attn")
    return out


def layernorm_rows(x, gamma, beta, eps=1e-5, valid=None, ia=None, ib=None, out=None, split=False):
    Cc = gamma.shape[0]
    rows = x.shape[0] if ia is None else ia.shape[0]
    if split:
        o = SplitAct.empty(rows, Cc, x.device)
        rc = lib().scp_layernorm_rows_split(x.data_ptr(), x.stride(0), x.shape[0], None if ia is None else _dev(ia, torch.int64),
                                            None if ib is None else _dev(ib, torch.int64), Cc, _dev(gamma), _dev(beta),
                                            None if valid is None else _dev(valid, torch.float32), float(eps), o.t[0].data_ptr(),
                                            o.t[1].data_ptr(), o.t.stride(1), rows, _stream())
        _check(rc, "scp_layernorm_rows_split")
        return o
    if out is None:
        out = torch.empty((rows, Cc), dtype=torch.float32, device=x.device)
    rc = lib().scp_layernorm_rows(x.data_ptr(), x.stride(0), x.shape[0], None if ia is None else _dev(ia, torch.int64),
                                  None if ib is None else _dev(ib, torch.int64), Cc, _dev(gamma), _dev(beta),
                                  None if valid is None else _dev(valid, torch.float32), float(eps), out.data_ptr(), out.stride(0),
                                  rows, _stream())
    _check(rc, "scp_layernorm_rows")
    return out


def layernorm_add(a, b, gamma, beta, eps=1e-5, planes=False):
    Cc = a.shape[-1]
    if not a.is_contiguous() or (b is not None and (not b.is_contiguous() or b.shape != a.shape)):
        raise ScpError("layernorm_add: contiguous operands of one shape expected")
    out = torch.empty_like(a)
    if planes:
        M, ld = a.numel() // Cc, -(-Cc // 32) * 32
        pl = torch.empty((2, M, ld), dtype=torch.float16, device=a.device)
        ws = torch.empty((2, M), dtype=torch.float32, device=a.device)
        _check(lib().scp_layernorm_add_split_f16(_dev(a, torch.float32), None if b is None else _dev(b, torch.float32), M, Cc, _dev(gamma), _dev(beta),
                                                 float(eps), out.data_ptr(), pl[0].data_ptr(), pl[1].data_ptr(), ld, ws[0].data_ptr(), ws[1].data_ptr(),
                                                 _stream()), "scp_layernorm_add_split_f16")
        return out, SplitActF16(parts=(pl[0], pl[1], ws[0], ws[1], Cc))
    _check(lib().scp_layernorm_add(_dev(a, torch.float32), None if b is None else _dev(b, torch.float32), a.numel() // Cc, Cc, _dev(gamma), _dev(beta),
                                   float(eps), out.data_ptr(), _stream()), "scp_layernorm_add")
    return out


def gather_rows(src, idx, out):
    Cc = out.shape[1]
    rc = lib().scp_gather_rows(src.data_ptr(), src.stride(0), _dev(idx, torch.int64), Cc, out.data_ptr(), out.stride(0), idx.shape[0],
                               _stream())
    _check(rc, "scp_gather_rows")
    return out


def linear_f32(x, w, bias=None, act=ACT_NONE):
    K = w.shape[1]
    N = w.shape[0]
    lead = x.shape[:-1]
    x2 = x.reshape(-1, K) if x.is_contiguous() else x.contiguous().reshape(-1, K)
    M = x2.shape[0]
    out = torch.empty((M, N), dtype=torch.float32, device=x.device)
    wc = w if w.is_contiguous() else w.contiguous()
    rc = lib().scp_linear_f32(x2.data_ptr(), x2.stride(0), _dev(wc.detach(), torch.float32), _opt(bias), out.data_ptr(), N, M, N, K, act,
                              _stream())
    _check(rc, "scp_linear_f32")
    return out.reshape(*lead, N)


OCTATTN_MODE = os.environ.get("SCP_OCTATTN", "f16x3")


def octattn_attention(q_u, k, k_u, v, v_u, heads, out=None, out_u=None, vmax=None):
    B, c, D = q_u.shape
    if out is None:
        out, out_u = torch.empty_like(q_u), torch.empty_like(q_u)
    elif not (out.is_contiguous() and out_u.is_contiguous() and out.shape == q_u.shape and out_u.shape == q_u.shape):
        raise ScpError("octattn_attention: out / out_u must be contiguous [B, c, D] float32")
    hd = D // heads
    ld = k.stride(-2)
    strided_ok = all(t.is_cuda and t.dtype == torch.float32 and t.stride(-1) == 1 and t.stride(-2) == ld and (t.dim() == 2 or t.stride(0) == c * ld)
                     for t in (k, k_u, v, v_u))
    if OCTATTN_MODE == "f16x3" and hd == 150 and (D & 3) == 0 and strided_ok:
        nb = lib().scp_octattn_f16x3_ws_bytes(B, c, heads)
        ws = torch.empty((nb + 1024,), dtype=torch.uint8, device=q_u.device)
        off = (-ws.data_ptr()) % 1024
        if vmax is not None:
            rc = lib().scp_octattn_attention_f16x3_vmax(_dev(q_u), k.data_ptr(), k_u.data_ptr(), v.data_ptr(), v_u.data_ptr(), ld, B, c, heads, hd, _dev(out),
                                                        _dev(out_u), ws.data_ptr() + off, nb, _dev(vmax, torch.int32), _stream())
            _check(rc, "scp_octattn_attention_f16x3_vmax")
            return out, out_u
        rc = lib().scp_octattn_attention_f16x3(_dev(q_u), k.data_ptr(), k_u.data_ptr(), v.data_ptr(), v_u.data_ptr(), ld, B, c, heads, hd, _dev(out),
                                               _dev(out_u), ws.data_ptr() + off, nb, _stream())
        _check(rc, "scp_octattn_attention_f16x3")
        return out, out_u
    k, k_u, v, v_u = (t.contiguous() for t in (k, k_u, v, v_u))
    rc = lib().scp_octattn_attention(_dev(q_u), _dev(k), _dev(k_u), _dev(v), _dev(v_u), B, c, heads, hd,
                                     _dev(out), _dev(out_u), _stream())
    _check(rc, "scp_octattn_attention")
    return out, out_u


def _win_strides(t):
    if not (t.is_cuda and t.dtype == torch.float32 and t.stride(-1) == 1):
        raise ScpError("octattn_attention_rowinv: float32 device tensors with unit channel stride expected")
    return (t.stride(0) if t.dim() == 3 else 0), t.stride(-2)


def octattn_attention_rowinv(q_u, k, v, heads, k_u=None, v_u=None, out=None, out_u=None, q0=0, q1=None, qoff=0):
    D = q_u.shape[-1]
    B = q_u.shape[0] if q_u.dim() == 3 else 1
    q1 = (q_u.shape[-2] + qoff) if q1 is None else q1
    if out is None and out_u is None:
        raise ScpError("octattn_attention_rowinv: nothing to compute (out and out_u are None)")
    if q1 > k.shape[-2] or q1 - qoff > q_u.shape[-2]:
        raise ScpError("octattn_attention_rowinv: query range beyond the key rows")
    for t in (out, out_u, k_u, v_u):
        if t is not None and t.shape[-2] < q1 - qoff:
            raise ScpError("octattn_attention_rowinv: operand shorter than the query range")
    qw, qr = _win_strides(q_u)
    kw, kr = _win_strides(k)
    if _win_strides(v) != (kw, kr):
        raise ScpError("octattn_attention_rowinv: k and v must share their strides")
    uw = ur = 0
    if out_u is not None:
        uw, ur = _win_strides(k_u)
        if _win_strides(v_u) != (uw, ur):
            raise ScpError("octattn_attention_rowinv: k_u and v_u must share their strides")
    ow, orr = _win_strides(out if out is not None else out_u)
    if out is not None and out_u is not None and _win_strides(out_u) != (ow, orr):
        raise ScpError("octattn_attention_rowinv: out and out_u must share their strides")
    ptr = lambda t: None if t is None else t.data_ptr()
    rc = lib().scp_octattn_attention_rowinv(q_u.data_ptr(), qw, qr, k.data_ptr(), v.data_ptr(), kw, kr, ptr(k_u), ptr(v_u), uw, ur, ptr(out),
                                            ptr(out_u), ow, orr, B, int(q0), int(q1), int(qoff), int(heads), D // heads, _stream())
    _check(rc, "scp_octattn_attention_rowinv")
    return out, out_u


def decode_expand_octattn(sym, ctx, apos, L, depth):
    dev, n = sym.device, sym.shape[0]
    tab = _POPC.get(dev)
    if tab is None:
        tab = _POPC[dev] = torch.tensor([bin(v).count("1") for v in range(256)], dtype=torch.int64, device=dev)
    cum = torch.cumsum(tab[sym + 1], 0)
    m = int(cum[-1])
    occ8 = torch.empty(n, dtype=torch.uint8, device=dev)
    cctx = torch.empty((m, 12), dtype=torch.uint8, device=dev)
    capos = torch.empty((m, 4, 3), dtype=torch.int32, device=dev)
    cpos = torch.empty((m, 4, 3), dtype=torch.float32, device=dev)
    if m == 0:
        return (sym + 1).clamp_(min=0).to(torch.uint8), cctx, capos, cpos
    _check(lib().scp_decode_expand_octattn(_dev(sym, torch.int64), cum.data_ptr(), _dev(ctx, torch.uint8), _dev(apos, torch.int32), n, int(L),
                                           int(depth - L), int(depth), cctx.data_ptr(), capos.data_ptr(), cpos.data_ptr(), occ8.data_ptr(), _stream()),
           "scp_decode_expand_octattn")
    return occ8, cctx, capos, cpos


def octattn_embed(ctx, pos, c, occ_enc, level_enc, octant_enc, pos_w, pos_b, pe, level_cap, max_level):
    n = ctx.shape[0]
    d_occ, d_lvl, d_oct = occ_enc.shape[1], level_enc.shape[1], octant_enc.shape[1]
    d_pos = 0 if pos_w is None else pos_w.shape[0]
    D = 4 * (d_occ + d_lvl + d_oct + d_pos)
    ld = -(-D // 32) * 32
    dev = ctx.device
    E = torch.empty((2, n, D), dtype=torch.float32, device=dev)
    pl = torch.empty((2, 2 * n, ld), dtype=torch.float16, device=dev)
# ... 85 lines not shown
```

Before: 15.57 frames/s.

## Skip LN-QKV GEMM on padding tiles and stamp precomputed pad planes

Swin LN+linear and LN+QKV kernels now take a list of real 128-row tiles and run the GEMM only on those, so tiles that hold only window padding are not computed. For the KV planes, padding tiles are filled by copying a precomputed image of one all-padding tile (zero input, zero validity), which keeps attention inputs identical. This removes redundant matmul work on padded rows, at the cost of indirect tile lookup and extra copy traffic for the pad tiles. It is enabled by default through SCP_PAD_SKIP.

Result: no change. 15.72 frames/s (median of 6 runs) (+0.9%).

```diff
diff --git a/include/scp.h b/include/scp.h
--- a/include/scp.h
+++ b/include/scp.h
@@ -236,6 +236,9 @@
 
 SCP_API int scp_swin_ln_linear(const float *x, int64_t ldx, const float *valid, const void *Whi, const void *Wlo, const float *bias,
                                const float *wbeta, float eps, float *out, int64_t ldo, int32_t M, int32_t N, void *stream);
+SCP_API int scp_swin_ln_linear_tiles(const float *x, int64_t ldx, const float *valid, const void *Whi, const void *Wlo, const float *bias,
+                                     const float *wbeta, float eps, float *out, int64_t ldo, int32_t M, int32_t N, const int32_t *tile_list,
+                                     int32_t n_list, void *stream);
 SCP_API int scp_swin_post_attn(const void *Ohi, const void *Olo, int64_t ldo_in, const float *x, int64_t ldx, const void *W, const float *bp,
                                const float *b1, const float *b2, float eps, float *out, int64_t ldc, int32_t M, const int32_t *tile_list,
                                int32_t n_tiles, void *stream);
@@ -253,6 +256,10 @@
 SCP_API int scp_swin_kv_planes(const float *k, const float *v, int64_t ldkv, int64_t rows, void *khi, void *klo, void *vthi, void *vtlo, void *stream);
 SCP_API int scp_swin_ln_qkv(const float *x, int64_t ldx, const float *valid, const void *Whi, const void *Wlo, const float *bias, const float *wbeta,
                             float eps, float *q, int64_t ldq, void *planes, int64_t Tp, int32_t M, int32_t N, void *stream);
+SCP_API int scp_swin_ln_qkv_tiles(const float *x, int64_t ldx, const float *valid, const void *Whi, const void *Wlo, const float *bias,
+                                  const float *wbeta, float eps, float *q, int64_t ldq, void *planes, int64_t Tp, int32_t M, int32_t N,
+                                  const int32_t *tile_list, int32_t n_list, const int32_t *pad_list, int32_t n_pad, const void *pad_img,
+                                  void *stream);
 SCP_API int scp_swin_attention_packed_planes(const float *q, const void *khi, const void *klo, const void *vthi, const void *vtlo,
                                              const float *bias_table, const int32_t *wtab, int32_t total_windows, int32_t shift, int32_t ldq,
                                              float *out, void *ohi, void *olo, int64_t ldo, const float *valid, void *stream);
diff --git a/scp_amd/csrc/rowchain.hip b/scp_amd/csrc/rowchain.hip
--- a/scp_amd/csrc/rowchain.hip
+++ b/scp_amd/csrc/rowchain.hip
@@ -143,6 +143,9 @@
     unsigned long long *dbg;
     __bf16 *planes; int64_t plane_bytes; int nq;
     int ngroups;
+    const int32_t *tile_list; int n_list;
+    const int32_t *pad_list; int n_pad;
+    const __bf16 *pad_img;
 };
 
 #define RC_DS_WRITE(addr, val, off) asm volatile("ds_write_b128 %0, %1 offset:%2" :: "v"(addr), "v"(val), "n"(off) : "memory")
@@ -299,10 +302,27 @@
     }
     __syncthreads();
     const int ngr = a.ngroups > 1 ? a.ngroups : 1;
-    int tile = blockIdx.x / ngr;
+    const int nlist = a.tile_list ? a.n_list : ntiles;
+    auto tile_of = [&](int i) { return a.tile_list ? a.tile_list[i] : i; };
+    int ti = blockIdx.x / ngr;
     const int tstride = (int)gridDim.x / ngr;
     const int j0 = (int)(blockIdx.x % ngr) * (nsteps / ngr), j1 = j0 + nsteps / ngr;
-    if (tile >= ntiles) return;
+    if (KV && a.n_pad > 0) {
+        const int64_t pb = a.plane_bytes;
+        for (int p = (int)gridDim.x - 1 - (int)blockIdx.x; p < a.n_pad; p += (int)gridDim.x) {
+            const int pt = a.pad_list[p];
+            if ((unsigned)pt >= (unsigned)ntiles) continue;
+            char *dst = (char *)a.planes + (int64_t)pt * (RC_ROWS * 512);
+            const char *src = (const char *)a.pad_img;
+#pragma unroll 4
+            for (int i = threadIdx.x; i < 4 * 4096; i += 256) {
+                const int part = i >> 12, off = (i & 4095) * 16;
+                *(ri32x4 *)(dst + part * pb + off) = *(const ri32x4 *)(src + part * (RC_ROWS * 512) + off);
+            }
+        }
+    }
+    if (ti >= nlist) return;
+    int tile = tile_of(ti);
     char *bounce = smem + RC_OFF_BOUNCE + L.w * RC_BOUNCE;
     unsigned bw[4];
 #pragma unroll
@@ -346,7 +366,8 @@
         RC_DS_READ4_WAIT(A[0][1], ad0, 16384, A[0][3], ad0, RC_SLOT + 16384, A[0][0], ad0, 0, A[0][2], ad0, RC_SLOT);
     }
     int gstep = 0;
-    for (; tile < ntiles; tile += tstride) {
+    for (; ti < nlist; ti += tstride) {
+        tile = tile_of(ti);
         const int m0 = tile * RC_ROWS;
         const int row = m0 + 32 * L.w + L.col;
         const int rowc = row < a.M ? row : a.M - 1;
@@ -368,8 +389,8 @@
         const int64_t rows_left = (int64_t)a.M - m0;
         const int64_t span = (rows_left < RC_ROWS ? rows_left : RC_ROWS) * a.ldo * 4;
         const __amdgpu_buffer_rsrc_t rs = (a.probe & 1) ? rs_none : __builtin_amdgcn_make_buffer_rsrc(a.out + (int64_t)m0 * a.ldo, 0, (int)span, 0x00020000);
-        const bool more = tile + tstride < ntiles;
-        const float *xnext = xrow(more ? tile + tstride : tile);
+        const bool more = ti + tstride < nlist;
+        const float *xnext = xrow(more ? tile_of(ti + tstride) : tile);
 
         rf32x16 acc[2][2];
 #pragma unroll
@@ -1571,10 +1592,12 @@
     return g_rc_num_cu;
 }
 
-extern "C" SCP_API int scp_swin_ln_linear(const float *x, int64_t ldx, const float *valid, const void *Whi, const void *Wlo, const float *bias,
-                                          const float *wbeta, float eps, float *out, int64_t ldo, int32_t M, int32_t N, void *stream) {
+static int rc_ln_linear_launch(const float *x, int64_t ldx, const float *valid, const void *Whi, const void *Wlo, const float *bias,
+                               const float *wbeta, float eps, float *out, int64_t ldo, int32_t M, int32_t N, const int32_t *tile_list, int32_t n_list,
+                               void *stream) {
     if (!x || !Whi || !Wlo || !out || M <= 0 || N <= 0 || (N & 127) || N > 1024 || ldx < 256 || (ldx & 3) || ldo < N || (ldo & 3) ||
-        (((uintptr_t)x | (uintptr_t)out | (uintptr_t)Whi | (uintptr_t)Wlo) & 15) || (int64_t)RC_ROWS * ldo * 4 > 0x7fffffffLL)
+        (((uintptr_t)x | (uintptr_t)out | (uintptr_t)Whi | (uintptr_t)Wlo) & 15) || (int64_t)RC_ROWS * ldo * 4 > 0x7fffffffLL ||
+        (tile_list && (n_list <= 0 || n_list > (M + RC_ROWS - 1) / RC_ROWS)))
         return SCP_EINVAL;
     static bool configured = false;
     if (!configured) {
@@ -1585,23 +1608,38 @@
     a.x = x; a.ldx = ldx; a.valid = valid; a.Whi = (const __bf16 *)Whi; a.Wlo = (const __bf16 *)Wlo; a.bias = bias; a.wbeta = wbeta;
     a.out = out; a.ldo = ldo; a.M = M; a.N = N; a.eps = eps;
     a.planes = nullptr; a.plane_bytes = 0; a.nq = 0;
+    a.tile_list = tile_list; a.n_list = tile_list ? n_list : 0; a.pad_list = nullptr; a.n_pad = 0; a.pad_img = nullptr;
     { static int pr = -1; if (pr < 0) { const char *e = getenv("SCP_RC_PROBE"); pr = e ? atoi(e) : 0; } a.probe = pr; }
     if (a.probe) { const char *e = getenv("SCP_RC_PROBE"); a.probe = e ? atoi(e) : 0; }
     a.dbg = g_rc_dbg;
-    const int ntiles = (M + RC_ROWS - 1) / RC_ROWS;
+    const int ntiles = tile_list ? n_list : (M + RC_ROWS - 1) / RC_ROWS;
     const int ncu = rc_num_cu();
-    SCP_PROF(SCP_PROF_LN_LINEAR, stream, 2.0 * M * 256.0 * N);
+    SCP_PROF(SCP_PROF_LN_LINEAR, stream, 2.0 * (tile_list ? (double)n_list * RC_ROWS : (double)M) * 256.0 * N);
     a.ngroups = rc_ll_groups(ntiles, N / 64, ncu);
     hipLaunchKernelGGL(rc_ln_linear_kernel<0>, dim3((unsigned)(a.ngroups > 1 ? ntiles * a.ngroups : (ntiles < ncu ? ntiles : ncu))), dim3(256), RC_LDS, (hipStream_t)stream, a);
     LAUNCH_CHECK();
     return SCP_OK;
 }
 
-extern "C" SCP_API int scp_swin_ln_qkv(const float *x, int64_t ldx, const float *valid, const void *Whi, const void *Wlo, const float *bias,
-                                       const float *wbeta, float eps, float *q, int64_t ldq, void *planes, int64_t Tp, int32_t M, int32_t N, void *stream) {
+extern "C" SCP_API int scp_swin_ln_linear(const float *x, int64_t ldx, const float *valid, const void *Whi, const void *Wlo, const float *bias,
+                                          const float *wbeta, float eps, float *out, int64_t ldo, int32_t M, int32_t N, void *stream) {
+    return rc_ln_linear_launch(x, ldx, valid, Whi, Wlo, bias, wbeta, eps, out, ldo, M, N, nullptr, 0, stream);
+}
+
+extern "C" SCP_API int scp_swin_ln_linear_tiles(const float *x, int64_t ldx, const float *valid, const void *Whi, const void *Wlo, const float *bias,
+                                                const float *wbeta, float eps, float *out, int64_t ldo, int32_t M, int32_t N, const int32_t *tile_list,
+                                                int32_t n_list, void *stream) {
+    if (!tile_list) return SCP_EINVAL;
+    return rc_ln_linear_launch(x, ldx, valid, Whi, Wlo, bias, wbeta, eps, out, ldo, M, N, tile_list, n_list, stream);
+}
+
+static int rc_ln_qkv_launch(const float *x, int64_t ldx, const float *valid, const void *Whi, const void *Wlo, const float *bias,
+                            const float *wbeta, float eps, float *q, int64_t ldq, void *planes, int64_t Tp, int32_t M, int32_t N,
+                            const int32_t *tile_list, int32_t n_list, const int32_t *pad_list, int32_t n_pad, const void *pad_img, void *stream) {
     if (!x || !Whi || !Wlo || !planes || M <= 0 || (M & 127) || (N != 768 && N != 512) || (N == 768 && (!q || ldq < 256 || (ldq & 3))) || ldx < 256 ||
-        (ldx & 3) || Tp < M || (Tp & 31) || (((uintptr_t)x | (uintptr_t)q | (uintptr_t)Whi | (uintptr_t)Wlo | (uintptr_t)planes) & 15) ||
-        (q && (int64_t)RC_ROWS * ldq * 4 > 0x7fffffffLL) || 4 * Tp * 512 > 0x7fffffffLL)
+        (ldx & 3) || Tp < M || (Tp & 31) || (((uintptr_t)x | (uintptr_t)q | (uintptr_t)Whi | (uintptr_t)Wlo | (uintptr_t)planes | (uintptr_t)pad_img) & 15) ||
+        (q && (int64_t)RC_ROWS * ldq * 4 > 0x7fffffffLL) || 4 * Tp * 512 > 0x7fffffffLL ||
+        (tile_list && (n_list <= 0 || n_pad < 0 || (n_pad > 0 && (!pad_list || !pad_img)) || (int64_t)n_list + n_pad != M / RC_ROWS)))
         return SCP_EINVAL;
     static bool configured = false;
     if (!configured) {
@@ -1612,12 +1650,27 @@
     a.x = x; a.ldx = ldx; a.valid = valid; a.Whi = (const __bf16 *)Whi; a.Wlo = (const __bf16 *)Wlo; a.bias = bias; a.wbeta = wbeta;
     a.out = q; a.ldo = q ? ldq : 256; a.M = M; a.N = N; a.eps = eps; a.probe = 0; a.dbg = nullptr;
     a.planes = (__bf16 *)planes; a.plane_bytes = Tp * 512; a.nq = N / 64 - 8;
-    const int ntiles = M / RC_ROWS, ncu = rc_num_cu();
-    SCP_PROF(SCP_PROF_LN_LINEAR, stream, 2.0 * M * 256.0 * N);
+    a.tile_list = tile_list; a.n_list = tile_list ? n_list : 0;
+    a.pad_list = tile_list ? pad_list : nullptr; a.n_pad = tile_list ? n_pad : 0; a.pad_img = (const __bf16 *)pad_img;
+    const int ntiles = tile_list ? n_list : M / RC_ROWS, ncu = rc_num_cu();
+    SCP_PROF(SCP_PROF_LN_LINEAR, stream, 2.0 * (double)ntiles * RC_ROWS * 256.0 * N);
     a.ngroups = rc_ll_groups(ntiles, N / 64, ncu);
     hipLaunchKernelGGL((rc_ln_linear_kernel<0, true>), dim3((unsigned)(a.ngroups > 1 ? ntiles * a.ngroups : (ntiles < ncu ? ntiles : ncu))), dim3(256), RC_LDS, (hipStream_t)stream, a);
     LAUNCH_CHECK();
     return SCP_OK;
+}
+
+extern "C" SCP_API int scp_swin_ln_qkv(const float *x, int64_t ldx, const float *valid, const void *Whi, const void *Wlo, const float *bias,
+                                       const float *wbeta, float eps, float *q, int64_t ldq, void *planes, int64_t Tp, int32_t M, int32_t N, void *stream) {
+    return rc_ln_qkv_launch(x, ldx, valid, Whi, Wlo, bias, wbeta, eps, q, ldq, planes, Tp, M, N, nullptr, 0, nullptr, 0, nullptr, stream);
+}
+
+extern "C" SCP_API int scp_swin_ln_qkv_tiles(const float *x, int64_t ldx, const float *valid, const void *Whi, const void *Wlo, const float *bias,
+                                             const float *wbeta, float eps, float *q, int64_t ldq, void *planes, int64_t Tp, int32_t M, int32_t N,
+                                             const int32_t *tile_list, int32_t n_list, const int32_t *pad_list, int32_t n_pad, const void *pad_img,
+                                             void *stream) {
+    if (!tile_list) return SCP_EINVAL;
+    return rc_ln_qkv_launch(x, ldx, valid, Whi, Wlo, bias, wbeta, eps, q, ldq, planes, Tp, M, N, tile_list, n_list, pad_list, n_pad, pad_img, stream);
 }
 
 extern "C" SCP_API int scp_swin_post_attn(const void *Ohi, const void *Olo, int64_t ldo_in, const float *x, int64_t ldx, const void *W, const float *bp,
diff --git a/scp_amd/models/packed.py b/scp_amd/models/packed.py
--- a/scp_amd/models/packed.py
+++ b/scp_amd/models/packed.py
@@ -125,6 +125,8 @@
                    post=native.PostAttnWeights(proj.weight, proj.bias, lna.weight, lna.bias, fc1.weight, fc1.bias, fc2.weight, fc2.bias))
         if cross:
             out["q"] = native.LnFoldedWeight(att.query.weight, lnb.weight, lnb.bias)
+        if native.attention_bf16x3():
+            out["kv_pad"] = native.swin_ln_qkv_pad_image(out["kv"], b, lnb.eps, device=W.device)
         return out
     return derived(layer, "rowchain+" if cross else "rowchain", srcs, build)
 
@@ -142,16 +144,21 @@
     return out
 
 
-def _swin_layer_rowchain(layer, x, valid, wtab, shift, query=None, tiles=None, q_pre=None):
+PAD_SKIP = __import__("os").environ.get("SCP_PAD_SKIP", "1")[:1] != "0"
+
+
+def _swin_layer_rowchain(layer, x, valid, wtab, shift, query=None, tiles=None, q_pre=None, pad_tiles=None):
     cross = query is not None
     w, table, qbias, eps_b, eps_a = _block_consts(layer, cross)
     v1 = None if valid is None else valid.reshape(-1)
     if native.attention_bf16x3():
+        skip = PAD_SKIP and tiles is not None and pad_tiles is not None and tiles.shape[0] > 0 and "kv_pad" in w
+        kw = dict(tiles=tiles, pad_tiles=pad_tiles, pad_image=w["kv_pad"]) if skip else {}
         if not cross:
-            q, kvp = native.swin_ln_qkv(x, w["kv"], w["b"], eps_b, v1)
+            q, kvp = native.swin_ln_qkv(x, w["kv"], w["b"], eps_b, v1, **kw)
         else:
-            q = q_pre if q_pre is not None else native.swin_ln_linear(query, w["q"], qbias, eps_b, v1)
-            _, kvp = native.swin_ln_qkv(x, w["kv"], w["b"], eps_b, v1)
+            q = q_pre if q_pre is not None else native.swin_ln_linear(query, w["q"], qbias, eps_b, v1, tiles=tiles if skip else None)
+            _, kvp = native.swin_ln_qkv(x, w["kv"], w["b"], eps_b, v1, **kw)
         o = native.swin_attention_packed_planes(q, kvp, table, wtab, shift, split=True, valid=v1 if tiles is not None else None)
         if tiles is not None and tiles.shape[0] > 0:
             return native.swin_post_attn(o, x, w["post"], eps_a, out=x, tiles=tiles)
@@ -168,11 +175,11 @@
     return native.swin_post_attn(o, x, w["post"], layer.layernorm_after.eps)
 
 
-def _swin_layer(layer, x, valid, wtab, shift, query=None, tiles=None, q_pre=None):
+def _swin_layer(layer, x, valid, wtab, shift, query=None, tiles=None, q_pre=None, pad_tiles=None):
     fc1, fc2 = layer.intermediate.dense, layer.output.dense
     if x.shape[1] != 256 or fc1.weight.shape != (1024, 256) or fc2.weight.shape != (256, 1024):
         raise native.ScpError("EHEM's Swin blocks are 256 wide with a 1024-wide MLP (configs/model/ehem.yaml); other widths are not built")
-    return _swin_layer_rowchain(layer, x, valid, wtab, shift, query, tiles, q_pre)
+    return _swin_layer_rowchain(layer, x, valid, wtab, shift, query, tiles, q_pre, pad_tiles)
 
 
 def _merge(m, x, maps):
@@ -184,12 +191,12 @@
     return native.swin_merge(x, ev, od, mw, m.norm.eps)
 
 
-def _encoder(enc, x, valids, tabs, merges, query=None, tiles=None, q_pre=None):
+def _encoder(enc, x, valids, tabs, merges, query=None, tiles=None, q_pre=None, pad_tiles=None):
     hs = [x]
     for s, stage in enumerate(enc.layers):
         for b, blk in enumerate(stage.blocks):
             x = _swin_layer(blk, x, valids[s], tabs[s], SHIFT if b % 2 else 0, query, None if tiles is None else tiles[s],
-                            None if q_pre is None else q_pre[s][b])
+                            None if q_pre is None else q_pre[s][b], None if tiles is None or pad_tiles is None else pad_tiles[s])
         hs.append(x)
         if s < len(enc.layers) - 1:
             x = _merge(stage.downsample, x, merges[s])
@@ -315,7 +322,8 @@
                  [l.bias for l in (g.edge_mlp1[0], g.edge_mlp1[2], g.edge_mlp1[4], g.edge_mlp2[0], g.edge_mlp2[2], g.edge_mlp2[4])],
                  lambda: native.EdgeMlpWeights(g.edge_mlp1, g.edge_mlp2))
     native.geo_edge_mlps(pos1, pos2, pos3, ew, feat[:, nx:])
-    hs = _encoder(model.swin_self_transformer, feat, d["self_valid"], d["self_tab"], d["self_merge"], tiles=d.get("self_tiles"))
+    hs = _encoder(model.swin_self_transformer, feat, d["self_valid"], d["self_tab"], d["self_merge"], tiles=d.get("self_tiles"),
+                  pad_tiles=d.get("self_pad_tiles"))
     feat_a = _mlp_over_concat(model.ancient_mlp, hs, d["self_parent"], grand=d["self_concat"][1]) if HIER else leaky_mlp3_s(model.ancient_mlp, _concat(hs, d["self_concat"]))
     Q0 = d["a1map"].shape[0]
     a1 = native.gather_rows(feat_a, d["a1map"], torch.empty((Q0, 256), dtype=torch.float32, device=dev))
@@ -337,12 +345,14 @@
     _head3(model, "pre_attn_mlp", a1, out=pre[:, no:])
     enc = model.swin_cross_transformer
     qs, query = [], a2
+    ct = d.get("cross_tiles") if PAD_SKIP and d.get("cross_pad_tiles") is not None else None
     for s, stage in enumerate(enc.layers):
         v1 = d["cross_valid"][s].reshape(-1)
+        tl = None if ct is None or ct[s].shape[0] == 0 else ct[s]
         row = []
         for blk in stage.blocks:
             w, _, qbias, eps_b, _ = _block_consts(blk, True)
-            row.append(native.swin_ln_linear(query, w["q"], qbias, eps_b, v1))
+            row.append(native.swin_ln_linear(query, w["q"], qbias, eps_b, v1, tiles=tl))
         qs.append(row)
         if s < len(enc.layers) - 1:
             query = _merge(stage.downsample, query, d["cross_merge"][s])
@@ -372,7 +382,7 @@
         _head3(model, "pre_attn_mlp", a1, out=pre[:, no:])
     native.gather_rows(lut, po, pre[:, :no])
     hc = _encoder(model.swin_cross_transformer, pre, d["cross_valid"], d["cross_tab"], d["cross_merge"], query=a2, tiles=d.get("cross_tiles"),
-                  q_pre=None if prep is None else prep["q"])
+                  q_pre=None if prep is None else prep["q"], pad_tiles=d.get("cross_pad_tiles"))
     if table is not None:
         a = _concat_layer(model.prob_pred_mlp2[0], hc, d["cross_parent"], a2, d["cross_concat"][1], None if prep is None else prep.get("a0")) if HIER else linear_s(_concat(hc, d["cross_concat"], extra=(a2, None)), model.prob_pred_mlp2[0].weight, model.prob_pred_mlp2[0].bias, act="leaky", want="split")
         from ..ops import _split
diff --git a/scp_amd/native.py b/scp_amd/native.py
--- a/scp_amd/native.py
+++ b/scp_amd/native.py
@@ -54,6 +54,7 @@
         "scp_mlp3_rows": (C.c_int, [_vp, i64, i64, _vp, _vp, _vp, _vp, i64, _vp, i32, i32, _vp]),
         "scp_swin_merge": (C.c_int, [_vp, i64, i64, _vp, _vp, _vp, _vp, C.c_float, _vp, i64, i32, _vp]),
         "scp_swin_ln_qkv": (C.c_int, [_vp, i64, _vp, _vp, _vp, _vp, _vp, C.c_float, _vp, i64, _vp, i64, i32, i32, _vp]),
+        "scp_swin_ln_qkv_tiles": (C.c_int, [_vp, i64, _vp, _vp, _vp, _vp, _vp, C.c_float, _vp, i64, _vp, i64, i32, i32, _vp, i32, _vp, i32, _vp, _vp]),
         "scp_swin_kv_planes": (C.c_int, [_vp, _vp, i64, i64, _vp, _vp, _vp, _vp, _vp]),
         "scp_swin_attention_packed_planes": (C.c_int, [_vp, _vp, _vp, _vp, _vp, _vp, _vp, i32, i32, i32, _vp, _vp, _vp, i64, _vp, _vp]),
         "scp_split_rows_f16": (C.c_int, [_vp, i64, i32, i32, _vp, _vp, i64, _vp, _vp, _vp]),
@@ -123,6 +124,7 @@
         "scp_linear_split": (C.c_int, [_vp, _vp, i64, _vp, _vp, i32, i32, _vp, _vp, i64, _vp, i64, _vp, _vp, i64, i32, i32, i32, i32, i32, _vp]),
         "scp_tile_weight_bf16": (C.c_int, [_vp, i32, i32, _vp, _vp]),
         "scp_swin_ln_linear": (C.c_int, [_vp, i64, _vp, _vp, _vp, _vp, _vp, C.c_float, _vp, i64, i32, i32, _vp]),
+        "scp_swin_ln_linear_tiles": (C.c_int, [_vp, i64, _vp, _vp, _vp, _vp, _vp, C.c_float, _vp, i64, i32, i32, _vp, i32, _vp]),
         "scp_swin_post_attn": (C.c_int, [_vp, _vp, i64, _vp, i64, _vp, _vp, _vp, _vp, C.c_float, _vp, i64, i32, _vp, i32, _vp]),
         "scp_swin_post_attn_weight_bytes": (C.c_int64, []),
         "scp_gelu_prescale": (C.c_double, []),
@@ -496,31 +498,39 @@
              self_valid=[t[f"valid{l}"] for l in range(5)], cross_valid=[t[f"valid{l}"] for l in range(5, 9)],
              self_parent=[t[f"sp{s_}"] for s_ in range(4)], cross_parent=[t[f"cp{s_}"] for s_ in range(3)],
              even_out=t["even_out"], odd_out=t["odd_out"])
-    d["self_tiles"], d["cross_tiles"] = real_tiles(c, device)
+    d["self_tiles"], d["cross_tiles"], d["self_pad_tiles"], d["cross_pad_tiles"] = real_tiles(c, device, with_pad=True)
     return r, d
 
 
-def real_tiles(lengths, device, n_self=5, n_cross=4):
+def real_tiles(lengths, device, n_self=5, n_cross=4, with_pad=False):
     import numpy as np
     c = np.asarray(lengths, np.int64)
     e = c + (c & 1)
 
     def lists(L, n):
-        out = []
+        out, pads = [], []
         for _ in range(n):
             Lp = -(-L // 512) * 512
             base = np.cumsum(Lp) - Lp
             nt = -(-L // 128)
             first = np.repeat(base // 128, nt)
             within = np.arange(int(nt.sum())) - np.repeat(np.cumsum(nt) - nt, nt)
-            out.append((first + within).astype(np.int32))
+            real = (first + within).astype(np.int32)
+            out.append(real)
+            keep = np.ones(int(Lp.sum()) // 128, bool)
+            keep[real] = False
+            pads.append(np.flatnonzero(keep).astype(np.int32))
             L = (L + 1) // 2
-        return out
-    parts = lists(e, n_self) + lists(e // 2, n_cross)
+        return out, pads
+    (rs, ps), (rc, pc) = lists(e, n_self), lists(e // 2, n_cross)
+    parts = rs + rc + (ps + pc if with_pad else [])
     flat = torch.from_numpy(np.concatenate(parts)).to(device, non_blocking=True)
     cuts = np.cumsum([0] + [len(p) for p in parts])
     views = [flat[cuts[i]:cuts[i + 1]] for i in range(len(parts))]
-    return views[:n_self], views[n_self:]
+    n = n_self + n_cross
+    if with_pad:
+        return views[:n_self], views[n_self:n], views[n:n + n_self], views[n + n_self:]
+    return views[:n_self], views[n_self:n]
 
 
 def edge_gather_max_rows(u, v, idx, scale, shift, out=None):
@@ -977,30 +987,47 @@
         note_cache_fill()
 
 
-def swin_ln_linear(x, fw, bias, eps=1e-5, valid=None, out=None):
+def swin_ln_linear(x, fw, bias, eps=1e-5, valid=None, out=None, tiles=None):
     M = x.shape[0]
     if x.shape[1] != 256 or fw.K != 256 or x.stride(1) != 1:
         raise ScpError("swin_ln_linear: 256-channel rows expected")
     if out is None:
         out = torch.empty((M, fw.N), dtype=torch.float32, device=x.device)
     t = fw.planes
-    rc = lib().scp_swin_ln_linear(x.data_ptr(), x.stride(0), None if valid is None else _dev(valid, torch.float32), t[0].data_ptr(), t[1].data_ptr(),
-                                  _opt(bias), _dev(fw.wbeta), float(eps), out.data_ptr(), out.stride(0), M, fw.N, _stream())
-    _check(rc, "scp_swin_ln_linear")
-    return out
-
-
-def swin_ln_qkv(x, fw, bias, eps=1e-5, valid=None):
+    args = (x.data_ptr(), x.stride(0), None if valid is None else _dev(valid, torch.float32), t[0].data_ptr(), t[1].data_ptr(),
+            _opt(bias), _dev(fw.wbeta), float(eps), out.data_ptr(), out.stride(0), M, fw.N)
+    if tiles is None:
+        _check(lib().scp_swin_ln_linear(*args, _stream()), "scp_swin_ln_linear")
+    else:
+        _check(lib().scp_swin_ln_linear_tiles(*args, _dev(tiles, torch.int32), int(tiles.shape[0]), _stream()), "scp_swin_ln_linear_tiles")
+    return out
+
+
+def swin_ln_qkv(x, fw, bias, eps=1e-5, valid=None, tiles=None, pad_tiles=None, pad_image=None):
     M = x.shape[0]
     if x.shape[1] != 256 or fw.K != 256 or x.stride(1) != 1 or fw.N not in (512, 768) or (M & 127):
         raise ScpError("swin_ln_qkv: 256-channel rows in multiples of 128, N = 768 or 512 expected")
     q = torch.empty((M, 256), dtype=torch.float32, device=x.device) if fw.N == 768 else None
     pl = torch.empty((4, M, 256), dtype=torch.bfloat16, device=x.device)
     t = fw.planes
-    rc = lib().scp_swin_ln_qkv(x.data_ptr(), x.stride(0), None if valid is None else _dev(valid, torch.float32), t[0].data_ptr(), t[1].data_ptr(),
-                               _opt(bias), _dev(fw.wbeta), float(eps), None if q is None else q.data_ptr(), 256, pl.data_ptr(), M, M, fw.N, _stream())
-    _check(rc, "scp_swin_ln_qkv")
+    args = (x.data_ptr(), x.stride(0), None if valid is None else _dev(valid, torch.float32), t[0].data_ptr(), t[1].data_ptr(),
+            _opt(bias), _dev(fw.wbeta), float(eps), None if q is None else q.data_ptr(), 256, pl.data_ptr(), M, M, fw.N)
+    if tiles is None:
+        _check(lib().scp_swin_ln_qkv(*args, _stream()), "scp_swin_ln_qkv")
+    else:
+        n_pad = 0 if pad_tiles is None else int(pad_tiles.shape[0])
+        if n_pad and (pad_image is None or tuple(pad_image.shape) != (4, 128, 256) or pad_image.dtype != torch.bfloat16):
+            raise ScpError("swin_ln_qkv: the pad tiles need the [4, 128, 256] bf16 planes of one padding tile (swin_ln_qkv_pad_image)")
+        _check(lib().scp_swin_ln_qkv_tiles(*args, _dev(tiles, torch.int32), int(tiles.shape[0]), _dev(pad_tiles, torch.int32) if n_pad else None, n_pad,
+                                           _dev(pad_image) if n_pad else None, _stream()), "scp_swin_ln_qkv_tiles")
     return q, KvPlanes(t=pl)
+
+
+def swin_ln_qkv_pad_image(fw, bias, eps=1e-5, device=None):
+    dev = device if device is not None else fw.wbeta.device
+    x = torch.zeros((128, 256), dtype=torch.float32, device=dev)
+    _, kv = swin_ln_qkv(x, fw, bias, eps, torch.zeros((128,), dtype=torch.float32, device=dev))
+    return kv.t.contiguous()
 
 
 class EdgeMlpWeights:
```
